# bminixhofer/zett

Hardware: AMD Instinct MI355X
Metric: predicted token-embeddings/sec (full target vocab) (higher is better)
Workload: dtype f16

## Files before the change

### zett_amd/csrc/gemm.hip.h

```cpp
#pragma once

#include <hip/hip_runtime.h>
#include <stdint.h>

#include <type_traits>

#ifndef ZETT_GROUP_M
#define ZETT_GROUP_M 4
#endif

namespace zett {

typedef __attribute__((ext_vector_type(16))) float f32x16;
typedef __attribute__((ext_vector_type(4))) float f32x4;
typedef __attribute__((ext_vector_type(8))) __bf16 bf16x8;
typedef __attribute__((ext_vector_type(4))) uint32_t u32x4;

typedef uint16_t bf16_t;
typedef _Float16 f16_t;
typedef __attribute__((ext_vector_type(8))) _Float16 f16x8;

__device__ __forceinline__ float bf16_to_f32(bf16_t v) { return __uint_as_float(((uint32_t)v) << 16); }
__device__ __forceinline__ bf16_t f32_to_bf16(float f) {
    return __builtin_bit_cast(bf16_t, (__bf16)f);
// ... 76 lines not shown
}

typedef __attribute__((ext_vector_type(2))) float f32x2;
#define ZETT_PIN_STAGE(arr, n) do { _Pragma("unroll") for (int e_ = 0; e_ < (n); ++e_) asm volatile("" : "+v"((arr)[e_])); } while (0)

template <int ACT, bool HAS_RES, bool HAS_SCALE, int NV>
__device__ __forceinline__ void epi_values(float (&vs)[NV], const float (&bias)[NV], const float (&res)[NV], const float (&sc)[NV], const float (&sh)[NV]) {
#pragma clang fp contract(off)
    static_assert(NV % 2 == 0, "pairs");
    constexpr int NP = NV / 2;
    f32x2 v[NP];
#pragma unroll
    for (int e = 0; e < NP; ++e) v[e] = f32x2{vs[2 * e], vs[2 * e + 1]} + f32x2{bias[2 * e], bias[2 * e + 1]};
    if (ACT == ACT_GELU_TANH) {
        f32x2 u2[NP], t[NP];
        ZETT_PIN_STAGE(v, NP);
#pragma unroll
        for (int e = 0; e < NP; ++e) u2[e] = (v[e] * v[e]) * v[e];
        ZETT_PIN_STAGE(u2, NP);
#pragma unroll
        for (int e = 0; e < NP; ++e) u2[e] = 1.5957691216057308f * __builtin_elementwise_fma(f32x2{0.044715f, 0.044715f}, u2[e], v[e]);
        ZETT_PIN_STAGE(u2, NP);
#pragma unroll
        for (int e = 0; e < NP; ++e) u2[e] = u2[e] * 1.4426950408889634f;
        ZETT_PIN_STAGE(u2, NP);
#pragma unroll
        for (int e = 0; e < NP; ++e) t[e] = f32x2{__builtin_amdgcn_exp2f(u2[e].x), __builtin_amdgcn_exp2f(u2[e].y)};
        ZETT_PIN_STAGE(t, NP);
#pragma unroll
        for (int e = 0; e < NP; ++e) t[e] = 1.0f + t[e];
        ZETT_PIN_STAGE(t, NP);
#pragma unroll
        for (int e = 0; e < NP; ++e) t[e] = f32x2{__builtin_amdgcn_rcpf(t[e].x), __builtin_amdgcn_rcpf(t[e].y)};
        ZETT_PIN_STAGE(t, NP);
#pragma unroll
        for (int e = 0; e < NP; ++e) t[e] = 1.0f - 2.0f * t[e];
        ZETT_PIN_STAGE(t, NP);
#pragma unroll
        for (int e = 0; e < NP; ++e) v[e] = (0.5f * v[e]) * (1.0f + t[e]);
        ZETT_PIN_STAGE(v, NP);
    } else if (ACT == ACT_GELU_ERF) {
        f32x2 z[NP], ax[NP], t[NP], p[NP], ex[NP];
        ZETT_PIN_STAGE(v, NP);
#pragma unroll
        for (int e = 0; e < NP; ++e) z[e] = v[e] * 0.70710678118654752440f;
        ZETT_PIN_STAGE(z, NP);
#pragma unroll
        for (int e = 0; e < NP; ++e) ax[e] = __builtin_elementwise_abs(z[e]);
#pragma unroll
        for (int e = 0; e < NP; ++e) t[e] = __builtin_elementwise_fma(f32x2{0.3275911f, 0.3275911f}, ax[e], f32x2{1.0f, 1.0f});
        ZETT_PIN_STAGE(t, NP);
#pragma unroll
        for (int e = 0; e < NP; ++e) t[e] = f32x2{__builtin_amdgcn_rcpf(t[e].x), __builtin_amdgcn_rcpf(t[e].y)};
        ZETT_PIN_STAGE(t, NP);
#pragma unroll
        for (int e = 0; e < NP; ++e) ex[e] = (ax[e] * ax[e]) * -1.4426950408889634f;
        ZETT_PIN_STAGE(ex, NP);
#pragma unroll
        for (int e = 0; e < NP; ++e) ex[e] = f32x2{__builtin_amdgcn_exp2f(ex[e].x), __builtin_amdgcn_exp2f(ex[e].y)};
        ZETT_PIN_STAGE(ex, NP);
#pragma unroll
        for (int e = 0; e < NP; ++e) p[e] = __builtin_elementwise_fma(f32x2{1.061405429f, 1.061405429f}, t[e], f32x2{-1.453152027f, -1.453152027f});
        ZETT_PIN_STAGE(p, NP);
#pragma unroll
        for (int e = 0; e < NP; ++e) p[e] = __builtin_elementwise_fma(p[e], t[e], f32x2{1.421413741f, 1.421413741f});
        ZETT_PIN_STAGE(p, NP);
#pragma unroll
        for (int e = 0; e < NP; ++e) p[e] = __builtin_elementwise_fma(p[e], t[e], f32x2{-0.284496736f, -0.284496736f});
        ZETT_PIN_STAGE(p, NP);
#pragma unroll
        for (int e = 0; e < NP; ++e) p[e] = __builtin_elementwise_fma(p[e], t[e], f32x2{0.254829592f, 0.254829592f});
        ZETT_PIN_STAGE(p, NP);
#pragma unroll
        for (int e = 0; e < NP; ++e) p[e] = -(p[e] * t[e]);
        ZETT_PIN_STAGE(p, NP);
#pragma unroll
        for (int e = 0; e < NP; ++e) p[e] = __builtin_elementwise_fma(p[e], ex[e], f32x2{1.0f, 1.0f});
        ZETT_PIN_STAGE(p, NP);
#pragma unroll
        for (int e = 0; e < NP; ++e) p[e] = 1.0f + __builtin_elementwise_copysign(p[e], z[e]);
        ZETT_PIN_STAGE(p, NP);
#pragma unroll
        for (int e = 0; e < NP; ++e) v[e] = (v[e] * 0.5f) * p[e];
        ZETT_PIN_STAGE(v, NP);
    }
    if (HAS_RES) {
#pragma unroll
        for (int e = 0; e < NP; ++e) v[e] = v[e] + f32x2{res[2 * e], res[2 * e + 1]};
    }
    if (HAS_SCALE) {
#pragma unroll
        for (int e = 0; e < NP; ++e) v[e] = __builtin_elementwise_fma(f32x2{sc[2 * e], sc[2 * e + 1]}, v[e], f32x2{sh[2 * e], sh[2 * e + 1]});
    }
#pragma unroll
    for (int e = 0; e < NP; ++e) { vs[2 * e] = v[e].x; vs[2 * e + 1] = v[e].y; }
}

template <typename T>
struct GemmEpilogue {
    const float* bias;
    int act;
    const float* residual;
    int ld_res;
    const float* res_stats;
    const float* res_gamma;
    const float* res_beta;
    const int32_t* res_index;
    float2* stats_part;
    int ld_part;
    const float* fold_stats;
    const float* fold_c;
    const float* scale;
    const float* shift;
    float* out_f32;
    int ld_f32;
    T* out_lo;
    int ld_lo;
    int split_col;
    float* out_f32_b;
    int32_t* range_flag;
    int range_final;
    const T* residual_lo;
    int ld_res_lo;
    void* dst;
    const int64_t* dst_rows;
    int64_t ld_dst;
    int dst_dtype;
};

template <typename T> struct LoRange { static constexpr bool checked = false; static constexpr float limit = 0.f; };
template <> struct LoRange<f16_t> { static constexpr bool checked = true; static constexpr float limit = 65504.0f; };
__device__ __forceinline__ bool out_of_range(float v, float limit) { return !(__builtin_fabsf(v) <= limit); }
constexpr float ZETT_F32_MAX = 3.402823466e38f;
constexpr int ZETT_RANGE_BIT_SOURCE = 1, ZETT_RANGE_BIT_ACTIVATION = 2, ZETT_RANGE_BIT_OUTPUT = 4, ZETT_RANGE_BIT_WEIGHT = 8, ZETT_RANGE_BIT_DEST = 16;
template <typename OT> __device__ __forceinline__ bool dest_overflow(float v) {
    if constexpr (std::is_same<OT, f16_t>::value) { const float a = __builtin_fabsf(v); return a >= 65520.0f && a <= 3.402823466e38f; }
    else return false;
}
__device__ __forceinline__ void range_report(int32_t* flag, bool bad, int bit) {
    if (bad && flag) atomicOr(flag, bit);
}

template <typename T>
struct GemmArgs {
    const T* A;
    int lda;
    const T* W;
    int ldw;
    int M, N, K;
    GemmEpilogue<T> epi;
    int tile_order = 0;
    int group = 0;
    int row0 = 0;
};

constexpr int GEMM_BM = 128;
constexpr int GEMM_BN = 128;
constexpr int GEMM_WAIT_VMCNT0 = 0x0F70;
constexpr int GEMM_ROW_BYTES = 128;
constexpr int GEMM_TILE_BYTES = GEMM_BM * GEMM_ROW_BYTES;

__device__ __forceinline__ int lds_chunk_off(int row, int chunk) {
    return row * GEMM_ROW_BYTES + ((chunk ^ ((row >> 1) & 7)) << 4);
}

template <typename T>
__device__ __forceinline__ void mfma_chunk(const u32x4& a, const u32x4& b, f32x16& acc);

template <>
__device__ __forceinline__ void mfma_chunk<bf16_t>(const u32x4& a, const u32x4& b, f32x16& acc) {
    acc = __builtin_amdgcn_mfma_f32_32x32x16_bf16(__builtin_bit_cast(bf16x8, a), __builtin_bit_cast(bf16x8, b),
                                                  acc, 0, 0, 0);
}
template <>
__device__ __forceinline__ void mfma_chunk<f16_t>(const u32x4& a, const u32x4& b, f32x16& acc) {
    acc = __builtin_amdgcn_mfma_f32_32x32x16_f16(__builtin_bit_cast(f16x8, a), __builtin_bit_cast(f16x8, b), acc, 0, 0, 0);
}
template <>
__device__ __forceinline__ void mfma_chunk<float>(const u32x4& a, const u32x4& b, f32x16& acc) {
#pragma unroll
    for (int j = 0; j < 4; ++j)
        acc = __builtin_amdgcn_mfma_f32_32x32x2f32(__uint_as_float(a[j]), __uint_as_float(b[j]), acc, 0, 0, 0);
}

template <typename T>
__global__ __launch_bounds__(256) void gemm_tn_kernel(GemmArgs<T> g) {
    extern __shared__ __attribute__((aligned(16))) unsigned char smem[];
    constexpr int EPC = 16 / (int)sizeof(T);
    constexpr int BK = GEMM_ROW_BYTES / (int)sizeof(T);

    const int tiles_m = (g.M + GEMM_BM - 1) / GEMM_BM;
    const int tiles_n = (g.N + GEMM_BN - 1) / GEMM_BN;
    const int nwg = tiles_m * tiles_n;
    int wg = blockIdx.x;
    {
        const int q = nwg >> 3, r = nwg & 7, xcd = wg & 7;
        wg = (xcd < r ? xcd * (q + 1) : r * (q + 1) + (xcd - r) * q) + (wg >> 3);
    }
    constexpr int GROUP_M = 8;
    const int group_size = GROUP_M * tiles_n;
    const int first_m = (wg / group_size) * GROUP_M;
    const int gm = (tiles_m - first_m) < GROUP_M ? (tiles_m - first_m) : GROUP_M;
    const int tm = first_m + (wg % group_size) % gm;
    const int tn = (wg % group_size) / gm;
    const int m0 = tm * GEMM_BM, n0 = tn * GEMM_BN;

    const int tid = threadIdx.x;
    const int lane = tid & 63, wave = tid >> 6;
    const int wm = wave >> 1, wn = wave & 1;
    const int l31 = lane & 31, hi = lane >> 5;

    const unsigned char* a_src[4];
    const unsigned char* w_src[4];
    int lds_dst[4];
#pragma unroll
    for (int i = 0; i < 4; ++i) {
        const int c = tid + 256 * i;
        const int row = c >> 3, ch = c & 7;
        int ar = m0 + row; ar = ar < g.M ? ar : g.M - 1;
        int wr = n0 + row; wr = wr < g.N ? wr : g.N - 1;
        a_src[i] = (const unsigned char*)(g.A + (size_t)ar * g.lda) + ch * 16;
        w_src[i] = (const unsigned char*)(g.W + (size_t)wr * g.ldw) + ch * 16;
        lds_dst[i] = lds_chunk_off(row, ch);
    }

    f32x16 acc[2][2];
#pragma unroll
    for (int i = 0; i < 2; ++i)
#pragma unroll
        for (int j = 0; j < 2; ++j)
#pragma unroll
            for (int r = 0; r < 16; ++r) acc[i][j][r] = 0.f;

    const int nk = g.K / BK;
    u32x4 ra[4], rw[4];
#pragma unroll
    for (int i = 0; i < 4; ++i) {
        ra[i] = *(const u32x4*)(a_src[i]);
        rw[i] = *(const u32x4*)(w_src[i]);
    }
#pragma unroll
    for (int i = 0; i < 4; ++i) {
        *(u32x4*)(smem + lds_dst[i]) = ra[i];
        *(u32x4*)(smem + GEMM_TILE_BYTES + lds_dst[i]) = rw[i];
    }
    __syncthreads();

    for (int kt = 0; kt < nk; ++kt) {
        const int cur = kt & 1;
        const unsigned char* As = smem + cur * 2 * GEMM_TILE_BYTES;
        const unsigned char* Ws = As + GEMM_TILE_BYTES;
        const bool more = kt + 1 < nk;
        if (more) {
            const size_t koff = (size_t)(kt + 1) * GEMM_ROW_BYTES;
#pragma unroll
            for (int i = 0; i < 4; ++i) {
                ra[i] = *(const u32x4*)(a_src[i] + koff);
                rw[i] = *(const u32x4*)(w_src[i] + koff);
            }
        }
#pragma unroll
        for (int kk = 0; kk < 4; ++kk) {
            const int ch = kk * 2 + hi;
            u32x4 fa[2], fw[2];
#pragma unroll
            for (int i = 0; i < 2; ++i) {
                fa[i] = *(const u32x4*)(As + lds_chunk_off(wm * 64 + i * 32 + l31, ch));
                fw[i] = *(const u32x4*)(Ws + lds_chunk_off(wn * 64 + i * 32 + l31, ch));
            }
#pragma unroll
            for (int i = 0; i < 2; ++i)
#pragma unroll
                for (int j = 0; j < 2; ++j) mfma_chunk<T>(fa[i], fw[j], acc[i][j]);
        }
        if (more) {
            unsigned char* Ad = smem + (cur ^ 1) * 2 * GEMM_TILE_BYTES;
#pragma unroll
            for (int i = 0; i < 4; ++i) {
                *(u32x4*)(Ad + lds_dst[i]) = ra[i];
                *(u32x4*)(Ad + GEMM_TILE_BYTES + lds_dst[i]) = rw[i];
            }
        }
        __syncthreads();
    }
    (void)EPC;

    const GemmEpilogue<T>& e = g.epi;
    bool bad_lo = false, bad_out = false;
#pragma unroll
    for (int j = 0; j < 2; ++j) {
        const int col = n0 + wn * 64 + j * 32 + l31;
        if (col >= g.N) continue;
        const float bias = e.bias ? e.bias[col] : 0.f;
        const float sc = e.scale ? e.scale[col] : 1.f;
        const float sh = e.shift ? e.shift[col] : 0.f;
#pragma unroll
        for (int i = 0; i < 2; ++i) {
#pragma unroll
            for (int r = 0; r < 16; ++r) {
                const int row = m0 + wm * 64 + i * 32 + (r & 3) + 8 * (r >> 2) + 4 * hi;
                if (row >= g.M) continue;
                const size_t rrow = e.res_index ? (size_t)e.res_index[row] : (size_t)row;
                float res = e.residual ? e.residual[rrow * e.ld_res + col] : 0.f;
                if (e.residual && e.res_stats) res = ln_affine(res, e.res_stats[2 * rrow], e.res_stats[2 * rrow + 1], e.res_gamma[col], e.res_beta[col]);
                const bool hr = e.residual != nullptr, hs = e.scale != nullptr;
                const float v = e.act == ACT_GELU_TANH ? epi_value<ACT_GELU_TANH>(acc[i][j][r], bias, hr, res, hs, sc, sh)
                              : e.act == ACT_GELU_ERF ? epi_value<ACT_GELU_ERF>(acc[i][j][r], bias, hr, res, hs, sc, sh)
// ... 31 lines not shown
```

### zett_amd/csrc/gemm4d.hip.h

```cpp
#pragma once

#include <hip/hip_runtime.h>
#include <stdint.h>

#include <algorithm>
#include <type_traits>

#include "gemm_tile.hip.h"

namespace zett {

#ifndef G4D_ABLATE
#define G4D_ABLATE 5
#endif
constexpr int G4D_ABL = G4D_ABLATE;
#ifdef G4D_MFMA32
constexpr bool G4D_M32 = true;
static_assert(G4D_ABLATE < 5, "the 32x32x16 K loop exists for the ablation levels without an epilogue");
#else
constexpr bool G4D_M32 = false;
#endif
typedef float f32x16 __attribute__((ext_vector_type(16)));

constexpr int g4d_wait_vm(int n) { return ((n >> 4) << 14) | 0x0F70 | (n & 15); }

template <typename T> __device__ __forceinline__ void mfma16_agpr(f32x4& c, const u32x4& a, const u32x4& b);
template <> __device__ __forceinline__ void mfma16_agpr<bf16_t>(f32x4& c, const u32x4& a, const u32x4& b) {
    asm volatile("v_mfma_f32_16x16x32_bf16 %0, %1, %2, %0" : "+a"(c) : "v"(a), "v"(b));
}
template <> __device__ __forceinline__ void mfma16_agpr<f16_t>(f32x4& c, const u32x4& a, const u32x4& b) {
    asm volatile("v_mfma_f32_16x16x32_f16 %0, %1, %2, %0" : "+a"(c) : "v"(a), "v"(b));
}

template <typename T> __device__ __forceinline__ void mfma32_agpr(f32x16& c, const u32x4& a, const u32x4& b);
template <> __device__ __forceinline__ void mfma32_agpr<bf16_t>(f32x16& c, const u32x4& a, const u32x4& b) {
    asm volatile("v_mfma_f32_32x32x16_bf16 %0, %1, %2, %0" : "+a"(c) : "v"(a), "v"(b));
}
template <> __device__ __forceinline__ void mfma32_agpr<f16_t>(f32x16& c, const u32x4& a, const u32x4& b) {
    asm volatile("v_mfma_f32_32x32x16_f16 %0, %1, %2, %0" : "+a"(c) : "v"(a), "v"(b));
}

template <int K> __device__ __forceinline__ float g4d_xor_lane(float v) {
    return __builtin_bit_cast(float, __builtin_amdgcn_ds_swizzle(__builtin_bit_cast(int, v), (K << 10) | 0x1f));
}


enum { G4D_EPI_GENERIC = 0, G4D_EPI_LO = 1, G4D_EPI_F32 = 2, G4D_EPI_F32_SCALE = 3, G4D_EPI_BOTH = 4, G4D_EPI_F32_LN = 5, G4D_EPI_LO_FOLD = 6,
       G4D_EPI_LO_LN = 7, G4D_EPI_F32_SCALE_FOLD = 8, G4D_EPI_LN16 = 9 };
constexpr int G4D_EPI_STRIDE = 132;
constexpr int G4D_EPI_REGION = 64 * G4D_EPI_STRIDE * 4;
constexpr int G4D_LDS_BYTES = 4 * G4D_EPI_REGION;
static_assert(G4D_LDS_BYTES >= G256_LDS_BYTES && G4D_LDS_BYTES <= 160 * 1024, "LDS budget");

template <bool HALF> struct G4dGeom {
    static constexpr int BM = HALF ? 128 : G256_BM;
    static constexpr int WROWS = BM / 2;
    static constexpr int MI = WROWS / 16;
    static constexpr int AREQ = BM / 32;
    static constexpr int NREQ = AREQ + 8;
    static constexpr int NPASS = WROWS / 64;
    static constexpr int STAGES = HALF ? 3 : 2;
    static constexpr int A_BYTES = BM * GEMM_ROW_BYTES;
    static constexpr int STAGE_BYTES = A_BYTES + G256_OPERAND_BYTES;
    static constexpr int LDS_BYTES = STAGES * STAGE_BYTES;
};

template <typename T, int ACT = ACT_NONE, bool RES = false, int EPI = G4D_EPI_GENERIC, bool HALF = false, typename OT = void>
__global__ __launch_bounds__(256) __attribute__((amdgpu_waves_per_eu(1, 1))) void gemm4d_tn_kernel(GemmArgs<T> g) {
    extern __shared__ __attribute__((aligned(16))) unsigned char smem[];
    constexpr int BK = GEMM_ROW_BYTES / (int)sizeof(T);
    typedef G4dGeom<HALF> GEO;
    static_assert(!HALF || EPI != G4D_EPI_GENERIC, "the half tile carries the streamlined epilogues only");
    constexpr bool DST = !std::is_void<OT>::value;
    static_assert(!DST || EPI == G4D_EPI_F32_SCALE || EPI == G4D_EPI_F32_SCALE_FOLD, "destination stores: the output heads' epilogues only");

    const int tiles_m = (g.M - g.row0 + GEO::BM - 1) / GEO::BM;
    const int tiles_n = (g.N + G256_BN - 1) / G256_BN;
    const int nwg = tiles_m * tiles_n;
    int wg = blockIdx.x;
    {
        const int q = nwg >> 3, r = nwg & 7, xcd = wg & 7;
        wg = (xcd < r ? xcd * (q + 1) : r * (q + 1) + (xcd - r) * q) + (wg >> 3);
    }
    const int GROUP_N = g.group > 0 ? g.group : 4;
    int tm, tn;
    if (g.tile_order == 0) {
        const int group_size = GROUP_N * tiles_m;
        const int first_n = (wg / group_size) * GROUP_N;
        const int gn = (tiles_n - first_n) < GROUP_N ? (tiles_n - first_n) : GROUP_N;
        tn = first_n + (wg % group_size) % gn;
        tm = (wg % group_size) / gn;
    } else {
        const int GROUP_M = g.group > 0 ? g.group : ZETT_GROUP_M;
        const int group_size = GROUP_M * tiles_n;
        const int first_m = (wg / group_size) * GROUP_M;
        const int gm = (tiles_m - first_m) < GROUP_M ? (tiles_m - first_m) : GROUP_M;
        tm = first_m + (wg % group_size) % gm;
        tn = (wg % group_size) / gm;
    }
    const int m0 = g.row0 + tm * GEO::BM, n0 = tn * G256_BN;

    const int tid = threadIdx.x;
    const int lane = tid & 63;
    const int wave = __builtin_amdgcn_readfirstlane(tid >> 6);
    const int wm = wave >> 1, wn = wave & 1;

    const unsigned char* a_base = (const unsigned char*)(g.A + (size_t)m0 * g.lda);
    const unsigned char* w_base = (const unsigned char*)(g.W + (size_t)n0 * g.ldw);
    uint32_t a_voff[8], w_voff[8];
#pragma unroll
    for (int r = 0; r < 8; ++r) {
        const int row = wave * 64 + r * 8 + (lane >> 3);
        const int chunk = ((lane & 7) ^ ((row >> 1) & 7)) << 4;
        int wr = row; wr = n0 + wr < g.N ? wr : g.N - 1 - n0;
        w_voff[r] = (uint32_t)wr * (uint32_t)g.ldw * (uint32_t)sizeof(T) + chunk;
    }
#pragma unroll
    for (int r = 0; r < GEO::AREQ; ++r) {
        const int row = wave * (GEO::AREQ * 8) + r * 8 + (lane >> 3);
        const int chunk = ((lane & 7) ^ ((row >> 1) & 7)) << 4;
        int ar = row; ar = m0 + ar < g.M ? ar : g.M - 1 - m0;
        a_voff[r] = (uint32_t)ar * (uint32_t)g.lda * (uint32_t)sizeof(T) + chunk;
    }
    const __amdgpu_buffer_rsrc_t a_rsrc = __builtin_amdgcn_make_buffer_rsrc((void*)a_base, (short)0, 0x7fffffff, G4R_RSRC_WORD3);
    const __amdgpu_buffer_rsrc_t w_rsrc = __builtin_amdgcn_make_buffer_rsrc((void*)w_base, (short)0, 0x7fffffff, G4R_RSRC_WORD3);
    unsigned char* const my_rows = smem + wave * 64 * GEMM_ROW_BYTES;
    unsigned char* const my_a_rows = smem + wave * (GEO::AREQ * 8) * GEMM_ROW_BYTES;
    auto dma_a = [&](int stage, int kt, int r) {
        __builtin_amdgcn_raw_ptr_buffer_load_lds(a_rsrc, (lds_ptr_t)(my_a_rows + stage * GEO::STAGE_BYTES + r * 8 * GEMM_ROW_BYTES), 16,
                                                 a_voff[r], kt * GEMM_ROW_BYTES, 0, 0);
    };
    auto dma_w = [&](int stage, int kt, int r) {
        __builtin_amdgcn_raw_ptr_buffer_load_lds(w_rsrc, (lds_ptr_t)(my_rows + stage * GEO::STAGE_BYTES + GEO::A_BYTES + r * 8 * GEMM_ROW_BYTES), 16,
                                                 w_voff[r], kt * GEMM_ROW_BYTES, 0, 0);
    };

    constexpr bool M32 = G4D_M32 && !HALF;
    f32x4 acc[8][8];
    f32x16 acc32[4][4];
    if constexpr (M32) {
#pragma unroll
        for (int i = 0; i < 4; ++i)
#pragma unroll
            for (int j = 0; j < 4; ++j)
#pragma unroll
                for (int r = 0; r < 16; ++r) acc32[i][j][r] = 0.f;
    } else {
#pragma unroll
    for (int i = 0; i < GEO::MI; ++i)
#pragma unroll
        for (int j = 0; j < 8; ++j)
#pragma unroll
            for (int r = 0; r < 4; ++r) acc[i][j][r] = 0.f;
    }

    int a_off[2], w_off[2];
    {
        const int l15 = lane & 15, kq = lane >> 4;
        const int swz = (l15 >> 1) & 7;
#pragma unroll
        for (int kb = 0; kb < 2; ++kb) {
            const int c = ((kb * 4 + kq) ^ swz) << 4;
            a_off[kb] = (wm * GEO::WROWS + l15) * GEMM_ROW_BYTES + c;
            w_off[kb] = GEO::A_BYTES + (wn * 128 + l15) * GEMM_ROW_BYTES + c;
        }
    }
    int a_off32[4], w_off32[4];
    if constexpr (M32) {
        const int l31 = lane & 31, kh = lane >> 5;
        const int swz = (l31 >> 1) & 7;
#pragma unroll
        for (int k16 = 0; k16 < 4; ++k16) {
            const int c = ((k16 * 2 + kh) ^ swz) << 4;
            a_off32[k16] = (wm * GEO::WROWS + l31) * GEMM_ROW_BYTES + c;
            w_off32[k16] = GEO::A_BYTES + (wn * 128 + l31) * GEMM_ROW_BYTES + c;
        }
    }
    u32x4 fa[2][8], fw[2][8];
    auto read_a = [&](int stage, int kb, int i) {
        if constexpr (M32) fa[kb][i] = *(const u32x4*)(smem + stage * GEO::STAGE_BYTES + a_off32[kb * 2 + (i >> 2)] + (i & 3) * 32 * GEMM_ROW_BYTES);
        else fa[kb][i] = *(const u32x4*)(smem + stage * GEO::STAGE_BYTES + a_off[kb] + i * 16 * GEMM_ROW_BYTES);
    };
    auto read_w = [&](int stage, int kb, int j) {
        if constexpr (M32) fw[kb][j] = *(const u32x4*)(smem + stage * GEO::STAGE_BYTES + w_off32[kb * 2 + (j >> 2)] + (j & 3) * 32 * GEMM_ROW_BYTES);
        else fw[kb][j] = *(const u32x4*)(smem + stage * GEO::STAGE_BYTES + w_off[kb] + j * 16 * GEMM_ROW_BYTES);
    };

    const int nk = g.K / BK;
    constexpr bool LN16K = EPI == G4D_EPI_LN16;
    uint4 res16[LN16K ? 16 : 1];
    const bool res16_early = LN16K && g.epi.res_index == nullptr;
    auto res16_request = [&](int p, int t) __attribute__((always_inline)) {
        if constexpr (LN16K) {
            int grow = m0 + wm * GEO::WROWS + p * 64 + t * 4 + (lane >> 4);
            grow = grow < g.M ? grow : g.M - 1;
            int gc = n0 + wn * 128 + (lane & 15) * 8;
            gc = gc < g.N ? gc : 0;
            res16[t] = *(const uint4*)(g.epi.residual_lo + (size_t)grow * g.epi.ld_res_lo + gc);
        }
    };
#pragma unroll
    for (int st = 0; st < GEO::STAGES; ++st) {
        if (st < nk) {
#pragma unroll
            for (int r = 0; r < 8; ++r) dma_w(st, st, r);
#pragma unroll
            for (int r = 0; r < GEO::AREQ; ++r) dma_a(st, st, r);
        }
    }
    {
        const int ahead = (nk < GEO::STAGES ? nk : GEO::STAGES) - 1;
        if (ahead >= 2) __builtin_amdgcn_s_waitcnt(g4d_wait_vm(2 * GEO::NREQ));
        else if (ahead == 1) __builtin_amdgcn_s_waitcnt(g4d_wait_vm(GEO::NREQ));
        else __builtin_amdgcn_s_waitcnt(g4d_wait_vm(0));
    }
    __builtin_amdgcn_s_barrier();
    __builtin_amdgcn_sched_barrier(0);
#pragma unroll
    for (int j = 0; j < 8; ++j) read_w(0, 0, j);
#pragma unroll
    for (int i = 0; i < GEO::MI; ++i) read_a(0, 0, i);
    if constexpr (G4D_ABL < 2) {
#pragma unroll
        for (int j = 0; j < 8; ++j) read_w(0, 1, j);
#pragma unroll
        for (int i = 0; i < GEO::MI; ++i) read_a(0, 1, i);
        __builtin_amdgcn_s_waitcnt(G4R_WAIT_LGKM0);
    }

    auto step = [&](int kt, int cur, auto more_c, auto more2_c, auto moreA_c, auto wave_c) {
        constexpr bool more = decltype(more_c)::value, more2 = decltype(more2_c)::value, moreA = decltype(moreA_c)::value;
        constexpr int WV = decltype(wave_c)::value;
        const int nxt = cur + 1 == GEO::STAGES ? 0 : cur + 1;
        constexpr int P_BAR1 = HALF ? 26 : 36, P_BAR2 = HALF ? 52 : 102;
        constexpr int INFLIGHT = HALF ? ((more2 ? 1 : 0) + (moreA ? 1 : 0)) * GEO::NREQ : (moreA ? GEO::NREQ : 0);
#pragma unroll
        for (int kb = 0; kb < 2; ++kb)
#pragma unroll
        for (int i = 0; i < GEO::MI; ++i)
// ... 301 lines not shown
                            const f32x2 y = __builtin_elementwise_fma(f32x2{v[u * CPL + c], v[u * CPL + c + 1]}, r2, x);
                            v[u * CPL + c] = y.x; v[u * CPL + c + 1] = y.y;
                            bb[u * CPL + c] = 0.f; bb[u * CPL + c + 1] = 0.f;
                        }
                    }
                }
                epi_values<ACT, RES, SCALE, NV>(v, bb, rr, ss, hh);
                if constexpr (CHK16) {
#pragma unroll
                    for (int x = 0; x < NV; ++x) bad |= out_of_range(v[x], LoRange<T>::limit);
                } else if (chk_final) {
#pragma unroll
                    for (int x = 0; x < NV; ++x) bad |= out_of_range(v[x], ZETT_F32_MAX);
                }
                if constexpr (LN16) {
                    static_assert(!LN16 || (GROUP == 4 && CPL == 8 && RPI == 4), "reduce-scatter layout");
                    float S[4], Q[4];
#pragma unroll
                    for (int u = 0; u < 4; ++u) {
                        const float* x = v + 8 * u;
                        S[u] = ((x[0] + x[1]) + (x[2] + x[3])) + ((x[4] + x[5]) + (x[6] + x[7]));
                        Q[u] = __builtin_fmaf(x[0], x[0], __builtin_fmaf(x[1], x[1], __builtin_fmaf(x[2], x[2], __builtin_fmaf(x[3], x[3],
                               __builtin_fmaf(x[4], x[4], __builtin_fmaf(x[5], x[5], __builtin_fmaf(x[6], x[6], x[7] * x[7])))))));
                    }
                    const bool b3 = (idx & 8) != 0, b2 = (idx & 4) != 0;
                    float ks0 = b3 ? S[2] : S[0], ks1 = b3 ? S[3] : S[1], kq0 = b3 ? Q[2] : Q[0], kq1 = b3 ? Q[3] : Q[1];
                    ks0 += g4d_xor_lane<8>(b3 ? S[0] : S[2]); ks1 += g4d_xor_lane<8>(b3 ? S[1] : S[3]);
                    kq0 += g4d_xor_lane<8>(b3 ? Q[0] : Q[2]); kq1 += g4d_xor_lane<8>(b3 ? Q[1] : Q[3]);
                    float ks = b2 ? ks1 : ks0, kq = b2 ? kq1 : kq0;
                    ks += g4d_xor_lane<4>(b2 ? ks0 : ks1); kq += g4d_xor_lane<4>(b2 ? kq0 : kq1);
                    ks += g4d_xor_lane<2>(ks); kq += g4d_xor_lane<2>(kq);
                    ks += g4d_xor_lane<1>(ks); kq += g4d_xor_lane<1>(kq);
                    const bool mine = (idx & 3) == (t0 >> 2);
                    acc_s = mine ? ks : acc_s; acc_q = mine ? kq : acc_q;
                } else if constexpr (LNP) {
                    static_assert(GROUP == 4 && CPL == 4 && RPI == 2, "reduce-scatter layout");
                    float S[4], Q[4];
#pragma unroll
                    for (int u = 0; u < 4; ++u) {
                        const float a = v[4 * u], b = v[4 * u + 1], c = v[4 * u + 2], d = v[4 * u + 3];
                        S[u] = (a + b) + (c + d);
                        Q[u] = __builtin_fmaf(a, a, __builtin_fmaf(b, b, __builtin_fmaf(c, c, d * d)));
                    }
                    const bool b4 = (idx & 16) != 0, b3 = (idx & 8) != 0;
                    float ks0 = b4 ? S[2] : S[0], ks1 = b4 ? S[3] : S[1], kq0 = b4 ? Q[2] : Q[0], kq1 = b4 ? Q[3] : Q[1];
                    ks0 += g4d_xor_lane<16>(b4 ? S[0] : S[2]); ks1 += g4d_xor_lane<16>(b4 ? S[1] : S[3]);
                    kq0 += g4d_xor_lane<16>(b4 ? Q[0] : Q[2]); kq1 += g4d_xor_lane<16>(b4 ? Q[1] : Q[3]);
                    float ks = b3 ? ks1 : ks0, kq = b3 ? kq1 : kq0;
                    ks += g4d_xor_lane<8>(b3 ? ks0 : ks1); kq += g4d_xor_lane<8>(b3 ? kq0 : kq1);
                    ks += g4d_xor_lane<4>(ks); kq += g4d_xor_lane<4>(kq);
                    ks += g4d_xor_lane<2>(ks); kq += g4d_xor_lane<2>(kq);
                    ks += g4d_xor_lane<1>(ks); kq += g4d_xor_lane<1>(kq);
                    const bool mine = (idx & 7) == (t0 >> 2);
                    acc_s = mine ? ks : acc_s; acc_q = mine ? kq : acc_q;
                }
#pragma unroll
                for (int u = 0; u < GROUP; ++u) {
                    const int grow = grow0 + p * 64 + (t0 + u) * RPI;
                    if (!FULL && (grow >= g.M || !col_ok)) continue;
                    if constexpr (LO || LN16) {
                        const float4 a = make_float4(v[u * 8], v[u * 8 + 1], v[u * 8 + 2], v[u * 8 + 3]);
                        const float4 b = make_float4(v[u * 8 + 4], v[u * 8 + 5], v[u * 8 + 6], v[u * 8 + 7]);
                        store_out8<T>(e.out_lo + (size_t)grow * e.ld_lo + gcol, a, b);
                    } else {
                        const f32x4 x = {v[u * 4], v[u * 4 + 1], v[u * 4 + 2], v[u * 4 + 3]};
                        if constexpr (DST) {
                            const int r0 = (t0 + u) * RPI;
                            static_assert(!DST || RPI == 2, "two rows per instruction");
                            const uint64_t d64 = (uint64_t)drow[p];
                            const uint32_t lo0 = __builtin_amdgcn_readlane((uint32_t)d64, r0), hi0 = __builtin_amdgcn_readlane((uint32_t)(d64 >> 32), r0);
                            const uint32_t lo1 = __builtin_amdgcn_readlane((uint32_t)d64, r0 + 1), hi1 = __builtin_amdgcn_readlane((uint32_t)(d64 >> 32), r0 + 1);
                            const int64_t d = (int64_t)(((uint64_t)(rsub ? hi1 : hi0) << 32) | (rsub ? lo1 : lo0));
                            if (d >= 0) {
                                store_out4<OT>((OT*)e.dst + d * e.ld_dst + gcol, make_float4(x[0], x[1], x[2], x[3]));
#pragma unroll
                                for (int c = 0; c < 4; ++c) bad_dst |= dest_overflow<OT>(x[c]);
                            }
                        } else if constexpr (WF32) {
                            float* d = e.out_f32 + (size_t)grow * e.ld_f32 + gcol;
                            if (RES) asm volatile("global_store_dwordx4 %0, %1, off nt\n\ts_nop 1" :: "v"(d), "v"(x) : "memory");
                            else *(f32x4*)d = x;
                        }
                        if constexpr (EPI == G4D_EPI_BOTH || LNP)
                            store_out4<T>(e.out_lo + (size_t)grow * e.ld_lo + gcol, make_float4(x[0], x[1], x[2], x[3]));
                    }
                }
                if constexpr (LN16 && GEO::NPASS == 2) { if (p == 0 && t0 == GROUP) load_res16(1, 0, NIT / 2); }
            }
            if constexpr (LN16 && GEO::NPASS == 2) { if (p == 0) load_res16(1, NIT / 2, NIT); }
            if constexpr (LNP) {
                const int rp = LN16 ? (((4 * (idx & 3) + 2 * ((idx >> 3) & 1) + ((idx >> 2) & 1)) << 2) + rsub)
                                    : (((4 * (idx & 7) + 2 * ((idx >> 4) & 1) + ((idx >> 3) & 1)) << 1) + rsub);
                const int grow = m0 + wm * GEO::WROWS + p * 64 + rp;
                if (grow < g.M && n0 + wn * 128 < g.N)
                    e.stats_part[(size_t)((n0 + wn * 128) >> 7) * e.ld_part + grow] = make_float2(acc_s, acc_q);
            }
        };
        auto drain_pass = [&](int p) {
            const bool full = m0 + wm * GEO::WROWS + p * 64 + 64 <= g.M && n0 + wn * 128 + 128 <= g.N;
            if (full) drain(p, std::integral_constant<bool, true>{});
            else drain(p, std::integral_constant<bool, false>{});
        };
        if constexpr (LN16) { if (!res16_early) load_res(0); }
        else load_res(0);
        stage(0);
        __builtin_amdgcn_sched_barrier(0);
        if constexpr (!LNP && GEO::NPASS == 2) load_res(1);
        __builtin_amdgcn_sched_barrier(0);
        drain_pass(0);
        if constexpr (GEO::NPASS == 2) {
            if constexpr (LNP && !LN16) { __builtin_amdgcn_sched_barrier(0); load_res(1); __builtin_amdgcn_sched_barrier(0); }
            stage(1);
            drain_pass(1);
        }
        range_report(e.range_flag, bad, W16 ? ZETT_RANGE_BIT_ACTIVATION : ZETT_RANGE_BIT_OUTPUT);
        if constexpr (DST) range_report(e.range_flag, bad_dst, ZETT_RANGE_BIT_DEST);
    }
}

template <typename T>
inline int gemm4d_epi_mode(const GemmArgs<T>& g) {
    const GemmEpilogue<T>& e = g.epi;
    if (e.stats_part && e.residual_lo) {
        if (sizeof(T) == 2 && e.out_lo && !e.out_f32 && !e.residual && e.act == ACT_NONE && !e.scale && !e.shift && !e.out_f32_b && e.split_col >= g.N &&
            g.N % 128 == 0 && e.ld_lo % 8 == 0 && e.ld_res_lo % 8 == 0) return G4D_EPI_LN16;
        return -1;
    }
    if (e.stats_part) {
        const bool common = e.out_lo && e.residual && !e.scale && !e.shift && !e.out_f32_b && e.split_col >= g.N && g.N % 128 == 0 &&
                            e.ld_lo % 4 == 0 && e.ld_res % 4 == 0;
        if (common && e.out_f32 && e.act == ACT_NONE && e.ld_f32 % 4 == 0) return G4D_EPI_F32_LN;
        if (common && !e.out_f32 && e.act == ACT_GELU_TANH && !e.res_stats && !e.res_index) return G4D_EPI_LO_LN;
        return -1;
    }
    if (e.fold_stats) {
        if (e.fold_c && e.out_lo && !e.out_f32 && !e.residual && !e.scale && !e.shift && !e.out_f32_b && e.split_col >= g.N &&
            g.N % 8 == 0 && e.ld_lo % 8 == 0) return G4D_EPI_LO_FOLD;
        if (e.fold_c && e.out_f32 && !e.out_lo && !e.residual && e.scale && e.shift && e.act == ACT_NONE && !e.out_f32_b && e.split_col >= g.N &&
            g.N % 4 == 0 && e.ld_f32 % 4 == 0) return G4D_EPI_F32_SCALE_FOLD;
        return -1;
    }
    if (e.out_f32_b || e.split_col < g.N) return G4D_EPI_GENERIC;
    if (e.res_stats && (e.act != ACT_NONE || !e.residual)) return G4D_EPI_GENERIC;
    if (e.out_lo && !e.out_f32 && !e.residual && !e.scale && !e.shift && g.N % 8 == 0 && e.ld_lo % 8 == 0) return G4D_EPI_LO;
    if (e.out_f32 && e.out_lo && !e.residual && !e.scale && !e.shift && e.act == ACT_NONE && g.N % 4 == 0 && e.ld_f32 % 4 == 0 && e.ld_lo % 4 == 0)
        return G4D_EPI_BOTH;
    if (e.out_f32 && !e.out_lo && g.N % 4 == 0 && e.ld_f32 % 4 == 0 && (!e.residual || e.ld_res % 4 == 0)) {
        if (e.scale && e.shift && !e.residual && e.act == ACT_NONE) return G4D_EPI_F32_SCALE;
        if (!e.scale && !e.shift && (e.act == ACT_NONE || (e.act == ACT_GELU_TANH && e.residual))) return G4D_EPI_F32;
    }
    return G4D_EPI_GENERIC;
}

template <typename T, int ACT, bool RES, int EPI, bool HALF = false>
inline hipError_t launch_gemm4d_inst(const GemmArgs<T>& g, hipStream_t stream) {
    constexpr int lds = EPI == G4D_EPI_GENERIC ? G256_LDS_BYTES : (G4dGeom<HALF>::LDS_BYTES > G4D_LDS_BYTES ? G4dGeom<HALF>::LDS_BYTES : G4D_LDS_BYTES);
    static_assert(lds <= 160 * 1024, "LDS budget");
    static DeviceFlags attr;
    bool* done = attr.current();
    if (!done || !*done) {
        hipError_t e = hipFuncSetAttribute((const void*)gemm4d_tn_kernel<T, ACT, RES, EPI, HALF>, hipFuncAttributeMaxDynamicSharedMemorySize, lds);
        if (e != hipSuccess) return e;
        if (done) *done = true;
    }
    constexpr int BM = HALF ? 128 : G256_BM;
    const int tiles_m = (g.M - g.row0 + BM - 1) / BM;
    const int tiles_n = (g.N + G256_BN - 1) / G256_BN;
    if (tiles_m <= 0 || tiles_n <= 0) return hipSuccess;
    hipLaunchKernelGGL((gemm4d_tn_kernel<T, ACT, RES, EPI, HALF>), dim3(tiles_m * tiles_n), dim3(256), lds, stream, g);
    return hipGetLastError();
}

template <typename T, int ACT, bool HALF>
inline hipError_t launch_gemm4d_act(const GemmArgs<T>& g, hipStream_t stream, int mode) {
    const bool res = g.epi.residual != nullptr;
    switch (mode) {
        case G4D_EPI_LO: return launch_gemm4d_inst<T, ACT, false, G4D_EPI_LO, HALF>(g, stream);
        case G4D_EPI_LO_FOLD: return launch_gemm4d_inst<T, ACT, false, G4D_EPI_LO_FOLD, HALF>(g, stream);
        case G4D_EPI_F32:
            if constexpr (ACT == ACT_NONE) return res ? launch_gemm4d_inst<T, ACT, true, G4D_EPI_F32, HALF>(g, stream) : launch_gemm4d_inst<T, ACT, false, G4D_EPI_F32, HALF>(g, stream);
            else if constexpr (ACT == ACT_GELU_TANH) { if (res) return launch_gemm4d_inst<T, ACT, true, G4D_EPI_F32, HALF>(g, stream); }
            [[fallthrough]];
        default:
            if constexpr (HALF) return hipErrorInvalidValue;
            else return res ? launch_gemm4d_inst<T, ACT, true, G4D_EPI_GENERIC>(g, stream) : launch_gemm4d_inst<T, ACT, false, G4D_EPI_GENERIC>(g, stream);
    }
}

template <typename T, bool HALF>
inline hipError_t launch_gemm4d_mode(const GemmArgs<T>& g, hipStream_t stream, int mode) {
    if (mode == G4D_EPI_F32_LN) return launch_gemm4d_inst<T, ACT_NONE, true, G4D_EPI_F32_LN, HALF>(g, stream);
    if (mode == G4D_EPI_LN16) return launch_gemm4d_inst<T, ACT_NONE, true, G4D_EPI_LN16, HALF>(g, stream);
    if (mode == G4D_EPI_LO_LN) return launch_gemm4d_inst<T, ACT_GELU_TANH, true, G4D_EPI_LO_LN, HALF>(g, stream);
    if (mode == G4D_EPI_F32_SCALE_FOLD) return launch_gemm4d_inst<T, ACT_NONE, false, G4D_EPI_F32_SCALE_FOLD, HALF>(g, stream);
    if (mode == G4D_EPI_F32_SCALE) return launch_gemm4d_inst<T, ACT_NONE, false, G4D_EPI_F32_SCALE, HALF>(g, stream);
    if (mode == G4D_EPI_BOTH) return launch_gemm4d_inst<T, ACT_NONE, false, G4D_EPI_BOTH, HALF>(g, stream);
    switch (g.epi.act) {
        case ACT_GELU_TANH: return launch_gemm4d_act<T, ACT_GELU_TANH, HALF>(g, stream, mode);
        case ACT_GELU_ERF: return launch_gemm4d_act<T, ACT_GELU_ERF, HALF>(g, stream, mode);
        default: return launch_gemm4d_act<T, ACT_NONE, HALF>(g, stream, mode);
    }
}

template <typename T>
inline bool gemm4d_half_ok(const GemmArgs<T>& g, int mode) {
    if (mode <= G4D_EPI_GENERIC) return false;
    if (mode == G4D_EPI_F32) return g.epi.act == ACT_NONE || (g.epi.act == ACT_GELU_TANH && g.epi.residual);
    return true;
}

inline int gemm4d_row_split(int M, int N, int cus = 256, double half_cost = 0.62) {
    const long tn = (N + G256_BN - 1) / G256_BN, tm = (M + G256_BM - 1) / G256_BM;
    const long T = tm * tn;
    if (T % cus == 0) return M;
    const long rounds = (T + cus - 1) / cus;
    const long tm_full = std::min<long>(tm, ((rounds - 1) * cus) / tn);
    const long row0 = tm_full * G256_BM;
    if (row0 >= M) return M;
    const long th = ((M - row0 + 127) / 128) * tn;
    const double cost = (double)((tm_full * tn + cus - 1) / cus) + half_cost * (double)((th + cus - 1) / cus);
    return cost < (double)rounds - 0.05 ? (int)row0 : M;
}

template <typename T, int EPI, typename OT, bool HALF>
inline hipError_t launch_gemm4d_dst_inst(const GemmArgs<T>& g, hipStream_t stream) {
    constexpr int lds = G4dGeom<HALF>::LDS_BYTES > G4D_LDS_BYTES ? G4dGeom<HALF>::LDS_BYTES : G4D_LDS_BYTES;
    static DeviceFlags attr;
    bool* done = attr.current();
    if (!done || !*done) {
        hipError_t e = hipFuncSetAttribute((const void*)gemm4d_tn_kernel<T, ACT_NONE, false, EPI, HALF, OT>, hipFuncAttributeMaxDynamicSharedMemorySize, lds);
        if (e != hipSuccess) return e;
        if (done) *done = true;
    }
    constexpr int BM = HALF ? 128 : G256_BM;
    const int tiles_m = (g.M - g.row0 + BM - 1) / BM;
    const int tiles_n = (g.N + G256_BN - 1) / G256_BN;
    if (tiles_m <= 0 || tiles_n <= 0) return hipSuccess;
    hipLaunchKernelGGL((gemm4d_tn_kernel<T, ACT_NONE, false, EPI, HALF, OT>), dim3(tiles_m * tiles_n), dim3(256), lds, stream, g);
    return hipGetLastError();
}

template <typename T, bool HALF>
inline hipError_t launch_gemm4d_dst_mode(const GemmArgs<T>& g, hipStream_t stream, int mode) {
    const int dt = g.epi.dst_dtype;
    if (mode == G4D_EPI_F32_SCALE_FOLD) {
        if (dt == 1) return launch_gemm4d_dst_inst<T, G4D_EPI_F32_SCALE_FOLD, f16_t, HALF>(g, stream);
        if (dt == 2) return launch_gemm4d_dst_inst<T, G4D_EPI_F32_SCALE_FOLD, bf16_t, HALF>(g, stream);
        return launch_gemm4d_dst_inst<T, G4D_EPI_F32_SCALE_FOLD, float, HALF>(g, stream);
    }
    if (dt == 1) return launch_gemm4d_dst_inst<T, G4D_EPI_F32_SCALE, f16_t, HALF>(g, stream);
    if (dt == 2) return launch_gemm4d_dst_inst<T, G4D_EPI_F32_SCALE, bf16_t, HALF>(g, stream);
    return launch_gemm4d_dst_inst<T, G4D_EPI_F32_SCALE, float, HALF>(g, stream);
}

template <typename T>
inline int gemm4d_dst_mode(const GemmArgs<T>& g) {
    const GemmEpilogue<T>& e = g.epi;
    if (!e.dst || e.dst_dtype < 0 || e.dst_dtype > 2 || e.ld_dst % 4 != 0) return -1;
    const size_t align = e.dst_dtype == 0 ? 16 : 8;
    if ((uintptr_t)e.dst % align) return -1;
    GemmArgs<T> f = g;
    f.epi.out_f32 = (float*)e.dst;
    f.epi.ld_f32 = 4;
    const int mode = gemm4d_epi_mode(f);
    return (mode == G4D_EPI_F32_SCALE || mode == G4D_EPI_F32_SCALE_FOLD) ? mode : -1;
}

hipError_t launch_gemm_4d_half(const GemmArgs<f16_t>& g, hipStream_t stream, int mode);
hipError_t launch_gemm_4d_half(const GemmArgs<bf16_t>& g, hipStream_t stream, int mode);

hipError_t launch_gemm_4d_half_dst(const GemmArgs<f16_t>& g, hipStream_t stream, int mode);
hipError_t launch_gemm_4d_half_dst(const GemmArgs<bf16_t>& g, hipStream_t stream, int mode);

template <typename T>
inline hipError_t launch_gemm4d(const GemmArgs<T>& g, hipStream_t stream, bool force_generic = false) {
    const bool dst = g.epi.dst != nullptr;
    const int mode = dst ? gemm4d_dst_mode(g) : (force_generic && !g.epi.stats_part && !g.epi.fold_stats) ? G4D_EPI_GENERIC : gemm4d_epi_mode(g);
    if (mode < 0) return hipErrorInvalidValue;
    int split = g.row0 == -1 ? gemm4d_row_split(g.M, g.N) : (g.row0 == -2 ? 0 : (g.row0 > 0 ? std::min(g.row0, g.M) : g.M));
    if (split < g.M && (!gemm4d_half_ok(g, mode) || split % G256_BM != 0)) split = g.M;
    GemmArgs<T> full = g;
    full.row0 = 0;
    if (split < g.M) {
        full.M = split;
        if (split > 0)
            if (hipError_t e = dst ? launch_gemm4d_dst_mode<T, false>(full, stream, mode) : launch_gemm4d_mode<T, false>(full, stream, mode); e != hipSuccess) return e;
        GemmArgs<T> rest = g;
        rest.row0 = split;
        return dst ? launch_gemm_4d_half_dst(rest, stream, mode) : launch_gemm_4d_half(rest, stream, mode);
    }
    return dst ? launch_gemm4d_dst_mode<T, false>(full, stream, mode) : launch_gemm4d_mode<T, false>(full, stream, mode);
}

}
```

### zett_amd/csrc/gemm4d.inc

```
#include <hip/hip_runtime.h>

#include "gemm.hip.h"
#include "gemm_tile.hip.h"
#include "gemm4d.hip.h"
#include "gemm_launch.hip.h"

namespace zett {

hipError_t launch_gemm_4d(const GemmArgs<ZETT_GEMM_T>& g, hipStream_t stream, bool generic_epilogue) {
    return launch_gemm4d<ZETT_GEMM_T>(g, stream, generic_epilogue);
}

int gemm_4d_dst_mode(const GemmArgs<ZETT_GEMM_T>& g) { return gemm4d_dst_mode<ZETT_GEMM_T>(g); }

}
```

### zett_amd/csrc/gemm_launch.hip.h

```cpp
#pragma once

#include <hip/hip_runtime.h>

#include "gemm.hip.h"

namespace zett {

hipError_t launch_gemm_variant(int variant, const GemmArgs<f16_t>& g, hipStream_t stream);
hipError_t launch_gemm_variant(int variant, const GemmArgs<bf16_t>& g, hipStream_t stream);
hipError_t launch_gemm_variant(int variant, const GemmArgs<float>& g, hipStream_t stream);

hipError_t launch_gemm_x(int variant, const GemmArgs<f16_t>& g, hipStream_t stream);
hipError_t launch_gemm_x(int variant, const GemmArgs<bf16_t>& g, hipStream_t stream);
hipError_t launch_gemm_x(int variant, const GemmArgs<float>& g, hipStream_t stream);
hipError_t launch_gemm_4d(const GemmArgs<f16_t>& g, hipStream_t stream, bool generic_epilogue);
hipError_t launch_gemm_4d(const GemmArgs<bf16_t>& g, hipStream_t stream, bool generic_epilogue);
int gemm_4d_dst_mode(const GemmArgs<f16_t>& g);
int gemm_4d_dst_mode(const GemmArgs<bf16_t>& g);
inline int gemm_4d_dst_mode(const GemmArgs<float>&) { return -1; }

}
```

### zett_amd/csrc/rowops.hip.h

```cpp
#pragma once

#include <hip/hip_runtime.h>
#include <stdint.h>

#include <type_traits>

#include "gemm.hip.h"

namespace zett {


struct PlanArrays {
    int32_t* row_count;
    int32_t* row_offset;
    uint8_t* row_uniform;
    int32_t* id_flag;
    int32_t* id_slot;
    int32_t* id_list;
    int32_t* tok_slot;
    int32_t* tok_pos;
    int32_t* tok_row;
    int32_t* tok_pkey;
    int32_t* pair_flag;
    int32_t* pair_slot;
    int32_t* tok_pair;
    int32_t* pair_tslot;
    int32_t* pair_pos;
    uint8_t* tok_key;
    int32_t* err;
    int32_t* counters;
    int32_t n_pair_keys;
};

__global__ void plan_rows_kernel(const int32_t* __restrict__ sfm, int64_t n_rows, int seq, int pad, int lam,
                                 int n_ids, PlanArrays p) {
    const int64_t n = (int64_t)blockIdx.x * blockDim.x + threadIdx.x;
    if (n >= n_rows) return;
    const int32_t* row = sfm + n * seq;
    int visible = 0;
    for (int j = 0; j < seq; ++j) {
        const int id = row[j];
        if (id < 0 || id >= n_ids) {
            atomicMax(p.err, (int)(n < 0x7ffffffe ? n + 1 : 0x7fffffff));
            p.row_count[n] = 0;
            p.row_uniform[n] = 2;
            return;
        }
        visible += (id != pad);
    }
    const bool uniform = (visible + lam) == 0;
    int count;
    if (uniform) {
        count = seq;
        for (int j = 0; j < seq; ++j) p.id_flag[row[j]] = 1;
    } else {
        count = visible + lam + (row[0] == pad ? 1 : 0);
        for (int j = 0; j < seq; ++j)
            if (j == 0 || row[j] != pad) p.id_flag[row[j]] = 1;
    }
    p.row_count[n] = count;
    p.row_uniform[n] = uniform ? 1 : 0;
}

__global__ __launch_bounds__(1024) void exclusive_scan_kernel(const int32_t* __restrict__ in,
                                                              int32_t* __restrict__ out, int64_t n) {
    __shared__ int32_t part[1024];
    const int t = threadIdx.x;
    const int64_t per = (n + 1023) / 1024;
    const int64_t b = (int64_t)t * per, e = (b + per < n) ? b + per : n;
    int32_t s = 0;
    for (int64_t i = b; i < e; ++i) s += in[i];
    part[t] = s;
    __syncthreads();
    for (int off = 1; off < 1024; off <<= 1) {
        int32_t v = (t >= off) ? part[t - off] : 0;
        __syncthreads();
        part[t] += v;
        __syncthreads();
    }
    int32_t run = (t == 0) ? 0 : part[t - 1];
    for (int64_t i = b; i < e; ++i) { const int32_t v = in[i]; out[i] = run; run += v; }
    if (t == 1023) out[n] = part[1023];
}

constexpr int SCAN_CHUNK = 4096;

__device__ __forceinline__ int32_t block_exclusive_scan_256(int32_t v, int32_t* sh , int32_t* total) {
    const int t = threadIdx.x;
    sh[t] = v;
    __syncthreads();
    for (int off = 1; off < 256; off <<= 1) {
        const int32_t add = (t >= off) ? sh[t - off] : 0;
        __syncthreads();
        sh[t] += add;
        __syncthreads();
    }
    if (total) *total = sh[255];
    return sh[t] - v;
}

__global__ __launch_bounds__(256) void scan_chunk_sums_kernel(const int32_t* __restrict__ in, int64_t n, int32_t* __restrict__ sums) {
    __shared__ int32_t sh[256];
    const int64_t base = (int64_t)blockIdx.x * SCAN_CHUNK + threadIdx.x * 16;
    int32_t s = 0;
#pragma unroll
    for (int k = 0; k < 16; ++k) { const int64_t i = base + k; if (i < n) s += in[i]; }
    int32_t total;
    block_exclusive_scan_256(s, sh, &total);
    if (threadIdx.x == 0) sums[blockIdx.x] = total;
}

__global__ __launch_bounds__(256) void scan_apply_kernel(const int32_t* __restrict__ in, int64_t n, const int32_t* __restrict__ offs,
                                                         int32_t* __restrict__ out) {
    __shared__ int32_t sh[256];
    const int64_t base = (int64_t)blockIdx.x * SCAN_CHUNK + threadIdx.x * 16;
    int32_t v[16];
    int32_t s = 0;
#pragma unroll
    for (int k = 0; k < 16; ++k) { const int64_t i = base + k; v[k] = i < n ? in[i] : 0; s += v[k]; }
    int32_t run = offs[blockIdx.x] + block_exclusive_scan_256(s, sh, nullptr);
#pragma unroll
    for (int k = 0; k < 16; ++k) { const int64_t i = base + k; if (i < n) out[i] = run; run += v[k]; }
    if (blockIdx.x == gridDim.x - 1 && threadIdx.x == 0) out[n] = offs[gridDim.x];
}

inline void launch_exclusive_scan(const int32_t* in, int32_t* out, int64_t n, int32_t* scratch, hipStream_t st) {
    if (n <= SCAN_CHUNK * 4) {
        hipLaunchKernelGGL(exclusive_scan_kernel, dim3(1), dim3(1024), 0, st, in, out, n);
        return;
    }
    const int chunks = (int)((n + SCAN_CHUNK - 1) / SCAN_CHUNK);
    int32_t* sums = scratch;
    int32_t* offs = scratch + chunks;
    hipLaunchKernelGGL(scan_chunk_sums_kernel, dim3(chunks), dim3(256), 0, st, in, n, sums);
    hipLaunchKernelGGL(exclusive_scan_kernel, dim3(1), dim3(1024), 0, st, (const int32_t*)sums, offs, (int64_t)chunks);
    hipLaunchKernelGGL(scan_apply_kernel, dim3(chunks), dim3(256), 0, st, in, n, (const int32_t*)offs, out);
}

__global__ void plan_tokens_kernel(const int32_t* __restrict__ sfm, int64_t n_rows, int seq, int pad, int lam,
                                   int n_ids, PlanArrays p) {
    const int64_t n = (int64_t)blockIdx.x * blockDim.x + threadIdx.x;
    if (n >= n_rows) return;
    const int32_t* row = sfm + n * seq;
    int t = p.row_offset[n];
    if (p.row_uniform[n] == 2) return;
    const bool uniform = p.row_uniform[n] == 1;
    const int lp = seq + lam;
    for (int j = 0; j < seq; ++j) {
        const int id = row[j];
        const bool vis = id != pad;
        if (uniform || vis || j == 0) {
            p.tok_slot[t] = p.id_slot[id];
            p.tok_pos[t] = j;
            p.tok_row[t] = (int32_t)n;
            p.tok_key[t] = vis ? 1 : 0;
            if (p.pair_flag) { const int key = id * lp + j; p.tok_pkey[t] = key; p.pair_flag[key] = 1; }
            ++t;
        }
    }
    if (lam) {
        p.tok_slot[t] = -1;
        p.tok_pos[t] = seq;
        p.tok_row[t] = (int32_t)n;
        p.tok_key[t] = 1;
        if (p.pair_flag) { const int key = n_ids * lp + seq; p.tok_pkey[t] = key; p.pair_flag[key] = 1; }
    }
}

__global__ void plan_pairs_kernel(int64_t n_rows, PlanArrays p) {
    const int64_t t = (int64_t)blockIdx.x * blockDim.x + threadIdx.x;
    if (t >= p.row_offset[n_rows]) return;
    const int ps = p.pair_slot[p.tok_pkey[t]];
    p.tok_pair[t] = ps;
    p.pair_tslot[ps] = p.tok_slot[t];
    p.pair_pos[ps] = p.tok_pos[t];
}

__device__ __forceinline__ int chunk_row(int t_rel, int row_rel, bool first, int rows);
__global__ void pair_rows_kernel(int m, int tok0, int64_t row0, int rows, PlanArrays p, int32_t* __restrict__ brow_pair) {
    const int t = blockIdx.x * blockDim.x + threadIdx.x;
    if (t >= m) return;
    const int n = p.tok_row[tok0 + t];
    brow_pair[chunk_row(t, (int)(n - row0), p.row_offset[n] == tok0 + t, rows)] = p.tok_pair[tok0 + t];
}

__global__ void plan_idlist_kernel(int n_ids, PlanArrays p) {
    const int id = blockIdx.x * blockDim.x + threadIdx.x;
    if (id < n_ids && p.id_flag[id]) p.id_list[p.id_slot[id]] = id;
    if (id == 0) {
        p.counters[0] = p.id_slot[n_ids];
        p.counters[1] = p.err[0];
        p.counters[2] = p.n_pair_keys ? p.pair_slot[p.n_pair_keys] : 0;
    }
}

__device__ __forceinline__ float wave_sum(float v) {
#pragma unroll
    for (int off = 32; off > 0; off >>= 1) v += __shfl_xor(v, off, 64);
    return v;
}

__device__ __forceinline__ float block_sum_256(float v, float* red ) {
    v = wave_sum(v);
    __syncthreads();
    if ((threadIdx.x & 63) == 0) red[threadIdx.x >> 6] = v;
    __syncthreads();
    return red[0] + red[1] + red[2] + red[3];
}

template <typename T> __device__ __forceinline__ void store_lo4(T* dst, float4 v);
template <> __device__ __forceinline__ void store_lo4<float>(float* dst, float4 v) { *(float4*)dst = v; }
template <> __device__ __forceinline__ void store_lo4<bf16_t>(bf16_t* dst, float4 v) {
    *(uint2*)dst = make_uint2(pack2_lo<bf16_t>(v.x, v.y), pack2_lo<bf16_t>(v.z, v.w));
}
template <> __device__ __forceinline__ void store_lo4<f16_t>(f16_t* dst, float4 v) {
    *(uint2*)dst = make_uint2(pack2_lo<f16_t>(v.x, v.y), pack2_lo<f16_t>(v.z, v.w));
}

template <int SRC_DTYPE> __device__ __forceinline__ float4 load_src4(const void* base, size_t elem);
template <> __device__ __forceinline__ float4 load_src4<0>(const void* base, size_t e) {
    return *(const float4*)((const float*)base + e);
}
template <> __device__ __forceinline__ float4 load_src4<1>(const void* base, size_t e) {
    const uint2 u = *(const uint2*)((const uint16_t*)base + e);
    typedef __attribute__((ext_vector_type(4))) _Float16 f16x4;
    const f16x4 hv = __builtin_bit_cast(f16x4, u);
    return make_float4((float)hv[0], (float)hv[1], (float)hv[2], (float)hv[3]);
}
template <> __device__ __forceinline__ float4 load_src4<2>(const void* base, size_t e) {
    const uint2 u = *(const uint2*)((const uint16_t*)base + e);
    return make_float4(__uint_as_float(u.x << 16), __uint_as_float(u.x & 0xffff0000u),
                       __uint_as_float(u.y << 16), __uint_as_float(u.y & 0xffff0000u));
}

template <typename T, int SRC_DTYPE>
__global__ __launch_bounds__(256) void gather_src_kernel(const int32_t* __restrict__ id_list, int slot0, int n_slots,
                                                         const void* __restrict__ src, int e_in, int v0,
                                                         const float* __restrict__ fallback,
                                                         const float* __restrict__ sc_w, const float* __restrict__ sc_b,
                                                         T* __restrict__ out, int32_t* __restrict__ range_flag) {
    const int s = blockIdx.x;
    if (s >= n_slots) return;
    const int id = id_list[slot0 + s];
    T* dst = out + (size_t)s * e_in;
    bool bad = false;
    auto chk = [&](float4 v) {
        if (LoRange<T>::checked)
            bad |= out_of_range(v.x, LoRange<T>::limit) | out_of_range(v.y, LoRange<T>::limit) | out_of_range(v.z, LoRange<T>::limit) |
                   out_of_range(v.w, LoRange<T>::limit);
    };
    if (id >= v0) {
        const float* f = fallback + (size_t)(id - v0) * e_in;
        for (int c = threadIdx.x * 4; c < e_in; c += 1024) { const float4 v = *(const float4*)(f + c); chk(v); store_lo4<T>(dst + c, v); }
    } else {
        const size_t base = (size_t)id * e_in;
        for (int c = threadIdx.x * 4; c < e_in; c += 1024) {
            float4 v = load_src4<SRC_DTYPE>(src, base + c);
            if (sc_w) {
                const float4 w = *(const float4*)(sc_w + c), b = *(const float4*)(sc_b + c);
                v.x = w.x * v.x + b.x; v.y = w.y * v.y + b.y; v.z = w.z * v.z + b.z; v.w = w.w * v.w + b.w;
            }
            chk(v);
            store_lo4<T>(dst + c, v);
        }
    }
    range_report(range_flag, bad, ZETT_RANGE_BIT_SOURCE);
}

struct LnEmbed {
    const float* table;
    const int32_t* tok_slot;
    const int32_t* tok_pos;
    const float* type0;
    const float* pos_emb;
    const float* lang;
    int lang_pos;
    const int32_t* tok_row;
    const int32_t* row_offset;
    int64_t row0;
    int rows;
    const void* table_lo;
    const float* table_stats;
    const float* table_gamma;
    const float* table_beta;
};

__device__ __forceinline__ int chunk_row(int t_rel, int row_rel, bool first, int rows) {
    return first ? row_rel : rows + t_rel - row_rel - 1;
}

struct LnReadout {
    const float* bias_w;
    const float* bias_b;
    float* out_bias;
    const void* in_lo;
    const int64_t* bias_rows;
    int32_t* range_flag;
};

template <typename BT> __device__ __forceinline__ void ln_readout_store(const LnReadout& ro, int r, float v) {
    if constexpr (std::is_void<BT>::value) {
        ro.out_bias[r] = v;
    } else {
        const int64_t d = ro.bias_rows ? ro.bias_rows[r] : (int64_t)r;
        if (d < 0) return;
        ((BT*)ro.out_bias)[d] = to_lo<BT>(v);
        range_report(ro.range_flag, dest_overflow<BT>(v), ZETT_RANGE_BIT_DEST);
    }
}

constexpr int LN_MAX_VEC = 8;

template <typename T, bool EMBED, int TPR = 256, bool READOUT = false, typename BT = void>
__global__ __launch_bounds__(256) void layernorm_rows_kernel(const float* __restrict__ in, int ld_in, int rows, int H,
                                                             const float* __restrict__ gamma,
                                                             const float* __restrict__ beta, float eps,
                                                             float* __restrict__ out_f32, T* __restrict__ out_lo,
                                                             float* __restrict__ stats_out, float* __restrict__ sum_out,
                                                             LnEmbed emb, int tok0, LnReadout readout) {
    __shared__ float red[4];
    const int r = blockIdx.x * (256 / TPR) + (int)threadIdx.x / TPR;
    if (r >= rows) return;
    const int nvec = H >> 2;
    const int tid = threadIdx.x % TPR;
    auto row_sum = [&](float x_) { return TPR == 256 ? block_sum_256(x_, red) : wave_sum(x_); };
    const float* x = nullptr;
    const float* posr = nullptr;
    bool is_lang = false;
    int ro = r;
    const T* tbl_lo = nullptr;
    float2 tbl_st = make_float2(0.f, 1.f);
    if constexpr (EMBED) {
        const int slot = emb.tok_slot[tok0 + r];
        is_lang = slot < 0;
        if (emb.table_lo && !is_lang) {
            tbl_lo = (const T*)emb.table_lo + (size_t)slot * H;
            tbl_st = *(const float2*)(emb.table_stats + 2 * (size_t)slot);
            x = emb.lang;
        } else
        x = is_lang ? emb.lang : emb.table + (size_t)slot * H;
        posr = emb.pos_emb + (size_t)emb.tok_pos[tok0 + r] * H;
        if (emb.tok_row) {
            const int n = emb.tok_row[tok0 + r];
            ro = chunk_row(r, (int)(n - emb.row0), emb.row_offset[n] == tok0 + r, emb.rows);
        }
// ... 187 lines not shown
                load8<float>(emb.pos_emb + (size_t)emb.lang_pos * H + c, pl);
#pragma unroll
                for (int k = 0; k < 8; ++k) a[k] -= (t0[k] + pl[k]);
            }
#pragma unroll
            for (int k = 0; k < 8; ++k) a[k] = (a[k] + t0[k]) + p[k];
        }
    };
    float v[NVMAX][8];
    float s = 0.f;
#pragma unroll
    for (int j = 0; j < NVMAX; ++j) {
        if (j < nv) {
            load((tid + TPR * j) * 8, v[j]);
            s += ((v[j][0] + v[j][1]) + (v[j][2] + v[j][3])) + ((v[j][4] + v[j][5]) + (v[j][6] + v[j][7]));
        }
    }
    const float mean = group_sum<TPR>(s) / (float)H;
    float q = 0.f;
#pragma unroll
    for (int j = 0; j < NVMAX; ++j) {
        if (j < nv) {
            float d[8];
#pragma unroll
            for (int k = 0; k < 8; ++k) { d[k] = v[j][k] - mean; d[k] *= d[k]; }
            q += ((d[0] + d[1]) + (d[2] + d[3])) + ((d[4] + d[5]) + (d[6] + d[7]));
        }
    }
    const float var = group_sum<TPR>(q) / (float)H;
    const float rstd = 1.0f / sqrtf(var + eps);
    if (stats_out && tid == 0) *(float2*)(stats_out + 2 * (size_t)ro) = make_float2(mean, rstd);
    float dot = 0.f;
#pragma unroll
    for (int j = 0; j < NVMAX; ++j) {
        if (j < nv) {
            const int c = (tid + TPR * j) * 8;
            float g[8], b[8], o[8];
            load8<float>(gamma + c, g);
            load8<float>(beta + c, b);
#pragma unroll
            for (int k = 0; k < 8; ++k) o[k] = ln_affine(v[j][k], mean, rstd, g[k], b[k]);
            if (EMBED && sum_out) store8<float>(sum_out + (size_t)ro * H + c, v[j]);
            if (out_f32) store8<float>(out_f32 + (size_t)ro * H + c, o);
            if (out_lo) store8<T>(out_lo + (size_t)ro * H + c, o);
            if (READOUT && readout.bias_w) {
                float w[8];
                load8<float>(readout.bias_w + c, w);
                dot += ((o[0] * w[0] + o[1] * w[1]) + (o[2] * w[2] + o[3] * w[3])) + ((o[4] * w[4] + o[5] * w[5]) + (o[6] * w[6] + o[7] * w[7]));
            }
        }
    }
    if constexpr (READOUT) {
        if (readout.out_bias) {
            const float tot = group_sum<TPR>(dot);
            if (tid == 0) ln_readout_store<BT>(readout, r, readout.bias_w ? tot + readout.bias_b[0] : 0.f);
        }
    }
}

constexpr int ATT_FAST_KEYS = 8;

template <typename T> __device__ __forceinline__ float dot8_lo(const uint4& a, const uint4& b);
template <> __device__ __forceinline__ float dot8_lo<f16_t>(const uint4& a, const uint4& b) {
    typedef __attribute__((ext_vector_type(2))) _Float16 h2;
    float s = __builtin_amdgcn_fdot2(__builtin_bit_cast(h2, a.x), __builtin_bit_cast(h2, b.x), 0.f, false);
    s = __builtin_amdgcn_fdot2(__builtin_bit_cast(h2, a.y), __builtin_bit_cast(h2, b.y), s, false);
    s = __builtin_amdgcn_fdot2(__builtin_bit_cast(h2, a.z), __builtin_bit_cast(h2, b.z), s, false);
    return __builtin_amdgcn_fdot2(__builtin_bit_cast(h2, a.w), __builtin_bit_cast(h2, b.w), s, false);
}
template <> __device__ __forceinline__ float dot8_lo<bf16_t>(const uint4& a, const uint4& b) {
    float x[8], y[8];
    unpack2_lo<bf16_t>(a.x, x[0], x[1]); unpack2_lo<bf16_t>(a.y, x[2], x[3]); unpack2_lo<bf16_t>(a.z, x[4], x[5]); unpack2_lo<bf16_t>(a.w, x[6], x[7]);
    unpack2_lo<bf16_t>(b.x, y[0], y[1]); unpack2_lo<bf16_t>(b.y, y[2], y[3]); unpack2_lo<bf16_t>(b.z, y[4], y[5]); unpack2_lo<bf16_t>(b.w, y[6], y[7]);
    float s = 0.f;
#pragma unroll
    for (int c = 0; c < 8; ++c) s = fmaf(x[c], y[c], s);
    return s;
}
template <> __device__ __forceinline__ float dot8_lo<float>(const uint4&, const uint4&) { return 0.f; }

__device__ __forceinline__ float head_sum(float s, int lph) {
    auto dpp = [](float v, auto ctrl) {
        return __builtin_bit_cast(float, __builtin_amdgcn_update_dpp(0, __builtin_bit_cast(int, v), decltype(ctrl)::value, 0xf, 0xf, true));
    };
    if (lph >= 2) s += dpp(s, std::integral_constant<int, 0xB1>{});
    if (lph >= 4) s += dpp(s, std::integral_constant<int, 0x4E>{});
    if (lph >= 8) s += dpp(s, std::integral_constant<int, 0x141>{});
    if (lph >= 16) s += dpp(s, std::integral_constant<int, 0x140>{});
    if (lph >= 32) s += __builtin_bit_cast(float, __builtin_amdgcn_ds_swizzle(__builtin_bit_cast(int, s), (16 << 10) | 0x1f));
    if (lph >= 64) s += __shfl_xor(s, 32, 64);
    return s;
}

struct AttentionWaves { int64_t total, full; int full_groups, lanes_per_row; };
__host__ __device__ inline AttentionWaves attention_waves(int rows, int H, bool pack) {
    const int rem = H & 511, gfull = H >> 9;
    AttentionWaves a;
    if (pack && (rem == 256 || rem == 128 || rem == 64)) {
        a.full_groups = gfull; a.lanes_per_row = rem >> 3;
        a.full = (int64_t)rows * gfull;
        const int per = 64 / a.lanes_per_row;
        a.total = a.full + (rows + per - 1) / per;
    } else {
        a.full_groups = (H + 511) >> 9; a.lanes_per_row = 64;
        a.full = (int64_t)rows * a.full_groups;
        a.total = a.full;
    }
    return a;
}

template <typename T>
__global__ __launch_bounds__(256) void attention_rows_kernel(const T* __restrict__ qbase, size_t ldq,
                                                             const T* __restrict__ kbase, const T* __restrict__ vbase,
                                                             size_t ldkv, int H, int head_dim,
                                                             const int32_t* __restrict__ row_offset,
                                                             const uint8_t* __restrict__ row_uniform,
                                                             const uint8_t* __restrict__ tok_key, int64_t row0,
                                                             int rows, int tok0, float scaling, int flags ,
                                                             const int32_t* __restrict__ tok_pair, T* __restrict__ ctx) {
    const int cls_only = flags & 1;
    const int lane = threadIdx.x & 63;
    const int64_t w = (int64_t)blockIdx.x * 4 + (threadIdx.x >> 6);
    const AttentionWaves aw = attention_waves(rows, H, (flags & 4) != 0);
    if (w >= aw.total) return;
    int rl, grp, li = lane, base = 0, lpr = 64;
    bool valid = true;
    if (w < aw.full) { rl = (int)(w / aw.full_groups); grp = (int)(w % aw.full_groups); }
    else {
        lpr = aw.lanes_per_row;
        const int sub = lane / lpr;
        li = lane - sub * lpr;
        base = sub * lpr;
        rl = (int)(w - aw.full) * (64 / lpr) + sub;
        grp = aw.full_groups;
        valid = rl < rows;
        if (!valid) rl = rows - 1;
    }
    const int col = grp * 512 + li * 8;
    const bool active = valid && col < H;
    const int lph = head_dim >> 3;
    const int64_t n = row0 + rl;
    const int t0 = row_offset[n] - tok0, t1 = row_offset[n + 1] - tok0;
    const bool uniform = row_uniform[n];
    const int nq = cls_only ? 1 : (t1 - t0);
    const int ccol = active ? col : 0;
    auto brow = [&](int t) -> size_t { return (size_t)chunk_row(t, rl, t == t0, rows); };
    int pslot = 0;
    if (tok_pair) { const int t = t0 + li; pslot = t < t1 ? tok_pair[tok0 + t] : 0; }
    auto qrow = [&](int t) -> size_t {
        if (!tok_pair) return brow(t);
        return t - t0 < lpr ? (size_t)__shfl(pslot, base + (t - t0), 64) : (size_t)tok_pair[tok0 + t];
    };
    const int nk = t1 - t0;
    if constexpr (sizeof(T) == 2) {
        if (nk <= ATT_FAST_KEYS && (flags & 2)) {
            const bool mine = li < nk && (uniform || tok_key[tok0 + t0 + li] != 0);
            const unsigned on = (unsigned)(__ballot(mine) >> base) & (lpr >= 32 ? 0xffffffffu : ((1u << lpr) - 1u));
            uint4 kk[ATT_FAST_KEYS], vv[ATT_FAST_KEYS], qq[ATT_FAST_KEYS];
#pragma unroll
            for (int j = 0; j < ATT_FAST_KEYS; ++j) {
                if (j < nk) {
                    const size_t kr = qrow(t0 + j);
                    kk[j] = *(const uint4*)(kbase + kr * ldkv + ccol);
                    vv[j] = *(const uint4*)(vbase + kr * ldkv + ccol);
                    if (!cls_only) qq[j] = *(const uint4*)(qbase + kr * ldq + ccol);
                }
            }
            if (cls_only) qq[0] = *(const uint4*)(qbase + (size_t)rl * ldq + ccol);
            const float sc2 = scaling * 1.4426950408889634f;
#pragma unroll
            for (int qi = 0; qi < ATT_FAST_KEYS; ++qi) {
                if (qi < nq) {
                    float sj[ATT_FAST_KEYS];
                    float mx = -INFINITY;
#pragma unroll
                    for (int j = 0; j < ATT_FAST_KEYS; ++j) {
                        sj[j] = -INFINITY;
                        if (j < nk && ((on >> j) & 1u)) {
                            const float d = head_sum(dot8_lo<T>(qq[qi], kk[j]), lph);
                            sj[j] = uniform ? 0.f : d * sc2;
                            mx = fmaxf(mx, sj[j]);
                        }
                    }
                    float l = 0.f, acc[8];
#pragma unroll
                    for (int c = 0; c < 8; ++c) acc[c] = 0.f;
#pragma unroll
                    for (int j = 0; j < ATT_FAST_KEYS; ++j) {
                        if (j < nk && ((on >> j) & 1u)) {
                            const float pj = __builtin_amdgcn_exp2f(sj[j] - mx);
                            l += pj;
                            float v[8];
                            unpack2_lo<T>(vv[j].x, v[0], v[1]); unpack2_lo<T>(vv[j].y, v[2], v[3]);
                            unpack2_lo<T>(vv[j].z, v[4], v[5]); unpack2_lo<T>(vv[j].w, v[6], v[7]);
#pragma unroll
                            for (int c = 0; c < 8; ++c) acc[c] = fmaf(pj, v[c], acc[c]);
                        }
                    }
                    const float inv = 1.0f / l;
#pragma unroll
                    for (int c = 0; c < 8; ++c) acc[c] *= inv;
                    if (active) {
                        const size_t orow = cls_only ? (size_t)rl : brow(t0 + qi);
                        store8<T>(ctx + orow * H + col, acc);
                    }
                }
            }
            return;
        }
    }
    for (int qi = 0; qi < nq; ++qi) {
        float q[8];
        load8<T>(qbase + (cls_only ? (size_t)rl : qrow(t0 + qi)) * ldq + ccol, q);
        float mx = -INFINITY, l = 0.f, acc[8];
#pragma unroll
        for (int c = 0; c < 8; ++c) acc[c] = 0.f;
        for (int kj = t0; kj < t1; ++kj) {
            if (!uniform && !tok_key[tok0 + kj]) continue;
            float k[8], v[8];
            const size_t kr = qrow(kj);
            load8<T>(kbase + kr * ldkv + ccol, k);
            load8<T>(vbase + kr * ldkv + ccol, v);
            float s = 0.f;
#pragma unroll
            for (int c = 0; c < 8; ++c) s = fmaf(q[c], k[c], s);
            for (int off = 1; off < lph; off <<= 1) s += __shfl_xor(s, off, 64);
            s = uniform ? 0.f : s * scaling;
            const float nm = fmaxf(mx, s);
            const float corr = expf(mx - nm);
            const float p = expf(s - nm);
            l = fmaf(l, corr, p);
#pragma unroll
            for (int c = 0; c < 8; ++c) acc[c] = fmaf(acc[c], corr, p * v[c]);
            mx = nm;
        }
        const float inv = 1.0f / l;
#pragma unroll
        for (int c = 0; c < 8; ++c) acc[c] *= inv;
        if (active) {
            const size_t orow = cls_only ? (size_t)rl : brow(t0 + qi);
            store8<T>(ctx + orow * H + col, acc);
        }
    }
}

__global__ __launch_bounds__(64) void ln_stats_kernel(const float2* __restrict__ part, int parts, int ld_part, int rows, int H, float eps,
                                                      float* __restrict__ stats) {
    const int r = blockIdx.x * blockDim.x + threadIdx.x;
    if (r >= rows) return;
    float s = 0.f, q = 0.f;
    const float2* col = part + r;
    int p = 0;
    for (; p + 8 <= parts; p += 8) {
        float2 v[8];
#pragma unroll
        for (int j = 0; j < 8; ++j) v[j] = col[(size_t)(p + j) * ld_part];
#pragma unroll
        for (int j = 0; j < 8; ++j) { s += v[j].x; q += v[j].y; }
    }
    {
        float2 v[8];
#pragma unroll
        for (int j = 0; j < 8; ++j) v[j] = p + j < parts ? col[(size_t)(p + j) * ld_part] : make_float2(0.f, 0.f);
#pragma unroll
        for (int j = 0; j < 8; ++j)
            if (p + j < parts) { s += v[j].x; q += v[j].y; }
    }
    const float mean = s / (float)H;
    const float var = fmaxf(q / (float)H - mean * mean, 0.f);
    *(float2*)(stats + 2 * (size_t)r) = make_float2(mean, 1.0f / sqrtf(var + eps));
}

template <typename T>
__global__ __launch_bounds__(256) void fold_weight_kernel(const float* __restrict__ w, int K, const float* __restrict__ gamma,
                                                          const float* __restrict__ beta, const float* __restrict__ bias,
                                                          T* __restrict__ w_fold, float* __restrict__ c_out, float* __restrict__ b_out,
                                                          int32_t* __restrict__ range_flag) {
    __shared__ float red[4];
    const int n = blockIdx.x;
    const float* row = w + (size_t)n * K;
    float cs = 0.f, bs = 0.f;
    for (int k = threadIdx.x; k < K; k += 256) {
        const float x = row[k];
        if (LoRange<T>::checked) range_report(range_flag, out_of_range(x * gamma[k], LoRange<T>::limit), ZETT_RANGE_BIT_WEIGHT);
        const T lo = to_lo<T>(x * gamma[k]);
        w_fold[(size_t)n * K + k] = lo;
        cs += lo_to_f32<T>(lo);
        bs = fmaf(x, beta[k], bs);
    }
    const float ct = block_sum_256(cs, red);
    const float bt = block_sum_256(bs, red);
    if (threadIdx.x == 0) { c_out[n] = ct; b_out[n] = bias[n] + bt; }
}

template <typename T>
__global__ void convert_f32_to_lo_kernel(const float* __restrict__ in, T* __restrict__ out, size_t n, int32_t* __restrict__ range_flag) {
    size_t i = ((size_t)blockIdx.x * blockDim.x + threadIdx.x) * 4;
    const size_t stride = (size_t)gridDim.x * blockDim.x * 4;
    bool bad = false;
    for (; i + 3 < n; i += stride) {
        const float4 v = *(const float4*)(in + i);
        if (LoRange<T>::checked)
            bad |= out_of_range(v.x, LoRange<T>::limit) | out_of_range(v.y, LoRange<T>::limit) | out_of_range(v.z, LoRange<T>::limit) |
                   out_of_range(v.w, LoRange<T>::limit);
        store_lo4<T>(out + i, v);
    }
    if (blockIdx.x == 0 && threadIdx.x == 0) {
        for (size_t j = n & ~(size_t)3; j < n; ++j) { out[j] = to_lo<T>(in[j]); if (LoRange<T>::checked) bad |= out_of_range(in[j], LoRange<T>::limit); }
    }
    range_report(range_flag, bad, ZETT_RANGE_BIT_WEIGHT);
}
template <int SRC_DTYPE>
__global__ void convert_to_f32_kernel(const void* __restrict__ in, float* __restrict__ out, size_t n) {
    size_t i = (size_t)blockIdx.x * blockDim.x + threadIdx.x;
    const size_t stride = (size_t)gridDim.x * blockDim.x;
    for (; i < n; i += stride) {
        if constexpr (SRC_DTYPE == 1) out[i] = (float)((const _Float16*)in)[i];
        else out[i] = __uint_as_float(((uint32_t)((const uint16_t*)in)[i]) << 16);
    }
}

template <typename OT> __device__ __forceinline__ void store4_dst(OT* d, float4 v) {
    if constexpr (std::is_same<OT, float>::value) *(float4*)d = v;
    else *(uint2*)d = make_uint2(pack2_lo<OT>(v.x, v.y), pack2_lo<OT>(v.z, v.w));
}

template <typename OT, bool VEC>
__global__ __launch_bounds__(256) void dest_store_rows_kernel(const float* __restrict__ src, int64_t ld_src, OT* __restrict__ dst, int64_t ld_dst,
                                                              const int64_t* __restrict__ rows, int64_t n_rows, int cols, int32_t* range_flag) {
    bool bad = false;
    for (int64_t i = blockIdx.x; i < n_rows; i += gridDim.x) {
        const int64_t d = rows ? rows[i] : i;
        if (d < 0) continue;
        const float* s = src + i * ld_src;
        OT* o = dst + d * ld_dst;
        if constexpr (VEC) {
            for (int c = (int)threadIdx.x * 4; c < cols; c += 256 * 4) {
                const float4 v = *(const float4*)(s + c);
                store4_dst<OT>(o + c, v);
                bad |= dest_overflow<OT>(v.x) | dest_overflow<OT>(v.y) | dest_overflow<OT>(v.z) | dest_overflow<OT>(v.w);
            }
        } else {
            for (int c = (int)threadIdx.x; c < cols; c += 256) {
                const float v = s[c];
                o[c] = to_lo<OT>(v);
                bad |= dest_overflow<OT>(v);
            }
        }
    }
    range_report(range_flag, bad, ZETT_RANGE_BIT_DEST);
}

__global__ void dest_rows_check_kernel(const int64_t* __restrict__ rows, int64_t n, int64_t n_dest, int32_t* err) {
    const int64_t i = (int64_t)blockIdx.x * blockDim.x + threadIdx.x;
    if (i < n && rows[i] >= n_dest) atomicMax(err, (int)(i < 0x7ffffffe ? i + 1 : 0x7fffffff));
}

}
```

### zett_amd/csrc/zett_hip.hip

```cpp
#include <hip/hip_runtime.h>

#include <algorithm>
#include <array>
#include <cstdlib>
#include <cmath>
#include <cstdarg>
#include <cstdio>
#include <cstring>
#include <map>
#include <string>
#include <type_traits>
#include <vector>

#include "../../include/zett_hip.h"
#include "common.hip.h"
#include "gemm.hip.h"
#include "gemm_launch.hip.h"
#include "rowops.hip.h"
#include "retok.hip.h"
#include "lexical.hip.h"
#include "partition.hip.h"

using namespace zett;

namespace {

struct Tensor {
    float* f32 = nullptr;
    void* lo = nullptr;
    std::vector<int64_t> shape;
    size_t numel = 0;
};

inline size_t round_up(size_t v, size_t m) { return (v + m - 1) / m * m; }

}

struct zett_hypernet {
    zett_config cfg{};
    int device = 0;
    int precision = ZETT_PREC_BF16;
    bool finalized = false;
    std::map<std::string, Tensor> w;
    std::vector<void*> qkv_w;
    std::vector<float*> qkv_b;
    struct Folded { void* w = nullptr; float* c = nullptr; float* b = nullptr; };
    std::vector<Folded> fold_qkv, fold_up;
    Folded fold_head_in, fold_head_out;
    float* head_one = nullptr;
    float* head_zero = nullptr;
    int ln_fold = 1;
    float* head_scale = nullptr;
    float* head_shift = nullptr;
    std::vector<void*> owned;
    int64_t max_chunk_tokens = 0;
    int time_gemm = 0;
    int cls_only_last = 1;
    int pair_dedupe = 1;
    int residual_lo = 1;
    int concurrent_lanes = 0;
    hipStream_t lane_stream = nullptr;
    hipEvent_t lane_ev[4] = {nullptr, nullptr, nullptr, nullptr};
    int attention_fast = 1;
    int attention_pack = 1;
    int gemm_tail_split = 1;
    int gemm_tile_order = 0;
    int ln_rows8 = 1;
    int table_lo = 1;
    int gemm_group = 0;
    int gemm4d_min_k = 512;
    int gemm_variant = 0;
    struct PlanSlot {
        DevBuf i32, u8;
        int32_t* host = nullptr;
        size_t host_ints = 0;
        hipEvent_t done = nullptr;
        hipEvent_t released = nullptr;
        const int32_t* sfm = nullptr;
        int64_t n_rows = 0;
        int seq = 0;
        bool pair_plan = false;
        const int32_t* ext_id_slot = nullptr;
        bool pending = false;
    } plan[2];
    PlanSlot table_plan;
    struct ExtTable { const void* table = nullptr; const float* stats = nullptr; const int32_t* id_slot = nullptr; } ext;
    int plan_cur = 0;
    hipStream_t plan_stream = nullptr;
    hipEvent_t plan_fork = nullptr;
    DevBuf table, x0, yf, yt, big, pre, ctx, cf, ct, lnstats, lnparts;
    hipEvent_t out_ready[2] = {nullptr, nullptr};
    bool out_recorded = false;
    int range_accumulate = 0;
    int32_t* range_word = nullptr;
    int32_t* range_host = nullptr;
    DevBuf dest_word, dest_stage[2], dest_sink;
    int32_t* dest_host = nullptr;
    hipEvent_t dest_checked = nullptr;
    std::vector<hipEvent_t> ev;
    size_t ev_used = 0;
    std::vector<double> ev_flops;
    std::vector<std::array<int, 4>> ev_shape;
    std::vector<zett_gemm_record> gemm_log;
    zett_stats stats{};
};

namespace {

size_t elt_size(int precision) { return precision == ZETT_PREC_F32 ? 4 : 2; }

bool is_gemm_weight(const std::string& n) {
    static const char* suffixes[] = {"input_projection.0.weight", "dense1.weight", "dense2.weight",
                                     "query.weight", "key.weight", "value.weight", "dense.weight",
                                     "output_projection.1.weight", "output_projection_out.1.weight"};
    for (const char* s : suffixes) {
        const size_t ls = strlen(s);
        if (n.size() >= ls && n.compare(n.size() - ls, ls, s) == 0) return true;
    }
    return false;
}

void expected_shapes(const zett_config& c, std::map<std::string, std::vector<int64_t>>& s) {
    const int64_t H = c.hidden, I = c.intermediate;
    auto proj = [&](const std::string& p) {
        s[p + "dense1.weight"] = {I, H}; s[p + "dense1.bias"] = {I};
        s[p + "dense2.weight"] = {H, I}; s[p + "dense2.bias"] = {H};
        s[p + "ln.weight"] = {H}; s[p + "ln.bias"] = {H};
    };
    if (c.embed_lang) s["lang_embeddings.weight"] = {c.n_langs, H};
    s["model.embeddings.token_type_embeddings.weight"] = {1, H};
    s["model.embeddings.LayerNorm.weight"] = {H};
    s["model.embeddings.LayerNorm.bias"] = {H};
    s["model.embeddings.position_embeddings.weight"] = {c.max_positions, H};
    for (int l = 0; l < c.layers; ++l) {
        const std::string p = "model.encoder.layer." + std::to_string(l) + ".";
        for (const char* q : {"query", "key", "value"}) {
            s[p + "attention.self." + q + ".weight"] = {H, H};
            s[p + "attention.self." + q + ".bias"] = {H};
        }
        s[p + "attention.output.dense.weight"] = {H, H}; s[p + "attention.output.dense.bias"] = {H};
        s[p + "attention.output.LayerNorm.weight"] = {H}; s[p + "attention.output.LayerNorm.bias"] = {H};
        s[p + "intermediate.dense.weight"] = {I, H}; s[p + "intermediate.dense.bias"] = {I};
        s[p + "output.dense.weight"] = {H, I}; s[p + "output.dense.bias"] = {H};
        s[p + "output.LayerNorm.weight"] = {H}; s[p + "output.LayerNorm.bias"] = {H};
    }
    s["fallback_embeddings.weight"] = {c.n_extra, c.n_in_embd};
    s["input_projection.0.weight"] = {H, c.n_in_embd}; s["input_projection.0.bias"] = {H};
    proj("input_projection.1.");
    proj("output_projection.0.");
    const int64_t w0 = c.single_head ? c.n_in_embd : c.n_embd;
    s["output_projection.1.weight"] = {w0, H}; s["output_projection.1.bias"] = {w0};
    if (c.separate_out && !c.single_head) {
        proj("output_projection_out.0.");
        s["output_projection_out.1.weight"] = {c.n_embd, H}; s["output_projection_out.1.bias"] = {c.n_embd};
    }
    if (c.rescale) {
        s["in_scaler.w"] = {1, c.n_in_embd}; s["in_scaler.b"] = {1, c.n_in_embd};
        s["scaler.w"] = {1, c.n_embd}; s["scaler.b"] = {1, c.n_embd};
        if (c.separate_out) { s["out_scaler.w"] = {1, c.n_embd}; s["out_scaler.b"] = {1, c.n_embd}; }
    }
    if (c.predict_bias) { s["bias_projection.weight"] = {1, H}; s["bias_projection.bias"] = {1}; }
}

int validate_config(const zett_config& c, int precision) {
    if (c.n_embd <= 0 || c.hidden <= 0 || c.intermediate <= 0 || c.heads <= 0 || c.layers <= 0)
        return fail(ZETT_E_INVALID, "non-positive dimension in zett_config");
    if (c.n_in_embd != (c.separate_out ? 2 * c.n_embd : c.n_embd))
        return fail(ZETT_E_INVALID, "n_in_embd must be 2*n_embd iff separate_out");
    if (c.hidden % c.heads) return fail(ZETT_E_INVALID, "hidden %d not divisible by heads %d", c.hidden, c.heads);
    const int d = c.hidden / c.heads;
    if (d < 8 || d > 512 || (d & (d - 1))) return fail(ZETT_E_INVALID, "head_dim %d unsupported (need a power of two in [8,512])", d);
    const int kq = precision == ZETT_PREC_F32 ? 32 : 64;
    for (int k : {c.n_in_embd, c.hidden, c.intermediate})
        if (k % kq) return fail(ZETT_E_INVALID, "contraction width %d is not a multiple of %d", k, kq);
    if (c.n_embd % 4) return fail(ZETT_E_INVALID, "n_embd must be a multiple of 4");
    if (c.n_extra < 1) return fail(ZETT_E_INVALID, "n_extra must be >= 1 (reference allocates max(hn_n_extra_tokens,1))");
    if (c.pad_token_id < 0) return fail(ZETT_E_INVALID, "pad_token_id is required");
    if (c.embed_lang && c.n_langs <= 0) return fail(ZETT_E_INVALID, "hn_embed_lang_id needs n_langs");
    return 0;
}

struct WorkspaceSizes {
    int64_t chunk_tokens;
    size_t table, x0, f32_rows, lo_rows, big, stats;
    size_t total() const { return table + x0 + 3 * f32_rows + 3 * lo_rows + big + stats; }
};

static int64_t pair_keys(const zett_config& c, int seq) {
    return ((int64_t)c.original_vocab_size + c.n_extra + 1) * (int64_t)(seq + (c.embed_lang ? 1 : 0));
}

static size_t plan_i32_bytes(const zett_config& c, int64_t N, int seq) {
    const int64_t V = (int64_t)c.original_vocab_size + c.n_extra;
    const int64_t max_tok = N * (int64_t)(seq + (c.embed_lang ? 1 : 0));
    const int64_t K = pair_keys(c, seq);
    const size_t scan_scratch = 2 * ((size_t)std::max<int64_t>(std::max<int64_t>(N, V), K) / SCAN_CHUNK + 2) + 1;
    return ((size_t)N + (N + 1) + 3 + V + (V + 1) + V + 7 * (size_t)max_tok + 2 * (size_t)K + 2 + scan_scratch) * 4;
}

static int64_t chunk_token_cap(const zett_config& c, size_t es) {
    const size_t wide = (size_t)std::max(c.intermediate, 3 * c.hidden);
    const size_t per_token = (size_t)c.n_in_embd * es + 3 * (size_t)c.hidden * 4 + 3 * (size_t)c.hidden * es + wide * es + 24;
    return std::max<int64_t>(131072, (int64_t)(((size_t)12 << 30) / per_token));
}

static WorkspaceSizes workspace_sizes(const zett_config& c, size_t es, int seq, int64_t Ttot, int64_t D, int64_t cap) {
    const int lam = c.embed_lang ? 1 : 0;
    WorkspaceSizes w{};
    if (cap <= 0) cap = chunk_token_cap(c, es);
    w.chunk_tokens = std::max<int64_t>(std::min<int64_t>(cap, std::max<int64_t>(Ttot, D)), seq + lam);
    const size_t MC = (size_t)w.chunk_tokens, MCS = MC + 768;
    const size_t wide = (size_t)std::max(c.intermediate, 3 * c.hidden);
    w.table = (size_t)D * c.hidden * 4;
    w.x0 = MCS * c.n_in_embd * es;
    w.f32_rows = MCS * c.hidden * 4;
    w.lo_rows = MCS * c.hidden * es;
    w.big = MCS * wide * es;
    w.stats = 2 * MCS * 2 * sizeof(float);
    return w;
}

struct PlanLayout {
    PlanArrays p{};
    int32_t* scan_tmp = nullptr;
    bool pair_plan = false;
    int64_t PK = 0;
    size_t n_clear = 0;
};
static PlanLayout plan_layout(const zett_hypernet* h, const zett_hypernet::PlanSlot& s, int64_t N, int seq) {
    const zett_config& c = h->cfg;
    const int lam = c.embed_lang ? 1 : 0;
    const int V = c.original_vocab_size + c.n_extra;
    const int64_t max_tok = N * (int64_t)(seq + lam);
    PlanLayout L;
    PlanArrays& p = L.p;
    L.PK = pair_keys(c, seq);
    L.pair_plan = h->pair_dedupe && c.layers >= 2 && L.PK <= std::max<int64_t>(4 * max_tok, (int64_t)1 << 23) && L.PK < (int64_t)0x7fffffff;
    int32_t* base = s.i32.as<int32_t>();
    p.id_flag = base; base += V;
    if (L.pair_plan) { p.pair_flag = base; base += L.PK; }
    p.err = base; base += 1;
    L.n_clear = (size_t)(base - s.i32.as<int32_t>());
    p.row_count = base; base += N;
    p.row_offset = base; base += N + 1;
    p.counters = base; base += 3;
    p.id_slot = base; base += V + 1;
    p.id_list = base; base += V;
    p.tok_slot = base; base += max_tok;
    p.tok_pos = base; base += max_tok;
    p.tok_row = base; base += max_tok;
    p.n_pair_keys = L.pair_plan ? (int32_t)L.PK : 0;
    if (L.pair_plan) {
        p.tok_pkey = base; base += max_tok;
        p.tok_pair = base; base += max_tok;
        p.pair_tslot = base; base += max_tok;
        p.pair_pos = base; base += max_tok;
        p.pair_slot = base; base += L.PK + 1;
    }
    L.scan_tmp = base;
    p.row_uniform = s.u8.as<uint8_t>();
    p.tok_key = p.row_uniform + N;
    return L;
}

static int enqueue_plan(zett_hypernet* h, zett_hypernet::PlanSlot& s, const int32_t* sfm, int64_t N, int seq, hipStream_t st) {
    const zett_config& c = h->cfg;
    const int lam = c.embed_lang ? 1 : 0;
    const int V = c.original_vocab_size + c.n_extra;
    const int64_t max_tok = N * (int64_t)(seq + lam);
    if (int rc = s.i32.reserve(plan_i32_bytes(c, N, seq))) return rc;
    if (int rc = s.u8.reserve((size_t)N + (size_t)max_tok)) return rc;
    const size_t need_ints = (size_t)N + 1 + 3;
    if (s.host_ints < need_ints) {
        if (s.host) (void)hipHostFree(s.host);
        s.host = nullptr;
        HIP_TRY(hipHostMalloc((void**)&s.host, need_ints * 4, hipHostMallocDefault));
        s.host_ints = need_ints;
    }
    if (!s.done) HIP_TRY(hipEventCreateWithFlags(&s.done, hipEventDisableTiming));
    if (!s.released) HIP_TRY(hipEventCreateWithFlags(&s.released, hipEventDisableTiming));
    const PlanLayout L = plan_layout(h, s, N, seq);
    const PlanArrays& p = L.p;
    HIP_TRY(hipMemsetAsync(s.i32.p, 0, L.n_clear * 4, st));
    const int rb = (int)((N + 255) / 256);
    hipLaunchKernelGGL(plan_rows_kernel, dim3(rb), dim3(256), 0, st, sfm, N, seq, c.pad_token_id, lam, V, p);
    launch_exclusive_scan(p.row_count, p.row_offset, N, L.scan_tmp, st);
    launch_exclusive_scan(p.id_flag, p.id_slot, (int64_t)V, L.scan_tmp, st);
    {
        PlanArrays pt = p;
        if (h->ext.id_slot) pt.id_slot = const_cast<int32_t*>(h->ext.id_slot);
        hipLaunchKernelGGL(plan_tokens_kernel, dim3(rb), dim3(256), 0, st, sfm, N, seq, c.pad_token_id, lam, V, pt);
    }
    if (L.pair_plan) {
        launch_exclusive_scan(p.pair_flag, p.pair_slot, L.PK, L.scan_tmp, st);
        hipLaunchKernelGGL(plan_pairs_kernel, dim3((unsigned)((max_tok + 255) / 256)), dim3(256), 0, st, N, p);
    }
    hipLaunchKernelGGL(plan_idlist_kernel, dim3((V + 255) / 256), dim3(256), 0, st, V, p);
    HIP_TRY(hipGetLastError());
    HIP_TRY(hipMemcpyAsync(s.host, p.row_offset, ((size_t)N + 1 + 3) * 4, hipMemcpyDeviceToHost, st));
    HIP_TRY(hipEventRecord(s.done, st));
    s.sfm = sfm; s.n_rows = N; s.seq = seq; s.pair_plan = L.pair_plan; s.ext_id_slot = h->ext.id_slot;
    return 0;
}

template <typename T>
int do_forward(zett_hypernet* h, const int32_t* sfm, int64_t N, int seq, const void* src, int src_dtype, const zett_dest* dest,
               int64_t v_src, int lang_index, float* out_in, float* out_out, float* out_bias, hipStream_t st);
template <typename T>
int do_table_rows(zett_hypernet* h, const int32_t* id_list, int first, int count, const void* src, int src_dtype, void* table_out, float* stats_out, hipStream_t st);

}

extern "C" {

const char* zett_last_error(void) { return g_err.c_str(); }
int zett_abi_version(void) { return ZETT_ABI_VERSION; }

int zett_create(const zett_config* cfg, int device, int precision, zett_hypernet** out) {
    if (!cfg || !out) return fail(ZETT_E_INVALID, "null argument");
    if (precision != ZETT_PREC_BF16 && precision != ZETT_PREC_F32 && precision != ZETT_PREC_F16) return fail(ZETT_E_INVALID, "unknown precision %d", precision);
    if (int rc = validate_config(*cfg, precision)) return rc;
    int ndev = 0;
    HIP_TRY(hipGetDeviceCount(&ndev));
    if (device < 0 || device >= ndev) return fail(ZETT_E_INVALID, "device %d out of range (%d visible)", device, ndev);
    ZETT_ON_DEVICE(device);
    auto* h = new zett_hypernet();
    h->cfg = *cfg;
    h->device = device;
    h->precision = precision;
    if (hipMalloc((void**)&h->range_word, 64) != hipSuccess || hipHostMalloc((void**)&h->range_host, 64, hipHostMallocDefault) != hipSuccess ||
        hipMemset(h->range_word, 0, 64) != hipSuccess) {
        if (h->range_word) (void)hipFree(h->range_word);
        if (h->range_host) (void)hipHostFree(h->range_host);
        delete h;
        return fail(ZETT_E_HIP, "allocation of the range word failed");
    }
    *out = h;
    return 0;
}

int zett_destroy(zett_hypernet* h) {
    if (!h) return 0;
    ::zett::DeviceScope _scope(h->device);
    for (auto& kv : h->w) {
        if (kv.second.f32) (void)hipFree(kv.second.f32);
        if (kv.second.lo && kv.second.lo != (void*)kv.second.f32) (void)hipFree(kv.second.lo);
    }
    for (void* p : h->owned) (void)hipFree(p);
    for (DevBuf* b : {&h->table, &h->x0, &h->yf, &h->yt, &h->big, &h->pre, &h->ctx, &h->cf, &h->ct, &h->lnstats, &h->lnparts, &h->dest_word, &h->dest_stage[0], &h->dest_stage[1], &h->dest_sink})
        b->release();
    for (zett_hypernet::PlanSlot* psp : {&h->plan[0], &h->plan[1], &h->table_plan}) {
        zett_hypernet::PlanSlot& ps = *psp;
        ps.i32.release(); ps.u8.release();
        if (ps.host) (void)hipHostFree(ps.host);
        if (ps.done) (void)hipEventDestroy(ps.done);
        if (ps.released) (void)hipEventDestroy(ps.released);
    }
    if (h->plan_stream) (void)hipStreamDestroy(h->plan_stream);
    if (h->plan_fork) (void)hipEventDestroy(h->plan_fork);
    if (h->range_word) (void)hipFree(h->range_word);
    if (h->range_host) (void)hipHostFree(h->range_host);
    if (h->dest_host) (void)hipHostFree(h->dest_host);
    if (h->dest_checked) (void)hipEventDestroy(h->dest_checked);
    for (hipEvent_t e : h->out_ready) if (e) (void)hipEventDestroy(e);
    for (hipEvent_t e : h->lane_ev) if (e) (void)hipEventDestroy(e);
    if (h->lane_stream) (void)hipStreamDestroy(h->lane_stream);
    for (hipEvent_t e : h->ev) (void)hipEventDestroy(e);
    delete h;
    return 0;
}

int zett_load_weight(zett_hypernet* h, const char* name, const void* data, int dtype, const int64_t* shape, int ndim) {
    if (!h || !name || !data || !shape || ndim < 1) return fail(ZETT_E_INVALID, "null argument");
    if (h->finalized) return fail(ZETT_E_STATE, "weights are frozen after zett_finalize");
    std::map<std::string, std::vector<int64_t>> exp;
    expected_shapes(h->cfg, exp);
    const std::string n(name);
    auto it = exp.find(n);
    if (it == exp.end()) return 0;
    std::vector<int64_t> got(shape, shape + ndim);
    if (got != it->second) {
        std::string a, b;
        for (auto v : got) a += std::to_string(v) + ",";
        for (auto v : it->second) b += std::to_string(v) + ",";
        return fail(ZETT_E_INVALID, "%s: shape [%s] does not match the config's [%s]", name, a.c_str(), b.c_str());
    }
    ZETT_ON_DEVICE(h->device);
    size_t numel = 1;
    for (auto v : got) numel *= (size_t)v;
    Tensor& t = h->w[n];
    if (t.f32) { (void)hipFree(t.f32); t.f32 = nullptr; }
    t.shape = got;
    t.numel = numel;
    HIP_TRY(hipMalloc((void**)&t.f32, numel * 4));
    if (dtype == ZETT_F32) {
        HIP_TRY(hipMemcpy(t.f32, data, numel * 4, hipMemcpyDefault));
    } else if (dtype == ZETT_F16 || dtype == ZETT_BF16) {
        void* stage = nullptr;
        HIP_TRY(hipMalloc(&stage, numel * 2));
        hipError_t e = hipMemcpy(stage, data, numel * 2, hipMemcpyDefault);
        if (e == hipSuccess) {
            const int blocks = (int)std::min<size_t>((numel + 255) / 256, 65535);
            if (dtype == ZETT_F16) hipLaunchKernelGGL(convert_to_f32_kernel<1>, dim3(blocks), dim3(256), 0, 0, stage, t.f32, numel);
            else hipLaunchKernelGGL(convert_to_f32_kernel<2>, dim3(blocks), dim3(256), 0, 0, stage, t.f32, numel);
            e = hipDeviceSynchronize();
        }
        (void)hipFree(stage);
        if (e != hipSuccess) return fail(ZETT_E_HIP, "upload of %s failed: %s", name, hipGetErrorString(e));
    } else {
        return fail(ZETT_E_INVALID, "unknown dtype %d", dtype);
    }
    return 0;
}

int zett_finalize(zett_hypernet* h) {
    if (!h) return fail(ZETT_E_INVALID, "null handle");
    if (h->finalized) return 0;
    ZETT_ON_DEVICE(h->device);
    std::map<std::string, std::vector<int64_t>> exp;
    expected_shapes(h->cfg, exp);
    for (auto& kv : exp)
        if (!h->w.count(kv.first)) return fail(ZETT_E_STATE, "missing weight: %s", kv.first.c_str());
    const zett_config& c = h->cfg;
    const size_t es = elt_size(h->precision);
    for (auto& kv : h->w) {
        Tensor& t = kv.second;
        if (!is_gemm_weight(kv.first)) continue;
        if (h->precision == ZETT_PREC_F32) { t.lo = t.f32; continue; }
        HIP_TRY(hipMalloc(&t.lo, t.numel * 2));
        const int blocks = (int)std::min<size_t>((t.numel / 4 + 255) / 256 + 1, 65535);
        if (h->precision == ZETT_PREC_F16)
            hipLaunchKernelGGL(convert_f32_to_lo_kernel<f16_t>, dim3(blocks), dim3(256), 0, 0, t.f32, (f16_t*)t.lo, t.numel, h->range_word);
        else
            hipLaunchKernelGGL(convert_f32_to_lo_kernel<bf16_t>, dim3(blocks), dim3(256), 0, 0, t.f32, (bf16_t*)t.lo, t.numel, h->range_word);
    }
    HIP_TRY(hipDeviceSynchronize());
    const size_t H = c.hidden;
    for (int l = 0; l < c.layers; ++l) {
        const std::string p = "model.encoder.layer." + std::to_string(l) + ".attention.self.";
        void* wq = nullptr; float* bq = nullptr;
        HIP_TRY(hipMalloc(&wq, 3 * H * H * es));
        HIP_TRY(hipMalloc((void**)&bq, 3 * H * 4));
        h->owned.push_back(wq); h->owned.push_back(bq);
        int k = 0;
        for (const char* q : {"query", "key", "value"}) {
            Tensor& tw = h->w[p + q + ".weight"];
            Tensor& tb = h->w[p + q + ".bias"];
            HIP_TRY(hipMemcpy((char*)wq + (size_t)k * H * H * es, tw.lo, H * H * es, hipMemcpyDeviceToDevice));
            HIP_TRY(hipMemcpy(bq + (size_t)k * H, tb.f32, H * 4, hipMemcpyDeviceToDevice));
            ++k;
        }
        h->qkv_w.push_back(wq);
        h->qkv_b.push_back(bq);
    }
    if (h->precision != ZETT_PREC_F32 && c.hidden % 128 == 0) {
        auto fold = [&](const float* w32, size_t N, size_t K, const float* gamma, const float* beta, const float* bias,
                        zett_hypernet::Folded& f) -> int {
            HIP_TRY(hipMalloc(&f.w, N * K * es));
            HIP_TRY(hipMalloc((void**)&f.c, N * 4));
            HIP_TRY(hipMalloc((void**)&f.b, N * 4));
            h->owned.push_back(f.w); h->owned.push_back(f.c); h->owned.push_back(f.b);
            if (h->precision == ZETT_PREC_F16)
                hipLaunchKernelGGL(fold_weight_kernel<f16_t>, dim3((unsigned)N), dim3(256), 0, 0, w32, (int)K, gamma, beta, bias, (f16_t*)f.w, f.c, f.b, h->range_word);
            else
                hipLaunchKernelGGL(fold_weight_kernel<bf16_t>, dim3((unsigned)N), dim3(256), 0, 0, w32, (int)K, gamma, beta, bias, (bf16_t*)f.w, f.c, f.b, h->range_word);
            return 0;
        };
        h->fold_qkv.resize(c.layers); h->fold_up.resize(c.layers);
        float* tmp = nullptr;
        HIP_TRY(hipMalloc((void**)&tmp, 3 * H * H * 4));
        for (int l = 0; l < c.layers; ++l) {
            const std::string lp = "model.encoder.layer." + std::to_string(l) + ".";
            if (int rc = fold(h->w[lp + "intermediate.dense.weight"].f32, c.intermediate, H, h->w[lp + "attention.output.LayerNorm.weight"].f32,
                              h->w[lp + "attention.output.LayerNorm.bias"].f32, h->w[lp + "intermediate.dense.bias"].f32, h->fold_up[l])) return rc;
            if (l == 0) continue;
            const std::string pp = "model.encoder.layer." + std::to_string(l - 1) + ".output.LayerNorm.";
            int k = 0;
            for (const char* q : {"query", "key", "value"}) {
                HIP_TRY(hipMemcpy(tmp + (size_t)k * H * H, h->w[lp + "attention.self." + q + ".weight"].f32, H * H * 4, hipMemcpyDeviceToDevice));
                ++k;
            }
            if (int rc = fold(tmp, 3 * H, H, h->w[pp + "weight"].f32, h->w[pp + "bias"].f32, h->qkv_b[l], h->fold_qkv[l])) return rc;
        }
        if (!(c.single_head && c.separate_out)) {
            const size_t w0 = c.single_head ? c.n_in_embd : c.n_embd;
            if (int rc = fold(h->w["output_projection.1.weight"].f32, w0, H, h->w["output_projection.0.ln.weight"].f32,
                              h->w["output_projection.0.ln.bias"].f32, h->w["output_projection.1.bias"].f32, h->fold_head_in)) return rc;
            if (c.separate_out && !c.single_head)
                if (int rc = fold(h->w["output_projection_out.1.weight"].f32, c.n_embd, H, h->w["output_projection_out.0.ln.weight"].f32,
                                  h->w["output_projection_out.0.ln.bias"].f32, h->w["output_projection_out.1.bias"].f32, h->fold_head_out)) return rc;
            std::vector<float> ones(w0, 1.0f), zeros(w0, 0.0f);
            HIP_TRY(hipMalloc((void**)&h->head_one, w0 * 4));
            HIP_TRY(hipMalloc((void**)&h->head_zero, w0 * 4));
            h->owned.push_back(h->head_one); h->owned.push_back(h->head_zero);
            HIP_TRY(hipMemcpy(h->head_one, ones.data(), w0 * 4, hipMemcpyHostToDevice));
            HIP_TRY(hipMemcpy(h->head_zero, zeros.data(), w0 * 4, hipMemcpyHostToDevice));
        }
        HIP_TRY(hipDeviceSynchronize());
        (void)hipFree(tmp);
    }
    HIP_TRY(hipMemcpy(h->range_host, h->range_word, 4, hipMemcpyDeviceToHost));
    if (h->range_host[0] & ZETT_RANGE_WEIGHT)
        return fail(ZETT_E_RANGE, "a GEMM weight (or a LayerNorm-folded weight W*gamma) exceeds the half range (|w| > 65504 or not finite): "
                                  "this checkpoint needs ZETT_PREC_BF16 or ZETT_PREC_F32");
    if (c.rescale) {
        const size_t w0 = c.single_head ? c.n_in_embd : c.n_embd;
        HIP_TRY(hipMalloc((void**)&h->head_scale, w0 * 4));
        HIP_TRY(hipMalloc((void**)&h->head_shift, w0 * 4));
        h->owned.push_back(h->head_scale); h->owned.push_back(h->head_shift);
        HIP_TRY(hipMemcpy(h->head_scale, h->w["scaler.w"].f32, c.n_embd * 4, hipMemcpyDeviceToDevice));
        HIP_TRY(hipMemcpy(h->head_shift, h->w["scaler.b"].f32, c.n_embd * 4, hipMemcpyDeviceToDevice));
        if (c.single_head && c.separate_out) {
            HIP_TRY(hipMemcpy(h->head_scale + c.n_embd, h->w["out_scaler.w"].f32, c.n_embd * 4, hipMemcpyDeviceToDevice));
            HIP_TRY(hipMemcpy(h->head_shift + c.n_embd, h->w["out_scaler.b"].f32, c.n_embd * 4, hipMemcpyDeviceToDevice));
        }
    }
    if (h->precision != ZETT_PREC_F32) {
        for (auto& kv : h->w) {
            Tensor& t = kv.second;
            if (is_gemm_weight(kv.first) && t.f32) { (void)hipFree(t.f32); t.f32 = nullptr; }
        }
    }
    h->finalized = true;
    return 0;
}

int zett_set_option(zett_hypernet* h, const char* key, int64_t value) {
    if (!h || !key) return fail(ZETT_E_INVALID, "null argument");
    const std::string k(key);
    if (k == "max_chunk_tokens") {
        if (value < 1024) return fail(ZETT_E_INVALID, "max_chunk_tokens must be >= 1024");
        h->max_chunk_tokens = value;
    } else if (k == "time_gemm") {
        h->time_gemm = value != 0;
    } else if (k == "cls_only_last_layer") {
        h->cls_only_last = value != 0;
    } else if (k == "pair_dedupe") {
        h->pair_dedupe = value != 0;
    } else if (k == "residual_lo") {
        if (value < 0 || value > 2) return fail(ZETT_E_INVALID, "residual_lo must be 0 (fp32 residual stream), 1 (16-bit stream in f16 mode) or 2 (in bf16 mode too)");
        h->residual_lo = (int)value;
    } else if (k == "concurrent_lanes") {
        if (value < 0 || value > 2) return fail(ZETT_E_INVALID, "concurrent_lanes must be 0 (never), 1 (auto) or 2 (whenever a call is one chunk of >= 512 rows)");
        h->concurrent_lanes = (int)value;
    } else if (k == "attention_fast") {
        h->attention_fast = value != 0;
    } else if (k == "ln_fold") {
        if (value < 0 || value > 2) return fail(ZETT_E_INVALID, "ln_fold must be 0 (off), 1 (encoder and output heads) or 2 (encoder only: A/B)");
        h->ln_fold = (int)value;
    } else if (k == "gemm_tail_split") {
        if (value < 0 || value > 3) return fail(ZETT_E_INVALID, "gemm_tail_split must be 0 (never), 1 (auto), 2 (cut every gemm4d launch in the middle) or 3 (128x256 tiles only)");
        h->gemm_tail_split = (int)value;
    } else if (k == "attention_pack") {
        h->attention_pack = value != 0;
    } else if (k == "ln_rows8") {
        h->ln_rows8 = value != 0;
    } else if (k == "table_lo") {
        h->table_lo = value != 0;
    } else if (k == "gemm_group") {
        if (value < 0 || value > 64) return fail(ZETT_E_INVALID, "gemm_group must be 0 (default: 4) .. 64");
        h->gemm_group = (int)value;
    } else if (k == "gemm_tile_order") {
        if (value < 0 || value > 1) return fail(ZETT_E_INVALID, "gemm_tile_order must be 0 or 1");
        h->gemm_tile_order = (int)value;
    } else if (k == "gemm4d_min_k") {
        if (value < 64) return fail(ZETT_E_INVALID, "gemm4d_min_k must be >= 64");
        h->gemm4d_min_k = (int)value;
    } else if (k == "range_accumulate") {
        h->range_accumulate = value != 0;
    } else if (k == "gemm_variant") {
        if (value != 0 && value != 1 && value != 2 && value != 3 && value != 7 && value != 8)
            return fail(ZETT_E_INVALID, "gemm_variant must be 0 (auto), 1 (128x128), 2 (256x256 register-staged), 3 (384x256), 7 (256x256 four-wave direct-to-LDS) or 8 (7 with the generic epilogue drain)");
        h->gemm_variant = (int)value;
    } else {
        return fail(ZETT_E_INVALID, "unknown option %s", key);
    }
    return 0;
}

int zett_workspace_bytes(const zett_hypernet* h, int64_t n_rows, int32_t seq, int64_t* out_bytes) {
    if (!h || !out_bytes) return fail(ZETT_E_INVALID, "null argument");
    if (n_rows < 0 || seq < 1) return fail(ZETT_E_INVALID, "bad surface-form shape [%lld, %d]", (long long)n_rows, seq);
    const zett_config& c = h->cfg;
    const int64_t V = (int64_t)c.original_vocab_size + c.n_extra;
    const int64_t max_tok = n_rows * (int64_t)(seq + (c.embed_lang ? 1 : 0));
    const WorkspaceSizes w = workspace_sizes(c, elt_size(h->precision), seq, max_tok, std::min<int64_t>(V, max_tok), h->max_chunk_tokens);
    const size_t parts = c.hidden % 128 == 0 ? (size_t)(c.hidden / 128) * ((size_t)w.chunk_tokens + 768) * 8 : 0;
    *out_bytes = (int64_t)(w.total() + parts + plan_i32_bytes(c, n_rows, seq) + (size_t)n_rows + (size_t)max_tok);
    return 0;
}

int zett_get_stats(const zett_hypernet* h, zett_stats* out) {
    if (!h || !out) return fail(ZETT_E_INVALID, "null argument");
    *out = h->stats;
    return 0;
}

int zett_stream_wait_output(zett_hypernet* h, int which, void* stream) {
    if (!h) return fail(ZETT_E_INVALID, "null handle");
    if (which != ZETT_OUT_IN && which != ZETT_OUT_BIAS) return fail(ZETT_E_INVALID, "which must be ZETT_OUT_IN or ZETT_OUT_BIAS");
    if (!h->out_recorded) return fail(ZETT_E_STATE, "no forward has run on this handle");
    ZETT_ON_DEVICE(h->device);
    HIP_TRY(hipStreamWaitEvent((hipStream_t)stream, h->out_ready[which], 0));
    return 0;
}

int zett_get_gemm_log(const zett_hypernet* h, zett_gemm_record* out, int64_t capacity, int64_t* count) {
    if (!h || !count || capacity < 0 || (capacity > 0 && !out)) return fail(ZETT_E_INVALID, "null argument");
    *count = (int64_t)h->gemm_log.size();
    for (int64_t i = 0; i < capacity && i < *count; ++i) out[i] = h->gemm_log[(size_t)i];
    return 0;
}

int zett_check_range(zett_hypernet* h, void* stream, int32_t* flags) {
    if (!h) return fail(ZETT_E_INVALID, "null handle");
    ZETT_ON_DEVICE(h->device);
    hipStream_t st = (hipStream_t)stream;
    HIP_TRY(hipMemcpyAsync(h->range_host, h->range_word, 4, hipMemcpyDeviceToHost, st));
    HIP_TRY(hipStreamSynchronize(st));
    const int32_t w = h->range_host[0];
    if (h->range_accumulate && w) HIP_TRY(hipMemsetAsync(h->range_word, 0, 4, st));
    if (flags) *flags = w;
    if (!w) return 0;
    return fail(ZETT_E_RANGE, "the last forward left the range of its arithmetic:%s%s%s%s (precision %s)",
                (w & ZETT_RANGE_SOURCE) ? " in_scaler(source_embeddings) beyond the half range;" : "",
                (w & ZETT_RANGE_ACTIVATION) ? " a 16-bit activation (Q/K/V, FFN intermediate or the operand copy of the residual sum) beyond the half range;" : "",
                (w & ZETT_RANGE_OUTPUT) ? " non-finite predicted embeddings;" : "",
                (w & ZETT_RANGE_DEST) ? " a finite value beyond the range of an f16 destination (stored as inf);" : "",
                h->precision == ZETT_PREC_F16 ? "f16: re-run with ZETT_PREC_BF16" : h->precision == ZETT_PREC_BF16 ? "bf16" : "f32");
}

int zett_partition_workspace_bytes(int64_t n_rows, int32_t n_ids, int64_t* out_bytes) {
    if (!out_bytes || n_rows < 0 || n_ids < 1) return fail(ZETT_E_INVALID, "bad argument");
    *out_bytes = (int64_t)partition_workspace_bytes(n_rows, n_ids);
    return 0;
}

int zett_partition_rows(const int32_t* surface_forms, int64_t n_rows, int32_t seq, int32_t pad_id, int32_t n_ids, int32_t world,
                        const int32_t* caps, int32_t* perm_out, void* workspace, int64_t workspace_bytes, int32_t device, void* stream) {
    if (n_rows < 0 || seq < 1 || n_ids < 1) return fail(ZETT_E_INVALID, "bad surface-form shape [%lld, %d] / id range %d", (long long)n_rows, seq, n_ids);
    if (world < 1 || world > PART_MAX_RANKS) return fail(ZETT_E_INVALID, "zett_partition_rows handles 1..%d ranks (one node), got %d", PART_MAX_RANKS, world);
    if (n_rows == 0) return 0;
    if (!surface_forms || !caps || !perm_out || !workspace) return fail(ZETT_E_INVALID, "null argument");
    if (n_rows >= (int64_t)0x7fffffff) return fail(ZETT_E_INVALID, "too many rows for one call");
    int64_t total = 0;
    for (int r = 0; r < world; ++r) { if (caps[r] < 0) return fail(ZETT_E_INVALID, "negative capacity"); total += caps[r]; }
    if (total != n_rows) return fail(ZETT_E_INVALID, "the ranks' capacities sum to %lld, the matrix has %lld rows", (long long)total, (long long)n_rows);
    if ((size_t)workspace_bytes < partition_workspace_bytes(n_rows, n_ids)) return fail(ZETT_E_INVALID, "workspace too small (zett_partition_workspace_bytes)");
    ZETT_ON_DEVICE(device);
    hipStream_t st = (hipStream_t)stream;
    const size_t have_bytes = ((size_t)(n_ids + 3) / 4) * 4 + 64;
    uint32_t* have = (uint32_t*)workspace;
    PartCaps caps_arg = {};
    for (int r = 0; r < world; ++r) caps_arg.v[r] = caps[r];
    HIP_TRY(hipMemsetAsync(have, 0, have_bytes, st));
    const size_t lds_have = ((size_t)(n_ids + 3) / 4) * 4;
    if (lds_have <= 150 * 1024) {
        static bool attr_set[64] = {};
        if (device >= 64 || !attr_set[device]) {
            HIP_TRY(hipFuncSetAttribute((const void*)partition_rows_kernel<true>, hipFuncAttributeMaxDynamicSharedMemorySize, 150 * 1024));
            if (device < 64) attr_set[device] = true;
        }
        hipLaunchKernelGGL(partition_rows_kernel<true>, dim3(1), dim3(PART_THREADS), lds_have, st, surface_forms, n_rows, (int)seq, (int)pad_id, (int)n_ids,
                           (int)world, caps_arg, have, perm_out);
    } else {
        hipLaunchKernelGGL(partition_rows_kernel<false>, dim3(1), dim3(PART_THREADS), 0, st, surface_forms, n_rows, (int)seq, (int)pad_id, (int)n_ids,
                           (int)world, caps_arg, have, perm_out);
    }
    HIP_TRY(hipGetLastError());
    return 0;
}

int zett_scatter_rows(const void* src, void* dst, const int64_t* order, int64_t n_rows, int64_t row_bytes, int32_t device, void* stream) {
    if (n_rows < 0 || row_bytes < 1) return fail(ZETT_E_INVALID, "bad shape");
    if (n_rows == 0) return 0;
    if (!src || !dst || !order) return fail(ZETT_E_INVALID, "null argument");
    if (row_bytes != 4 && row_bytes % 16 != 0) return fail(ZETT_E_INVALID, "row_bytes must be 4 or a multiple of 16, got %lld", (long long)row_bytes);
    if (((uintptr_t)src | (uintptr_t)dst) % (row_bytes == 4 ? 4 : 16)) return fail(ZETT_E_INVALID, "misaligned buffer");
    ZETT_ON_DEVICE(device);
    hipStream_t st = (hipStream_t)stream;
    if (row_bytes == 4)
        hipLaunchKernelGGL(scatter_words_kernel, dim3((unsigned)((n_rows + 255) / 256)), dim3(256), 0, st, (const uint32_t*)src, (uint32_t*)dst, order, n_rows);
    else
        hipLaunchKernelGGL(scatter_rows_kernel, dim3((unsigned)std::min<int64_t>(n_rows, 65535 * 16)), dim3(256), 0, st, (const unsigned char*)src, (unsigned char*)dst,
                           order, n_rows, row_bytes);
    HIP_TRY(hipGetLastError());
    return 0;
}

int zett_forward_prepare(zett_hypernet* h, const int32_t* surface_forms, int64_t n_rows, int32_t seq, void* input_stream) {
    if (!h) return fail(ZETT_E_INVALID, "null handle");
    if (!h->finalized) return fail(ZETT_E_STATE, "zett_finalize has not been called");
    const zett_config& c = h->cfg;
    if (n_rows < 0 || seq < 1) return fail(ZETT_E_INVALID, "bad surface-form shape [%lld, %d]", (long long)n_rows, seq);
    if (n_rows == 0) return 0;
    if (!surface_forms) return fail(ZETT_E_INVALID, "null tensor argument");
    if (n_rows * (int64_t)(seq + 1) >= (int64_t)0x7fffffff) return fail(ZETT_E_INVALID, "too many positions for one call");
    (void)c;
    ZETT_ON_DEVICE(h->device);
    if (!h->plan_stream) {
        int least = 0, greatest = 0;
        HIP_TRY(hipDeviceGetStreamPriorityRange(&least, &greatest));
        HIP_TRY(hipStreamCreateWithPriority(&h->plan_stream, hipStreamNonBlocking, greatest));
    }
    if (!h->plan_fork) HIP_TRY(hipEventCreateWithFlags(&h->plan_fork, hipEventDisableTiming));
    zett_hypernet::PlanSlot& ps = h->plan[h->plan_cur ^ 1];
    if (ps.pending) HIP_TRY(hipEventSynchronize(ps.done));
    HIP_TRY(hipEventRecord(h->plan_fork, (hipStream_t)input_stream));
    HIP_TRY(hipStreamWaitEvent(h->plan_stream, h->plan_fork, 0));
    if (ps.released) HIP_TRY(hipStreamWaitEvent(h->plan_stream, ps.released, 0));
    if (int rc = enqueue_plan(h, ps, surface_forms, n_rows, seq, h->plan_stream)) return rc;
    ps.pending = true;
    return 0;
}

}

namespace {

int check_dest(const zett_hypernet* h, const zett_dest* d, int64_t n_rows) {
    const zett_config& c = h->cfg;
    if (!d) return fail(ZETT_E_INVALID, "null destination");
    if (!d->in) return fail(ZETT_E_INVALID, "the destination's `in` matrix is null");
    if (c.separate_out != (d->out != nullptr))
        return fail(ZETT_E_INVALID, c.separate_out ? "the destination's `out` matrix is required when separate_out_embeddings is set"
                                                   : "the destination's `out` must be null: this config has no second output");
    if (d->dtype < ZETT_F32 || d->dtype > ZETT_BF16) return fail(ZETT_E_INVALID, "unknown destination dtype %d", d->dtype);
    if (d->bias && (d->bias_dtype < ZETT_F32 || d->bias_dtype > ZETT_BF16)) return fail(ZETT_E_INVALID, "unknown bias destination dtype %d", d->bias_dtype);
    if (d->ld_in < c.n_embd || (d->out && d->ld_out < c.n_embd))
        return fail(ZETT_E_INVALID, "destination leading dimension (%lld, %lld) below n_embd %d", (long long)d->ld_in, (long long)d->ld_out, c.n_embd);
    if (d->n_dest_rows < 0 || (!d->rows && d->n_dest_rows < n_rows))
        return fail(ZETT_E_INVALID, "the destination has %lld rows, the identity map needs %lld", (long long)d->n_dest_rows, (long long)n_rows);
    return 0;
}

int forward_entry(zett_hypernet* h, const int32_t* surface_forms, int64_t n_rows, int32_t seq, const void* source_embeddings, int src_dtype,
                  int64_t v_src, int32_t lang_index, const zett_dest* dest, float* out_in, float* out_out, float* out_bias, void* stream) {
    if (!h) return fail(ZETT_E_INVALID, "null handle");
    if (!h->finalized) return fail(ZETT_E_STATE, "zett_finalize has not been called");
    const zett_config& c = h->cfg;
    if (n_rows < 0 || seq < 1) return fail(ZETT_E_INVALID, "bad surface-form shape [%lld, %d]", (long long)n_rows, seq);
    if (seq + (c.embed_lang ? 1 : 0) > c.max_positions) return fail(ZETT_E_INDEX, "sequence %d exceeds position_embeddings (%d rows)", seq, c.max_positions);
    if (n_rows == 0) {
        h->stats = zett_stats{};
        ZETT_ON_DEVICE(h->device);
        if (!h->range_accumulate) HIP_TRY(hipMemsetAsync(h->range_word, 0, 4, (hipStream_t)stream));
        for (hipEvent_t& e : h->out_ready) {
            if (!e) HIP_TRY(hipEventCreateWithFlags(&e, hipEventDisableTiming));
            HIP_TRY(hipEventRecord(e, (hipStream_t)stream));
        }
        h->out_recorded = true;
        return 0;
    }
    if (!surface_forms || !source_embeddings || (!dest && (!out_in || !out_bias))) return fail(ZETT_E_INVALID, "null tensor argument");
    const bool has_out = c.separate_out;
    if (!dest && has_out && !out_out) return fail(ZETT_E_INVALID, "out_out is required when separate_out_embeddings is set");
    if (src_dtype < ZETT_F32 || src_dtype > ZETT_BF16) return fail(ZETT_E_INVALID, "unknown source dtype %d", src_dtype);
    if (v_src < c.original_vocab_size) return fail(ZETT_E_INDEX, "source_embeddings has %lld rows, config.original_vocab_size is %d", (long long)v_src, c.original_vocab_size);
    if (c.embed_lang && (lang_index < 0 || lang_index >= c.n_langs)) return fail(ZETT_E_INDEX, "lang_index %d outside [0,%d)", lang_index, c.n_langs);
    if (n_rows * (int64_t)(seq + 1) >= (int64_t)0x7fffffff) return fail(ZETT_E_INVALID, "too many positions for one call");
    ZETT_ON_DEVICE(h->device);
    hipStream_t st = (hipStream_t)stream;
    if (h->precision == ZETT_PREC_F16)
        return do_forward<f16_t>(h, surface_forms, n_rows, seq, source_embeddings, src_dtype, dest, v_src, lang_index, out_in, out_out, out_bias, st);
    if (h->precision == ZETT_PREC_BF16)
        return do_forward<bf16_t>(h, surface_forms, n_rows, seq, source_embeddings, src_dtype, dest, v_src, lang_index, out_in, out_out, out_bias, st);
    return do_forward<float>(h, surface_forms, n_rows, seq, source_embeddings, src_dtype, dest, v_src, lang_index, out_in, out_out, out_bias, st);
}

}

extern "C" {

int zett_forward(zett_hypernet* h, const int32_t* surface_forms, int64_t n_rows, int32_t seq,
                 const void* source_embeddings, int src_dtype, int64_t v_src, int32_t lang_index,
                 float* out_in, float* out_out, float* out_bias, void* stream) {
    return forward_entry(h, surface_forms, n_rows, seq, source_embeddings, src_dtype, v_src, lang_index, nullptr, out_in, out_out, out_bias, stream);
}

int zett_forward_into(zett_hypernet* h, const int32_t* surface_forms, int64_t n_rows, int32_t seq, const void* source_embeddings, int src_dtype,
                      int64_t v_src, int32_t lang_index, const zett_dest* dest, void* stream) {
    if (!h) return fail(ZETT_E_INVALID, "null handle");
    if (int rc = check_dest(h, dest, n_rows)) return rc;
    return forward_entry(h, surface_forms, n_rows, seq, source_embeddings, src_dtype, v_src, lang_index, dest, nullptr, nullptr, nullptr, stream);
}

int zett_table_plan(zett_hypernet* h, const int32_t* surface_forms, int64_t n_rows, int32_t seq, int32_t* id_slot_out, int32_t* id_list_out,
                    int64_t* n_ids_out, void* stream) {
    if (!h) return fail(ZETT_E_INVALID, "null handle");
    if (!h->finalized) return fail(ZETT_E_STATE, "zett_finalize has not been called");
    if (!surface_forms || !id_slot_out || !id_list_out || !n_ids_out) return fail(ZETT_E_INVALID, "null argument");
    if (n_rows < 1 || seq < 1) return fail(ZETT_E_INVALID, "bad surface-form shape [%lld, %d]", (long long)n_rows, seq);
    if (n_rows * (int64_t)(seq + 1) >= (int64_t)0x7fffffff) return fail(ZETT_E_INVALID, "too many positions for one call");
    const zett_config& c = h->cfg;
    const int V = c.original_vocab_size + c.n_extra;
    ZETT_ON_DEVICE(h->device);
    hipStream_t st = (hipStream_t)stream;
    zett_hypernet::PlanSlot& ps = h->table_plan;
    const zett_hypernet::ExtTable saved = h->ext;
    h->ext = zett_hypernet::ExtTable{};
    const int rc = enqueue_plan(h, ps, surface_forms, n_rows, seq, st);
    h->ext = saved;
    if (rc) return rc;
    HIP_TRY(hipEventSynchronize(ps.done));
    const int32_t* hoff = ps.host;
    if (hoff[n_rows + 2] != 0)
        return fail(ZETT_E_INDEX, "surface-form row %d holds an id outside [0, %d) (original_vocab_size %d + %d fallback rows)",
                    hoff[n_rows + 2] - 1, V, c.original_vocab_size, c.n_extra);
    const int D = hoff[n_rows + 1];
    const PlanLayout L = plan_layout(h, ps, n_rows, seq);
    HIP_TRY(hipMemcpyAsync(id_slot_out, L.p.id_slot, ((size_t)V + 1) * 4, hipMemcpyDeviceToDevice, st));
    if (D > 0) HIP_TRY(hipMemcpyAsync(id_list_out, L.p.id_list, (size_t)D * 4, hipMemcpyDeviceToDevice, st));
    *n_ids_out = D;
    return 0;
}

int zett_table_rows(zett_hypernet* h, const int32_t* id_list, int64_t first, int64_t count, const void* source_embeddings, int src_dtype,
                    int64_t v_src, void* table_out, float* stats_out, void* stream) {
    if (!h) return fail(ZETT_E_INVALID, "null handle");
    if (!h->finalized) return fail(ZETT_E_STATE, "zett_finalize has not been called");
    if (first < 0 || count < 0 || first + count >= (int64_t)0x7fffffff) return fail(ZETT_E_INVALID, "bad table range [%lld, +%lld)", (long long)first, (long long)count);
    if (count == 0) return 0;
    if (!id_list || !source_embeddings || !table_out || !stats_out) return fail(ZETT_E_INVALID, "null tensor argument");
    if (src_dtype < ZETT_F32 || src_dtype > ZETT_BF16) return fail(ZETT_E_INVALID, "unknown source dtype %d", src_dtype);
    if (v_src < h->cfg.original_vocab_size) return fail(ZETT_E_INDEX, "source_embeddings has %lld rows, config.original_vocab_size is %d", (long long)v_src, h->cfg.original_vocab_size);
    ZETT_ON_DEVICE(h->device);
    hipStream_t st = (hipStream_t)stream;
    if (h->precision == ZETT_PREC_F16) return do_table_rows<f16_t>(h, id_list, (int)first, (int)count, source_embeddings, src_dtype, table_out, stats_out, st);
    if (h->precision == ZETT_PREC_BF16) return do_table_rows<bf16_t>(h, id_list, (int)first, (int)count, source_embeddings, src_dtype, table_out, stats_out, st);
    return fail(ZETT_E_INVALID, "zett_table_rows: the folded 16-bit table exists in the 16-bit modes only");
}

}

namespace {
int forward_table_entry(zett_hypernet* h, const int32_t* surface_forms, int64_t n_rows, int32_t seq, const void* table, const float* table_stats,
                        const int32_t* id_slot, int32_t lang_index, const zett_dest* dest, float* out_in, float* out_out, float* out_bias, void* stream) {
    if (!h) return fail(ZETT_E_INVALID, "null handle");
    if (!h->finalized) return fail(ZETT_E_STATE, "zett_finalize has not been called");
    const zett_config& c = h->cfg;
    if (n_rows < 1 || seq < 1) return fail(ZETT_E_INVALID, "bad surface-form shape [%lld, %d]", (long long)n_rows, seq);
    if (seq + (c.embed_lang ? 1 : 0) > c.max_positions) return fail(ZETT_E_INDEX, "sequence %d exceeds position_embeddings (%d rows)", seq, c.max_positions);
    if (!surface_forms || !table || !table_stats || !id_slot || (!dest && (!out_in || !out_bias))) return fail(ZETT_E_INVALID, "null tensor argument");
    if (!dest && c.separate_out && !out_out) return fail(ZETT_E_INVALID, "out_out is required when separate_out_embeddings is set");
    if (c.embed_lang && (lang_index < 0 || lang_index >= c.n_langs)) return fail(ZETT_E_INDEX, "lang_index %d outside [0,%d)", lang_index, c.n_langs);
    if (n_rows * (int64_t)(seq + 1) >= (int64_t)0x7fffffff) return fail(ZETT_E_INVALID, "too many positions for one call");
    if (h->precision == ZETT_PREC_F32) return fail(ZETT_E_INVALID, "zett_forward_table: the folded 16-bit table exists in the 16-bit modes only");
    ZETT_ON_DEVICE(h->device);
    hipStream_t st = (hipStream_t)stream;
    h->ext.table = table; h->ext.stats = table_stats; h->ext.id_slot = id_slot;
    int rc;
    if (h->precision == ZETT_PREC_F16)
        rc = do_forward<f16_t>(h, surface_forms, n_rows, seq, nullptr, ZETT_F32, dest, 0, lang_index, out_in, out_out, out_bias, st);
    else
        rc = do_forward<bf16_t>(h, surface_forms, n_rows, seq, nullptr, ZETT_F32, dest, 0, lang_index, out_in, out_out, out_bias, st);
    h->ext = zett_hypernet::ExtTable{};
    return rc;
}

}

extern "C" {

int zett_forward_table(zett_hypernet* h, const int32_t* surface_forms, int64_t n_rows, int32_t seq, const void* table, const float* table_stats,
                       const int32_t* id_slot, int32_t lang_index, float* out_in, float* out_out, float* out_bias, void* stream) {
    return forward_table_entry(h, surface_forms, n_rows, seq, table, table_stats, id_slot, lang_index, nullptr, out_in, out_out, out_bias, stream);
}

int zett_forward_table_into(zett_hypernet* h, const int32_t* surface_forms, int64_t n_rows, int32_t seq, const void* table, const float* table_stats,
                            const int32_t* id_slot, int32_t lang_index, const zett_dest* dest, void* stream) {
    if (!h) return fail(ZETT_E_INVALID, "null handle");
    if (int rc = check_dest(h, dest, n_rows)) return rc;
    return forward_table_entry(h, surface_forms, n_rows, seq, table, table_stats, id_slot, lang_index, dest, nullptr, nullptr, nullptr, stream);
}

}

namespace {

template <typename T>
struct Runner {
    zett_hypernet* h;
    hipStream_t st;
    int rc = 0;

    const Tensor& W(const std::string& n) { return h->w.at(n); }
    const T* Wlo(const std::string& n) { return (const T*)h->w.at(n).lo; }
    const float* Wf(const std::string& n) { return h->w.at(n).f32; }

    GemmEpilogue<T> epi() {
        GemmEpilogue<T> e{};
        e.split_col = 0x7fffffff;
        e.range_flag = h->range_word;
        return e;
    }

    long a_rows_readable = 0;
    bool staged_dst = false;
    int stage_lane = 0;

    int variant_for(int M, int N, int K, const GemmEpilogue<T>& e) const {
    constexpr bool is_f32 = std::is_same<T, float>::value;
    int variant = h->gemm_variant;
    if (variant == 0) {
        variant = (M > 128 && N > 128) ? 2 : 1;
        if (variant != 1 && N % 256 == 0 && !e.scale && !e.residual) {
            const long t256 = (long)((M + 255) / 256) * (N / 256), t384 = (long)((M + 383) / 384) * (N / 256);
            const double c256 = (double)((t256 + 255) / 256), c384 = 1.7 * (double)((t384 + 255) / 256);
            if (c384 < c256) variant = 3;
        }
    }
    if (variant == 3 && (N % 256 != 0 || (long)((M + 383) / 384) * 384 > a_rows_readable || e.scale || e.shift || e.residual || e.range_final)) variant = 2;
    if (h->gemm_variant == 0 && variant == 2 && !is_f32 && K >= h->gemm4d_min_k) variant = 7;
    if ((variant == 7 || variant == 8) && is_f32) variant = 2;
    const bool wide_ok = N % 8 == 0 && (!e.out_lo || e.ld_lo % 8 == 0) && e.ld_f32 % 4 == 0 && (!e.residual || e.ld_res % 4 == 0) &&
                         (e.split_col >= N || e.split_col % 8 == 0);
    if (variant != 1 && !wide_ok) variant = 1;
    if (e.residual && (e.scale || e.shift)) variant = 1;
    if (e.stats_part || e.fold_stats) variant = 7;
        return variant;
    }


    void gemm(const T* A, int lda, const T* Wp, int ldw, int M, int N, int K, const GemmEpilogue<T>& e) {
        if (rc || M <= 0) return;
        GemmArgs<T> g{A, lda, Wp, ldw, M, N, K, e};
        g.tile_order = h->gemm_tile_order;
        g.group = h->gemm_group;
        g.row0 = h->gemm_tail_split == 1 ? -1 : h->gemm_tail_split == 2 ? ((M / 2 + 255) / 256) * 256 : h->gemm_tail_split == 3 ? -2 : 0;
        const double fl = 2.0 * (double)M * (double)N * (double)K;
        hipEvent_t e0 = nullptr, e1 = nullptr;
        if (h->time_gemm) {
            while (h->ev.size() < h->ev_used + 2) {
                hipEvent_t ev;
                if (hipEventCreate(&ev) != hipSuccess) { rc = fail(ZETT_E_HIP, "hipEventCreate failed"); return; }
                h->ev.push_back(ev);
            }
            e0 = h->ev[h->ev_used++];
            e1 = h->ev[h->ev_used++];
            h->ev_flops.push_back(fl);
            h->ev_shape.push_back({M, N, K, 0});
            (void)hipEventRecord(e0, st);
        }
        const int variant = variant_for(M, N, K, e);
        if (h->time_gemm && !h->ev_shape.empty()) h->ev_shape.back()[3] = variant;
        {
            zett_gemm_record r{};
            r.m = M; r.n = N; r.k = K; r.variant = variant;
            r.epilogue = (e.out_lo ? 1 : 0) | ((e.out_f32 || e.out_f32_b) ? 2 : 0) | (e.residual ? 4 : 0) | ((e.scale || e.shift) ? 8 : 0) |
                         (e.stats_part ? 16 : 0) | (e.fold_stats ? 32 : 0) | (e.residual_lo ? 64 : 0) | (e.act << 8) |
                         (e.dst ? 1024 : 0) | (staged_dst ? 2048 : 0);
            r.flops = fl;
            const double mn = (double)M * (double)N;
            const double dst_es = e.dst_dtype == ZETT_F32 ? 4.0 : 2.0;
            r.bytes = ((double)M + (double)N) * (double)K * sizeof(T) + (e.out_lo ? mn * sizeof(T) : 0.0) + ((e.out_f32 || e.out_f32_b) ? mn * 4.0 : 0.0) +
                      (e.dst ? mn * dst_es : 0.0) +
                      (e.residual ? mn * 4.0 : 0.0) + (e.residual_lo ? mn * sizeof(T) : 0.0) + (e.stats_part ? (double)M * (N / 128) * 8.0 : 0.0) + ((e.fold_stats || e.res_stats) ? (double)M * 8.0 : 0.0);
            h->gemm_log.push_back(r);
        }
        const hipError_t err = launch_gemm_variant(variant, g, st);
        if (h->time_gemm) (void)hipEventRecord(e1, st);
        if (err != hipSuccess) { rc = fail(ZETT_E_HIP, "gemm launch failed: %s", hipGetErrorString(err)); return; }
        h->stats.executed_flops += fl;
        h->stats.gemm_launches += 1;
    }

    struct DestOut { void* p; const int64_t* rows; int64_t ld; int dtype; };

    void head_gemm(const T* A, const T* Wp, int M, int N, int K, const GemmEpilogue<T>& e, const DestOut* d, const DestOut* d_b, int split) {
        if (rc || M <= 0) return;
        if (!d) { gemm(A, K, Wp, K, M, N, K, e); return; }
        GemmEpilogue<T> ed = e;
        ed.out_f32 = nullptr; ed.out_f32_b = nullptr; ed.ld_f32 = N;
        ed.dst = d->p; ed.dst_rows = d->rows; ed.ld_dst = d->ld; ed.dst_dtype = d->dtype;
        const GemmArgs<T> probe{A, K, Wp, K, M, N, K, ed};
        if (!d_b && variant_for(M, N, K, ed) == 7 && gemm_4d_dst_mode(probe) >= 0) { gemm(A, K, Wp, K, M, N, K, ed); return; }
        DevBuf& stage_buf = h->dest_stage[stage_lane];
        if (int r = stage_buf.reserve((size_t)M * (size_t)N * sizeof(float))) { rc = r; return; }
        float* S = stage_buf.as<float>();
        GemmEpilogue<T> es = e;
        es.out_f32 = S; es.ld_f32 = N;
        if (d_b) es.out_f32_b = S + split;
        staged_dst = true;
        gemm(A, K, Wp, K, M, N, K, es);
        staged_dst = false;
        dest_store(S, N, *d, M, d_b ? split : N);
        if (d_b) dest_store(S + split, N, *d_b, M, N - split);
    }

    void dest_store(const float* S, int64_t ld_s, const DestOut& d, int rows, int cols) {
        if (rc || rows <= 0) return;
        const bool vec = cols % 4 == 0 && ld_s % 4 == 0 && d.ld % 4 == 0 && (uintptr_t)S % 16 == 0 && (uintptr_t)d.p % (d.dtype == ZETT_F32 ? 16 : 8) == 0;
        const dim3 grid((unsigned)std::min<int64_t>(rows, 65535 * 16));
#define ZETT_DEST_STORE(OT) do { if (vec) hipLaunchKernelGGL((dest_store_rows_kernel<OT, true>), grid, dim3(256), 0, st, S, ld_s, (OT*)d.p, d.ld, d.rows, (int64_t)rows, cols, h->range_word); \
                                 else hipLaunchKernelGGL((dest_store_rows_kernel<OT, false>), grid, dim3(256), 0, st, S, ld_s, (OT*)d.p, d.ld, d.rows, (int64_t)rows, cols, h->range_word); } while (0)
        if (d.dtype == ZETT_F16) ZETT_DEST_STORE(f16_t);
        else if (d.dtype == ZETT_BF16) ZETT_DEST_STORE(bf16_t);
        else ZETT_DEST_STORE(float);
#undef ZETT_DEST_STORE
        check("dest_store");
    }

    template <typename BT>
    void readout_dst(const float* in, int rows, const float* gamma, const float* beta, float eps, float* of, T* ol, const LnReadout& readout) {
        const int H = h->cfg.hidden;
        if constexpr (sizeof(T) == 2) {
            const int tpr8 = h->ln_rows8 ? ln_rows8_tpr(H) : 0;
            if (tpr8) {
                const dim3 grid8((rows + 256 / tpr8 - 1) / (256 / tpr8));
                if (tpr8 == 32) hipLaunchKernelGGL((layernorm_rows8_kernel<T, false, 32, true, BT>), grid8, dim3(256), 0, st, in, H, rows, H, gamma, beta, eps, of, ol, (float*)nullptr, (float*)nullptr, LnEmbed{}, 0, readout);
                else hipLaunchKernelGGL((layernorm_rows8_kernel<T, false, 64, true, BT>), grid8, dim3(256), 0, st, in, H, rows, H, gamma, beta, eps, of, ol, (float*)nullptr, (float*)nullptr, LnEmbed{}, 0, readout);
                check("readout");
                return;
            }
        }
        if (H <= 2048) hipLaunchKernelGGL((layernorm_rows_kernel<T, false, 64, true, BT>), dim3((rows + 3) / 4), dim3(256), 0, st, in, H, rows, H, gamma, beta, eps, of, ol, (float*)nullptr, (float*)nullptr, LnEmbed{}, 0, readout);
        else hipLaunchKernelGGL((layernorm_rows_kernel<T, false, 256, true, BT>), dim3(rows), dim3(256), 0, st, in, H, rows, H, gamma, beta, eps, of, ol, (float*)nullptr, (float*)nullptr, LnEmbed{}, 0, readout);
        check("readout");
    }

    void check(const char* what) {
        if (rc) return;
        hipError_t e = hipGetLastError();
        if (e != hipSuccess) rc = fail(ZETT_E_HIP, "%s launch failed: %s", what, hipGetErrorString(e));
    }

    void layernorm(const float* in, int rows, const float* gamma, const float* beta, float eps, float* of, T* ol, float* stats = nullptr,
                   LnReadout readout = LnReadout{}, const T* in_lo = nullptr, int bias_dtype = -1) {
        if (rc || rows <= 0) return;
        readout.in_lo = in_lo;
        if (bias_dtype >= 0 && readout.out_bias) {
            if (bias_dtype == ZETT_F16) readout_dst<f16_t>(in, rows, gamma, beta, eps, of, ol, readout);
            else if (bias_dtype == ZETT_BF16) readout_dst<bf16_t>(in, rows, gamma, beta, eps, of, ol, readout);
            else readout_dst<float>(in, rows, gamma, beta, eps, of, ol, readout);
            return;
        }
        const int H = h->cfg.hidden;
        if constexpr (sizeof(T) == 2) {
            const int tpr8 = h->ln_rows8 ? ln_rows8_tpr(H) : 0;
            if (tpr8) {
                const dim3 grid8((rows + 256 / tpr8 - 1) / (256 / tpr8));
#define ZETT_LN8_LAUNCH(TPR, RO) hipLaunchKernelGGL((layernorm_rows8_kernel<T, false, TPR, RO>), grid8, dim3(256), 0, st, in, H, rows, H, gamma, beta, eps, of, ol, stats, (float*)nullptr, LnEmbed{}, 0, readout)
                if (readout.out_bias) { if (tpr8 == 32) ZETT_LN8_LAUNCH(32, true); else ZETT_LN8_LAUNCH(64, true); }
                else { if (tpr8 == 32) ZETT_LN8_LAUNCH(32, false); else ZETT_LN8_LAUNCH(64, false); }
#undef ZETT_LN8_LAUNCH
                check("layernorm");
                return;
            }
        }
        const dim3 grid = H <= 2048 ? dim3((rows + 3) / 4) : dim3(rows);
#define ZETT_LN_LAUNCH(TPR, RO) hipLaunchKernelGGL((layernorm_rows_kernel<T, false, TPR, RO>), grid, dim3(256), 0, st, in, H, rows, H, gamma, beta, eps, of, ol, stats, (float*)nullptr, LnEmbed{}, 0, readout)
        if (readout.out_bias) { if (H <= 2048) ZETT_LN_LAUNCH(64, true); else ZETT_LN_LAUNCH(256, true); }
        else { if (H <= 2048) ZETT_LN_LAUNCH(64, false); else ZETT_LN_LAUNCH(256, false); }
#undef ZETT_LN_LAUNCH
        check("layernorm");
    }

    void ln_stats(const float2* parts, int ld_part, int rows, float eps, float* stats) {
        if (rc || rows <= 0) return;
        hipLaunchKernelGGL(ln_stats_kernel, dim3((rows + 63) / 64), dim3(64), 0, st, parts, h->cfg.hidden / 128, ld_part, rows,
                           h->cfg.hidden, eps, stats);
        check("ln_stats");
    }

    void projector(const std::string& p, const T* x_lo, const float* x_f32, int rows, T* big, float* pre, float* of, T* ol,
                   float2* fold_parts = nullptr, int ld_part = 0, float* fold_stats = nullptr) {
        const zett_config& c = h->cfg;
        GemmEpilogue<T> e1 = epi();
        e1.bias = Wf(p + "dense1.bias"); e1.act = ACT_GELU_TANH; e1.out_lo = big; e1.ld_lo = c.intermediate;
        gemm(x_lo, c.hidden, Wlo(p + "dense1.weight"), c.hidden, rows, c.intermediate, c.hidden, e1);
        GemmEpilogue<T> e2 = epi();
        e2.bias = Wf(p + "dense2.bias"); e2.act = ACT_GELU_TANH; e2.residual = x_f32; e2.ld_res = c.hidden;
        e2.ld_f32 = c.hidden;
        if (fold_parts) { e2.out_lo = ol; e2.ld_lo = c.hidden; e2.stats_part = fold_parts; e2.ld_part = ld_part; }
        else e2.out_f32 = pre;
        gemm(big, c.intermediate, Wlo(p + "dense2.weight"), c.intermediate, rows, c.hidden, c.intermediate, e2);
        if (fold_parts) ln_stats(fold_parts, ld_part, rows, c.ln_eps_projector, fold_stats);
        else layernorm(pre, rows, Wf(p + "ln.weight"), Wf(p + "ln.bias"), c.ln_eps_projector, of, ol);
    }
};

template <typename T, int SD>
void launch_gather(hipStream_t st, const int32_t* id_list, int s0, int m, const void* src, const zett_config& c,
                   const float* fallback, const float* sw, const float* sb, T* out, int32_t* range_flag) {
    hipLaunchKernelGGL((gather_src_kernel<T, SD>), dim3(m), dim3(256), 0, st, id_list, s0, m, src, c.n_in_embd,
                       c.original_vocab_size, fallback, sw, sb, out, range_flag);
}

template <typename T>
void table_phase(Runner<T>& R, const int32_t* id_list, int first, int count, const void* src, int src_dtype, int64_t MC, size_t MCS,
                 T* X0, float* Zf, T* Zt, T* BIG, float* PRE, float2* PARTS, bool table_lo, T* tbl16, float* tblst, float* tbl32) {
    zett_hypernet* h = R.h;
    const zett_config& c = h->cfg;
    const int H = c.hidden, EIN = c.n_in_embd;
    hipStream_t st = R.st;
    const float* in_w = c.rescale ? R.Wf("in_scaler.w") : nullptr;
    const float* in_b = c.rescale ? R.Wf("in_scaler.b") : nullptr;
    for (int s0 = first; s0 < first + count && !R.rc; s0 += (int)MC) {
        const int m = (int)std::min<int64_t>(MC, first + count - s0);
        const float* fb = R.Wf("fallback_embeddings.weight");
        if (src_dtype == ZETT_F32) launch_gather<T, 0>(st, id_list, s0, m, src, c, fb, in_w, in_b, X0, h->range_word);
        else if (src_dtype == ZETT_F16) launch_gather<T, 1>(st, id_list, s0, m, src, c, fb, in_w, in_b, X0, h->range_word);
        else launch_gather<T, 2>(st, id_list, s0, m, src, c, fb, in_w, in_b, X0, h->range_word);
        R.check("gather_src");
        GemmEpilogue<T> e0 = R.epi();
        e0.bias = R.Wf("input_projection.0.bias"); e0.out_f32 = Zf; e0.ld_f32 = H; e0.out_lo = Zt; e0.ld_lo = H;
        R.gemm(X0, EIN, R.Wlo("input_projection.0.weight"), EIN, m, H, EIN, e0);
        if (table_lo) R.projector("input_projection.1.", Zt, Zf, m, BIG, PRE, nullptr, tbl16 + (size_t)s0 * H, PARTS, (int)MCS, tblst + 2 * (size_t)s0);
        else R.projector("input_projection.1.", Zt, Zf, m, BIG, PRE, tbl32 + (size_t)s0 * H, nullptr);
    }
}

template <typename T>
bool folded_table_mode(const zett_hypernet* h) {
    const zett_config& c = h->cfg;
    const int H = c.hidden;
    const bool fold = h->ln_fold && !std::is_same<T, float>::value && h->gemm_variant == 0 && H % 128 == 0 && H >= 512 && (int)h->fold_up.size() == c.layers;
    const bool lo_stream = fold && c.layers >= 1 && sizeof(T) == 2 && (h->residual_lo == 2 || (h->residual_lo == 1 && std::is_same<T, f16_t>::value));
    return lo_stream && h->table_lo != 0;
}

template <typename T>
int do_table_rows(zett_hypernet* h, const int32_t* id_list, int first, int count, const void* src, int src_dtype, void* table_out, float* stats_out, hipStream_t st) {
    const zett_config& c = h->cfg;
    if (!folded_table_mode<T>(h))
        return fail(ZETT_E_INVALID, "zett_table_rows needs the folded 16-bit table: f16 arithmetic with the LayerNorm fold, the 16-bit residual stream and table_lo on");
    const WorkspaceSizes ws = workspace_sizes(c, sizeof(T), 1, count, count, h->max_chunk_tokens);
    const int64_t MC = ws.chunk_tokens;
    const size_t MCS = (size_t)MC + 768;
    if (int rc = h->x0.reserve(ws.x0)) return rc;
    if (int rc = h->yf.reserve(ws.f32_rows)) return rc;
    if (int rc = h->yt.reserve(ws.lo_rows)) return rc;
    if (int rc = h->big.reserve(ws.big)) return rc;
    if (int rc = h->pre.reserve(ws.f32_rows)) return rc;
    if (int rc = h->lnparts.reserve((size_t)(c.hidden / 128) * MCS * sizeof(float2))) return rc;
    Runner<T> R{h, st};
    R.a_rows_readable = (long)MCS;
    struct NoTiming { zett_hypernet* h; int saved; ~NoTiming() { h->time_gemm = saved; } } no_timing{h, h->time_gemm};
    h->time_gemm = 0;
    table_phase<T>(R, id_list, first, count, src, src_dtype, MC, MCS, h->x0.as<T>(), h->yf.as<float>(), h->yt.as<T>(), h->big.as<T>(), h->pre.as<float>(),
                   h->lnparts.as<float2>(), true, (T*)table_out, stats_out, nullptr);
    return R.rc;
}

template <typename T>
int do_forward(zett_hypernet* h, const int32_t* sfm, int64_t N, int seq, const void* src, int src_dtype, const zett_dest* dest,
               int64_t v_src, int lang_index, float* out_in, float* out_out, float* out_bias, hipStream_t st) {
    (void)v_src;
    const zett_config& c = h->cfg;
    const int H = c.hidden, I = c.intermediate, E = c.n_embd, EIN = c.n_in_embd;
    const int lam = c.embed_lang ? 1 : 0;
    const int V = c.original_vocab_size + c.n_extra;
    const int64_t max_tok = N * (int64_t)(seq + lam);
    h->stats = zett_stats{};
    h->stats.rows = N;
    h->ev_used = 0;
    h->ev_flops.clear();
    h->ev_shape.clear();
    h->gemm_log.clear();

    zett_hypernet::PlanSlot& ps = h->plan[h->plan_cur ^ 1];
    if (ps.pending && ps.sfm == sfm && ps.n_rows == N && ps.seq == seq && ps.pair_plan == plan_layout(h, ps, N, seq).pair_plan &&
        ps.ext_id_slot == h->ext.id_slot) {
        HIP_TRY(hipStreamWaitEvent(st, ps.done, 0));
    } else {
        if (ps.pending) HIP_TRY(hipEventSynchronize(ps.done));
        if (ps.released) HIP_TRY(hipStreamWaitEvent(st, ps.released, 0));
        if (int rc = enqueue_plan(h, ps, sfm, N, seq, st)) return rc;
    }
    ps.pending = false;
    h->plan_cur ^= 1;
    struct SlotGuard {
        zett_hypernet* h; zett_hypernet::PlanSlot* ps; hipStream_t st; bool lane_forked = false;
        ~SlotGuard() {
            if (lane_forked && h->lane_stream && h->lane_ev[3]) {
                (void)hipEventRecord(h->lane_ev[3], h->lane_stream);
                (void)hipStreamWaitEvent(st, h->lane_ev[3], 0);
            }
            if (ps->released) (void)hipEventRecord(ps->released, st);
        }
    } slot_guard{h, &ps, st};
    const PlanLayout PL = plan_layout(h, ps, N, seq);
    const PlanArrays& p = PL.p;
    const bool pair_plan = PL.pair_plan;
    if (!h->range_accumulate) HIP_TRY(hipMemsetAsync(h->range_word, 0, 4, st));
    for (hipEvent_t& e : h->out_ready)
        if (!e) HIP_TRY(hipEventCreateWithFlags(&e, hipEventDisableTiming));
    const bool dest_check = dest && dest->rows;
    if (dest_check) {
        if (int rc = h->dest_word.reserve(4)) return rc;
        if (!h->dest_host) HIP_TRY(hipHostMalloc((void**)&h->dest_host, 4, hipHostMallocDefault));
        if (!h->dest_checked) HIP_TRY(hipEventCreateWithFlags(&h->dest_checked, hipEventDisableTiming));
        HIP_TRY(hipMemsetAsync(h->dest_word.p, 0, 4, st));
        hipLaunchKernelGGL(dest_rows_check_kernel, dim3((unsigned)((N + 255) / 256)), dim3(256), 0, st, dest->rows, N, dest->n_dest_rows, h->dest_word.as<int32_t>());
        HIP_TRY(hipGetLastError());
        HIP_TRY(hipMemcpyAsync(h->dest_host, h->dest_word.p, 4, hipMemcpyDeviceToHost, st));
        HIP_TRY(hipEventRecord(h->dest_checked, st));
    }
    HIP_TRY(hipEventSynchronize(ps.done));
    int32_t* hoff = ps.host;
    if (hoff[N + 2] != 0)
        return fail(ZETT_E_INDEX, "surface-form row %d holds an id outside [0, %d) (original_vocab_size %d + %d fallback rows)",
                    hoff[N + 2] - 1, V, c.original_vocab_size, c.n_extra);
    if (dest_check) {
        HIP_TRY(hipEventSynchronize(h->dest_checked));
        if (h->dest_host[0] != 0)
            return fail(ZETT_E_INDEX, "destination row map: rows[%d] is outside the destination's %lld rows", h->dest_host[0] - 1, (long long)dest->n_dest_rows);
    }
    const int64_t Ttot = hoff[N];
    const int D = hoff[N + 1];
    h->stats.packed_tokens = Ttot;
    h->stats.distinct_ids = D;
    h->stats.distinct_positions = Ttot;

    const WorkspaceSizes ws = workspace_sizes(c, sizeof(T), seq, Ttot, D, h->max_chunk_tokens);
    const int64_t MC = ws.chunk_tokens;
    const size_t MCS = (size_t)MC + 768;
    if (int rc = h->table.reserve(ws.table)) return rc;
    if (int rc = h->x0.reserve(ws.x0)) return rc;
    if (int rc = h->yf.reserve(ws.f32_rows)) return rc;
    if (int rc = h->yt.reserve(ws.lo_rows)) return rc;
    if (int rc = h->big.reserve(ws.big)) return rc;
    if (int rc = h->pre.reserve(ws.f32_rows)) return rc;
    if (int rc = h->ctx.reserve(ws.lo_rows)) return rc;
    if (int rc = h->cf.reserve(ws.f32_rows)) return rc;
    if (int rc = h->ct.reserve(ws.lo_rows)) return rc;
    if (int rc = h->lnstats.reserve(ws.stats)) return rc;
    const bool fold = h->ln_fold && !std::is_same<T, float>::value && h->gemm_variant == 0 && H % 128 == 0 && H >= 512 &&
                      (int)h->fold_up.size() == c.layers;
    const bool lo_stream = fold && c.layers >= 1 && sizeof(T) == 2 &&
                           (h->residual_lo == 2 || (h->residual_lo == 1 && std::is_same<T, f16_t>::value));
    const size_t ws_parts = fold ? (size_t)(H / 128) * MCS * sizeof(float2) : 0;
    if (int rc = h->lnparts.reserve(ws_parts)) return rc;
    float2* PARTS = h->lnparts.as<float2>();
    float* TBL = h->table.as<float>();
    const bool table_lo = lo_stream && h->table_lo != 0;
    const bool ext_table = h->ext.table != nullptr;
    if (ext_table && !table_lo)
        return fail(ZETT_E_INVALID, "zett_forward_table needs the folded 16-bit table: f16 arithmetic with the LayerNorm fold, the 16-bit residual stream and table_lo on");
    T* TBL16 = ext_table ? (T*)const_cast<void*>(h->ext.table) : (T*)h->table.as<float>();
    float* TBLST = ext_table ? const_cast<float*>(h->ext.stats) : (float*)((char*)h->table.as<float>() + (((size_t)D * H * sizeof(T) + 15) / 16) * 16);
    T* X0 = h->x0.as<T>();
    float* Zf = h->yf.as<float>();
    T* Zt = h->yt.as<T>();
    T* BIG = h->big.as<T>();
    float* PRE = h->pre.as<float>();
    T* CTX = h->ctx.as<T>();
    float* Cf = h->cf.as<float>();
    T* Ct = h->ct.as<T>();
    float* STa = h->lnstats.as<float>();
    float* STb = STa + 2 * MCS;

    Runner<T> R{h, st};
    R.a_rows_readable = (long)MCS;

    if (!ext_table)
        table_phase<T>(R, p.id_list, 0, D, src, src_dtype, MC, MCS, X0, Zf, Zt, BIG, PRE, PARTS, table_lo, TBL16, TBLST, TBL);
    if (R.rc) return R.rc;

    const float* lang_vec = lam ? R.Wf("lang_embeddings.weight") + (size_t)lang_index * H : nullptr;
    const float scaling = 1.0f / std::sqrt((float)(H / c.heads));
    struct Lane { hipStream_t st; size_t off; };
    auto dest_out = [&](void* base, int64_t ld, int64_t r0) {
        const size_t es = dest->dtype == ZETT_F32 ? 4 : 2;
        return typename Runner<T>::DestOut{dest->rows ? base : (void*)((char*)base + (size_t)r0 * (size_t)ld * es), dest->rows ? dest->rows + r0 : nullptr, ld, dest->dtype};
    };
    const size_t ld_parts = MCS;
    auto run_chunk = [&](int64_t r0, int64_t r1, const Lane& lane, int ev_mode) -> int {
        const int rows = (int)(r1 - r0);
        const int tok0 = hoff[r0];
        const int m = hoff[r1] - tok0;
        h->stats.chunks += 1;
        hipStream_t st = lane.st;
        R.st = lane.st;
        R.stage_lane = ev_mode == 2 ? 1 : 0;
        R.a_rows_readable = (long)(MCS - lane.off);
        float* const Zf = h->yf.as<float>() + lane.off * H;
        T* const Zt = h->yt.as<T>() + lane.off * H;
        T* const BIG = h->big.as<T>() + lane.off * (size_t)std::max(I, 3 * H);
        float* const PRE = h->pre.as<float>() + lane.off * H;
        T* const CTX = h->ctx.as<T>() + lane.off * H;
        float* const Cf = h->cf.as<float>() + lane.off * H;
        T* const Ct = h->ct.as<T>() + lane.off * H;
        float* const STa = h->lnstats.as<float>() + 2 * lane.off;
        float* const STb = STa + 2 * MCS;
        float2* const PARTS = h->lnparts.as<float2>() + lane.off;

        LnEmbed emb{TBL, p.tok_slot, p.tok_pos, R.Wf("model.embeddings.token_type_embeddings.weight"),
                    R.Wf("model.embeddings.position_embeddings.weight"), lang_vec, seq, p.tok_row, p.row_offset, r0, rows,
                    table_lo ? (const void*)TBL16 : nullptr, TBLST, R.Wf("input_projection.1.ln.weight"), R.Wf("input_projection.1.ln.bias")};
        float* hs_sum = Zf;
        float* hs_stats = STb;
        const float* hs_gamma = R.Wf("model.embeddings.LayerNorm.weight");
        const float* hs_beta = R.Wf("model.embeddings.LayerNorm.bias");
        auto embed_ln = [&](const LnEmbed& e, int n, int t0, T* lo, float* stats, float* sum) {
            if constexpr (sizeof(T) == 2) {
                const int tpr8 = h->ln_rows8 ? ln_rows8_tpr(H) : 0;
                if (tpr8) {
                    const dim3 grid8((n + 256 / tpr8 - 1) / (256 / tpr8));
                    if (tpr8 == 32)
                        hipLaunchKernelGGL((layernorm_rows8_kernel<T, true, 32, false>), grid8, dim3(256), 0, st, (const float*)nullptr, H, n, H,
                                           hs_gamma, hs_beta, c.ln_eps_encoder, (float*)nullptr, lo, stats, sum, e, t0, LnReadout{});
                    else
                        hipLaunchKernelGGL((layernorm_rows8_kernel<T, true, 64, false>), grid8, dim3(256), 0, st, (const float*)nullptr, H, n, H,
                                           hs_gamma, hs_beta, c.ln_eps_encoder, (float*)nullptr, lo, stats, sum, e, t0, LnReadout{});
                    R.check("embed_layernorm");
                    return;
                }
            }
            if (H <= 2048)
                hipLaunchKernelGGL((layernorm_rows_kernel<T, true, 64>), dim3((n + 3) / 4), dim3(256), 0, st, (const float*)nullptr, H, n, H,
                                   hs_gamma, hs_beta, c.ln_eps_encoder, (float*)nullptr, lo, stats, sum, e, t0, LnReadout{});
            else
                hipLaunchKernelGGL((layernorm_rows_kernel<T, true, 256>), dim3(n), dim3(256), 0, st, (const float*)nullptr, H, n, H,
                                   hs_gamma, hs_beta, c.ln_eps_encoder, (float*)nullptr, lo, stats, sum, e, t0, LnReadout{});
            R.check("embed_layernorm");
        };
        const int P = pair_plan ? hoff[N + 3] : 0;
        const bool pairs = pair_plan && rows == N && P > 0 && (int64_t)P * 100 <= (int64_t)m * 85;
        int32_t* brow_pair = p.tok_pkey;
        if (pairs) {
            LnEmbed pe = emb;
            pe.tok_slot = p.pair_tslot; pe.tok_pos = p.pair_pos; pe.tok_row = nullptr;
            embed_ln(pe, P, 0, Zt, hs_stats, lo_stream ? (float*)nullptr : hs_sum);
            hipLaunchKernelGGL(pair_rows_kernel, dim3((m + 255) / 256), dim3(256), 0, st, m, tok0, r0, rows, p, brow_pair);
            R.check("pair_rows");
            h->stats.distinct_positions = P;
        } else {
            embed_ln(emb, m, tok0, Zt, hs_stats, lo_stream ? (float*)nullptr : hs_sum);
        }

        int zrows = m;
        bool raw = false;
        auto other = [&](float* b) { return b == Zf ? PRE : Zf; };
        auto other_stats = [&](float* b) { return b == STa ? STb : STa; };
        for (int l = 0; l < c.layers && !R.rc; ++l) {
            const std::string lp = "model.encoder.layer." + std::to_string(l) + ".";
            const bool last = l == c.layers - 1;
            const bool cls_only = h->cls_only_last && last;
            const T* wqkv = raw ? (const T*)h->fold_qkv[l].w : (const T*)h->qkv_w[l];
            const float* bqkv = raw ? h->fold_qkv[l].b : h->qkv_b[l];
            const float* cqkv = raw ? h->fold_qkv[l].c : nullptr;
            const int64_t waves = attention_waves(rows, H, h->attention_pack != 0).total;
            const int att_flags = (h->attention_fast ? 2 : 0) | (h->attention_pack ? 4 : 0);
            if (!cls_only) {
                const bool by_pair = pairs && l == 0;
                GemmEpilogue<T> eq = R.epi();
                eq.bias = bqkv; eq.out_lo = BIG; eq.ld_lo = 3 * H;
                if (raw) { eq.fold_stats = hs_stats; eq.fold_c = cqkv; }
                R.gemm(Zt, H, wqkv, H, by_pair ? P : m, 3 * H, H, eq);
                hipLaunchKernelGGL((attention_rows_kernel<T>), dim3((unsigned)((waves + 3) / 4)), dim3(256), 0, st,
                                   (const T*)BIG, (size_t)3 * H, (const T*)BIG + H, (const T*)BIG + 2 * H, (size_t)3 * H,
                                   H, H / c.heads, p.row_offset, p.row_uniform, p.tok_key, r0, rows, tok0, scaling, 0 | att_flags,
                                   by_pair ? (const int32_t*)p.tok_pair : (const int32_t*)nullptr, CTX);
                R.check("attention");
            } else {
                T* KV = BIG;
                T* Q = BIG + (size_t)m * 2 * H;
                GemmEpilogue<T> ekv = R.epi();
                ekv.bias = bqkv + H; ekv.out_lo = KV; ekv.ld_lo = 2 * H;
                if (raw) { ekv.fold_stats = hs_stats; ekv.fold_c = cqkv + H; }
                R.gemm(Zt, H, wqkv + (size_t)H * H, H, m, 2 * H, H, ekv);
                GemmEpilogue<T> eq = R.epi();
                eq.bias = bqkv; eq.out_lo = Q; eq.ld_lo = H;
                if (raw) { eq.fold_stats = hs_stats; eq.fold_c = cqkv; }
                R.gemm(Zt, H, wqkv, H, rows, H, H, eq);
                hipLaunchKernelGGL((attention_rows_kernel<T>), dim3((unsigned)((waves + 3) / 4)), dim3(256), 0, st,
                                   (const T*)Q, (size_t)H, (const T*)KV, (const T*)KV + H, (size_t)2 * H,
                                   H, H / c.heads, p.row_offset, p.row_uniform, p.tok_key, r0, rows, tok0, scaling, 1 | att_flags,
                                   (const int32_t*)nullptr, CTX);
                R.check("attention(position 0)");
                zrows = rows;
            }
            float* s1 = other(hs_sum);
            float* st1 = other_stats(hs_stats);
            GemmEpilogue<T> eo = R.epi();
            eo.bias = R.Wf(lp + "attention.output.dense.bias");
            if (pairs && l == 0) eo.res_index = brow_pair;
            if (lo_stream) {
                eo.residual_lo = Zt; eo.ld_res_lo = H;
                if (raw) { eo.res_stats = hs_stats; eo.res_gamma = hs_gamma; eo.res_beta = hs_beta; }
                eo.out_lo = Ct; eo.ld_lo = H; eo.stats_part = PARTS; eo.ld_part = (int)ld_parts;
            } else {
                eo.residual = hs_sum; eo.ld_res = H;
                eo.res_stats = hs_stats; eo.res_gamma = hs_gamma; eo.res_beta = hs_beta;
                eo.out_f32 = s1; eo.ld_f32 = H;
                if (fold) { eo.out_lo = Zt; eo.ld_lo = H; eo.stats_part = PARTS; eo.ld_part = (int)ld_parts; }
            }
            R.gemm(CTX, H, R.Wlo(lp + "attention.output.dense.weight"), H, zrows, H, H, eo);
            const float* g1 = R.Wf(lp + "attention.output.LayerNorm.weight");
            const float* b1 = R.Wf(lp + "attention.output.LayerNorm.bias");
            const T* mid = lo_stream ? Ct : Zt;
            GemmEpilogue<T> ei = R.epi();
            ei.act = ACT_GELU_ERF; ei.out_lo = BIG; ei.ld_lo = I;
            if (fold) {
                R.ln_stats(PARTS, (int)ld_parts, zrows, c.ln_eps_encoder, st1);
                ei.bias = h->fold_up[l].b; ei.fold_stats = st1; ei.fold_c = h->fold_up[l].c;
                R.gemm(mid, H, (const T*)h->fold_up[l].w, H, zrows, I, H, ei);
            } else {
                R.layernorm(s1, zrows, g1, b1, c.ln_eps_encoder, nullptr, Zt, st1);
                ei.bias = R.Wf(lp + "intermediate.dense.bias");
                R.gemm(Zt, H, R.Wlo(lp + "intermediate.dense.weight"), H, zrows, I, H, ei);
            }
            float* s2 = other(s1);
            float* st2 = other_stats(st1);
            GemmEpilogue<T> ef = R.epi();
            ef.bias = R.Wf(lp + "output.dense.bias");
            if (lo_stream) {
                ef.residual_lo = Ct; ef.ld_res_lo = H; ef.res_stats = st1; ef.res_gamma = g1; ef.res_beta = b1;
                ef.out_lo = Zt; ef.ld_lo = H; ef.stats_part = PARTS; ef.ld_part = (int)ld_parts;
            } else {
                ef.residual = s1; ef.ld_res = H;
                ef.res_stats = st1; ef.res_gamma = g1; ef.res_beta = b1;
                ef.out_f32 = s2; ef.ld_f32 = H;
                if (fold && !last) { ef.out_lo = Zt; ef.ld_lo = H; ef.stats_part = PARTS; ef.ld_part = (int)ld_parts; }
            }
            R.gemm(BIG, I, R.Wlo(lp + "output.dense.weight"), I, zrows, H, I, ef);
            hs_gamma = R.Wf(lp + "output.LayerNorm.weight");
            hs_beta = R.Wf(lp + "output.LayerNorm.bias");
            hs_sum = s2; hs_stats = st2;
            if (!last) {
                if (fold) { R.ln_stats(PARTS, (int)ld_parts, zrows, c.ln_eps_encoder, st2); raw = true; }
                else R.layernorm(s2, zrows, hs_gamma, hs_beta, c.ln_eps_encoder, nullptr, Zt, st2);
            }
        }
        if (R.rc) return R.rc;

        float* bias_out = out_bias ? out_bias + r0 : nullptr;
        const int64_t* bias_rows = nullptr;
        int bias_dtype = -1;
        if (dest && dest->bias) {
            const size_t bes = dest->bias_dtype == ZETT_F32 ? 4 : 2;
            bias_rows = dest->rows ? dest->rows + r0 : nullptr;
            bias_out = (float*)((char*)dest->bias + (dest->rows ? 0 : (size_t)r0 * bes));
            bias_dtype = dest->bias_dtype;
        } else if (dest) {
            if (int rc = h->dest_sink.reserve((size_t)N * sizeof(float))) return rc;
            bias_out = h->dest_sink.as<float>() + r0;
        }
        LnReadout ro{c.predict_bias ? R.Wf("bias_projection.weight") : (const float*)nullptr,
                     c.predict_bias ? R.Wf("bias_projection.bias") : (const float*)nullptr, bias_out};
        ro.bias_rows = bias_rows;
        ro.range_flag = h->range_word;
        R.layernorm(hs_sum, rows, hs_gamma, hs_beta, c.ln_eps_encoder, Cf, Ct, nullptr, ro,
                    lo_stream ? (const T*)Zt : (const T*)nullptr, bias_dtype);
        R.check("readout");
        if (!R.rc) {
            if (ev_mode == 2) HIP_TRY(hipEventRecord(h->lane_ev[1], st));
            if (ev_mode == 3) HIP_TRY(hipStreamWaitEvent(st, h->lane_ev[1], 0));
            if (ev_mode == 1 || ev_mode == 3) HIP_TRY(hipEventRecord(h->out_ready[ZETT_OUT_BIAS], st));
        }

        const bool fold_heads = fold && h->ln_fold == 1 && h->fold_head_in.w != nullptr;
        {
            if (fold_heads) R.projector("output_projection.0.", Ct, Cf, rows, BIG, PRE, nullptr, CTX, PARTS, (int)ld_parts, STa);
            else R.projector("output_projection.0.", Ct, Cf, rows, BIG, PRE, nullptr, CTX);
            GemmEpilogue<T> e = R.epi();
            e.bias = fold_heads ? h->fold_head_in.b : R.Wf("output_projection.1.bias");
            e.scale = c.rescale ? h->head_scale : (fold_heads ? h->head_one : nullptr);
            e.shift = c.rescale ? h->head_shift : (fold_heads ? h->head_zero : nullptr);
            if (fold_heads) { e.fold_stats = STa; e.fold_c = h->fold_head_in.c; }
            e.ld_f32 = E; e.range_final = 1;
            const int width = c.single_head ? EIN : E;
            const bool split = c.single_head && c.separate_out;
            if (!dest) {
                e.out_f32 = out_in + (size_t)r0 * E;
                if (split) { e.split_col = E; e.out_f32_b = out_out + (size_t)r0 * E; }
            } else if (split) {
                e.split_col = E;
            }
            const T* w1 = fold_heads ? (const T*)h->fold_head_in.w : R.Wlo("output_projection.1.weight");
            if (dest) {
                const typename Runner<T>::DestOut din = dest_out(dest->in, dest->ld_in, r0), dout = dest_out(dest->out, dest->ld_out, r0);
                R.head_gemm(CTX, w1, rows, width, H, e, &din, split ? &dout : nullptr, E);
            } else {
                R.gemm(CTX, H, w1, H, rows, width, H, e);
            }
            if (!R.rc) {
                if (ev_mode == 2) HIP_TRY(hipEventRecord(h->lane_ev[2], st));
                if (ev_mode == 3) HIP_TRY(hipStreamWaitEvent(st, h->lane_ev[2], 0));
                if (ev_mode == 1 || ev_mode == 3) HIP_TRY(hipEventRecord(h->out_ready[ZETT_OUT_IN], st));
            }
        }
        if (c.separate_out && !c.single_head) {
            if (fold_heads) R.projector("output_projection_out.0.", Ct, Cf, rows, BIG, PRE, nullptr, CTX, PARTS, (int)ld_parts, STa);
            else R.projector("output_projection_out.0.", Ct, Cf, rows, BIG, PRE, nullptr, CTX);
            GemmEpilogue<T> e = R.epi();
            e.bias = fold_heads ? h->fold_head_out.b : R.Wf("output_projection_out.1.bias");
            e.scale = c.rescale ? R.Wf("out_scaler.w") : (fold_heads ? h->head_one : nullptr);
            e.shift = c.rescale ? R.Wf("out_scaler.b") : (fold_heads ? h->head_zero : nullptr);
            if (fold_heads) { e.fold_stats = STa; e.fold_c = h->fold_head_out.c; }
            e.ld_f32 = E; e.range_final = 1;
            const T* w2 = fold_heads ? (const T*)h->fold_head_out.w : R.Wlo("output_projection_out.1.weight");
            if (dest) {
                const typename Runner<T>::DestOut dout = dest_out(dest->out, dest->ld_out, r0);
                R.head_gemm(CTX, w2, rows, E, H, e, &dout, nullptr, E);
            } else {
                e.out_f32 = out_out + (size_t)r0 * E;
                R.gemm(CTX, H, w2, H, rows, E, H, e);
            }
        }
        return R.rc;
    };
    bool two_lanes = false;
    if (h->concurrent_lanes && Ttot <= MC && N >= 512) {
        const int Pn = pair_plan ? hoff[N + 3] : 0;
        const bool pairs_taken = pair_plan && Pn > 0 && (int64_t)Pn * 100 <= Ttot * 85;
        const double r = (double)((Ttot + 255) / 256) * (double)((H + 255) / 256) / 256.0;
        two_lanes = h->concurrent_lanes == 2 ||
                    (!pairs_taken && !h->time_gemm && H >= 1024 && r < 4.0 && (std::ceil(r) - r) / std::ceil(r) > 0.08);
    }
    if (two_lanes) {
        if (!h->lane_stream) HIP_TRY(hipStreamCreateWithFlags(&h->lane_stream, hipStreamNonBlocking));
        for (hipEvent_t& e : h->lane_ev)
            if (!e) HIP_TRY(hipEventCreateWithFlags(&e, hipEventDisableTiming));
        int64_t ra = ((N / 2 + 128) / 256) * 256;
        ra = std::min<int64_t>(std::max<int64_t>(ra, 256), N - 1);
        const size_t off1 = (size_t)(hoff[ra] - hoff[0]) + 384;
        HIP_TRY(hipEventRecord(h->lane_ev[0], st));
// ... 50 lines not shown
```

Measured before the change: 629,600.

## Reorder single-token rows first and skip their Q/K GEMM tiles

Adds a planning pass that flags rows holding a single non-pad token, permutes them to the front, and records a row map so outputs are scattered back to vocabulary order. For those rows attention reduces to the value vector, so the QKV GEMM launches skip the Q/K column tiles over the leading single-row block and attention avoids loading Q/K. This removes wasted matmul work and loads for single-token words, at the cost of extra plan kernels, a permutation copy, an indirect output scatter and a more complex tile mapping.

Result: no change. 629,800, median of 5 (+0.0%).

```diff
diff --git a/zett_amd/csrc/gemm.hip.h b/zett_amd/csrc/gemm.hip.h
--- a/zett_amd/csrc/gemm.hip.h
+++ b/zett_amd/csrc/gemm.hip.h
@@ -252,7 +252,36 @@
     int tile_order = 0;
     int group = 0;
     int row0 = 0;
+    int skip_rows = 0, skip_cols = 0;
 };
+
+struct G4dTile { int tm, tn; };
+__host__ __device__ inline G4dTile gemm4d_live_tile(int wg, int tiles_m, int tiles_n, int group, int stm, int sc) {
+    G4dTile t;
+    const int gfull = sc / group, rem = sc % group;
+    const int a = group * (tiles_m - stm);
+    if (wg < gfull * a) {
+        const int idx = wg % a;
+        t.tm = stm + idx / group; t.tn = (wg / a) * group + idx % group;
+        return t;
+    }
+    wg -= gfull * a;
+    int first_n = gfull * group;
+    int gn = tiles_n - first_n < group ? tiles_n - first_n : group;
+    if (gn > 0) {
+        const int head = stm * (gn - rem), live = gn * tiles_m - rem * stm;
+        if (wg < head) { t.tm = wg / (gn - rem); t.tn = first_n + rem + wg % (gn - rem); return t; }
+        if (wg < live) { wg -= head; t.tm = stm + wg / gn; t.tn = first_n + wg % gn; return t; }
+        wg -= live;
+        first_n += gn;
+    }
+    const int group_size = group * tiles_m;
+    first_n += (wg / group_size) * group;
+    gn = tiles_n - first_n < group ? tiles_n - first_n : group;
+    t.tn = first_n + (wg % group_size) % gn;
+    t.tm = (wg % group_size) / gn;
+    return t;
+}
 
 constexpr int GEMM_BM = 128;
 constexpr int GEMM_BN = 128;
diff --git a/zett_amd/csrc/gemm4d.hip.h b/zett_amd/csrc/gemm4d.hip.h
--- a/zett_amd/csrc/gemm4d.hip.h
+++ b/zett_amd/csrc/gemm4d.hip.h
@@ -65,7 +65,20 @@
     static constexpr int LDS_BYTES = STAGES * STAGE_BYTES;
 };
 
-template <typename T, int ACT = ACT_NONE, bool RES = false, int EPI = G4D_EPI_GENERIC, bool HALF = false, typename OT = void>
+struct G4dSkip { int stm, sc; };
+template <int BM, typename T>
+__host__ __device__ inline G4dSkip gemm4d_skip(const GemmArgs<T>& g, int tiles_m, int tiles_n) {
+    G4dSkip s{0, 0};
+    if (g.skip_rows <= g.row0 || g.skip_cols < G256_BN) return s;
+    s.stm = (g.skip_rows - g.row0) / BM;
+    if (s.stm > tiles_m) s.stm = tiles_m;
+    s.sc = g.skip_cols / G256_BN;
+    if (s.sc > tiles_n) s.sc = tiles_n;
+    if (s.stm == 0 || s.sc == 0) s.stm = s.sc = 0;
+    return s;
+}
+
+template <typename T, int ACT = ACT_NONE, bool RES = false, int EPI = G4D_EPI_GENERIC, bool HALF = false, typename OT = void, bool SKIP = false>
 __global__ __launch_bounds__(256) __attribute__((amdgpu_waves_per_eu(1, 1))) void gemm4d_tn_kernel(GemmArgs<T> g) {
     extern __shared__ __attribute__((aligned(16))) unsigned char smem[];
     constexpr int BK = GEMM_ROW_BYTES / (int)sizeof(T);
@@ -76,7 +89,9 @@
 
     const int tiles_m = (g.M - g.row0 + GEO::BM - 1) / GEO::BM;
     const int tiles_n = (g.N + G256_BN - 1) / G256_BN;
-    const int nwg = tiles_m * tiles_n;
+    G4dSkip skip{0, 0};
+    if constexpr (SKIP) skip = gemm4d_skip<GEO::BM>(g, tiles_m, tiles_n);
+    const int nwg = tiles_m * tiles_n - skip.stm * skip.sc;
     int wg = blockIdx.x;
     {
         const int q = nwg >> 3, r = nwg & 7, xcd = wg & 7;
@@ -84,7 +99,10 @@
     }
     const int GROUP_N = g.group > 0 ? g.group : 4;
     int tm, tn;
-    if (g.tile_order == 0) {
+    if (SKIP && skip.stm > 0) {
+        const G4dTile t = gemm4d_live_tile(wg, tiles_m, tiles_n, GROUP_N, skip.stm, skip.sc);
+        tm = t.tm; tn = t.tn;
+    } else if (g.tile_order == 0) {
         const int group_size = GROUP_N * tiles_m;
         const int first_n = (wg / group_size) * GROUP_N;
         const int gn = (tiles_n - first_n) < GROUP_N ? (tiles_n - first_n) : GROUP_N;
@@ -692,14 +710,15 @@
     return G4D_EPI_GENERIC;
 }
 
-template <typename T, int ACT, bool RES, int EPI, bool HALF = false>
+template <typename T, int ACT, bool RES, int EPI, bool HALF = false, bool SKIP = false>
 inline hipError_t launch_gemm4d_inst(const GemmArgs<T>& g, hipStream_t stream) {
+    static_assert(!SKIP || ((EPI == G4D_EPI_LO || EPI == G4D_EPI_LO_FOLD) && ACT == ACT_NONE && !RES), "skipped blocks: the QKV projections' epilogues only");
     constexpr int lds = EPI == G4D_EPI_GENERIC ? G256_LDS_BYTES : (G4dGeom<HALF>::LDS_BYTES > G4D_LDS_BYTES ? G4dGeom<HALF>::LDS_BYTES : G4D_LDS_BYTES);
     static_assert(lds <= 160 * 1024, "LDS budget");
     static DeviceFlags attr;
     bool* done = attr.current();
     if (!done || !*done) {
-        hipError_t e = hipFuncSetAttribute((const void*)gemm4d_tn_kernel<T, ACT, RES, EPI, HALF>, hipFuncAttributeMaxDynamicSharedMemorySize, lds);
+        hipError_t e = hipFuncSetAttribute((const void*)gemm4d_tn_kernel<T, ACT, RES, EPI, HALF, void, SKIP>, hipFuncAttributeMaxDynamicSharedMemorySize, lds);
         if (e != hipSuccess) return e;
         if (done) *done = true;
     }
@@ -707,7 +726,10 @@
     const int tiles_m = (g.M - g.row0 + BM - 1) / BM;
     const int tiles_n = (g.N + G256_BN - 1) / G256_BN;
     if (tiles_m <= 0 || tiles_n <= 0) return hipSuccess;
-    hipLaunchKernelGGL((gemm4d_tn_kernel<T, ACT, RES, EPI, HALF>), dim3(tiles_m * tiles_n), dim3(256), lds, stream, g);
+    G4dSkip skip{0, 0};
+    if constexpr (SKIP) skip = gemm4d_skip<BM>(g, tiles_m, tiles_n);
+    if (tiles_m * tiles_n - skip.stm * skip.sc <= 0) return hipSuccess;
+    hipLaunchKernelGGL((gemm4d_tn_kernel<T, ACT, RES, EPI, HALF, void, SKIP>), dim3(tiles_m * tiles_n - skip.stm * skip.sc), dim3(256), lds, stream, g);
     return hipGetLastError();
 }
 
@@ -715,8 +737,12 @@
 inline hipError_t launch_gemm4d_act(const GemmArgs<T>& g, hipStream_t stream, int mode) {
     const bool res = g.epi.residual != nullptr;
     switch (mode) {
-        case G4D_EPI_LO: return launch_gemm4d_inst<T, ACT, false, G4D_EPI_LO, HALF>(g, stream);
-        case G4D_EPI_LO_FOLD: return launch_gemm4d_inst<T, ACT, false, G4D_EPI_LO_FOLD, HALF>(g, stream);
+        case G4D_EPI_LO:
+            if constexpr (ACT == ACT_NONE) { if (g.skip_rows > 0) return launch_gemm4d_inst<T, ACT, false, G4D_EPI_LO, HALF, true>(g, stream); }
+            return launch_gemm4d_inst<T, ACT, false, G4D_EPI_LO, HALF>(g, stream);
+        case G4D_EPI_LO_FOLD:
+            if constexpr (ACT == ACT_NONE) { if (g.skip_rows > 0) return launch_gemm4d_inst<T, ACT, false, G4D_EPI_LO_FOLD, HALF, true>(g, stream); }
+            return launch_gemm4d_inst<T, ACT, false, G4D_EPI_LO_FOLD, HALF>(g, stream);
         case G4D_EPI_F32:
             if constexpr (ACT == ACT_NONE) return res ? launch_gemm4d_inst<T, ACT, true, G4D_EPI_F32, HALF>(g, stream) : launch_gemm4d_inst<T, ACT, false, G4D_EPI_F32, HALF>(g, stream);
             else if constexpr (ACT == ACT_GELU_TANH) { if (res) return launch_gemm4d_inst<T, ACT, true, G4D_EPI_F32, HALF>(g, stream); }
@@ -813,10 +839,29 @@
 hipError_t launch_gemm_4d_half_dst(const GemmArgs<bf16_t>& g, hipStream_t stream, int mode);
 
 template <typename T>
+inline bool gemm4d_skips(const GemmArgs<T>& g, int mode) {
+    return g.skip_rows >= G256_BM && g.skip_cols >= G256_BN && g.tile_order == 0 && !g.epi.dst && g.epi.act == ACT_NONE &&
+           (mode == G4D_EPI_LO || mode == G4D_EPI_LO_FOLD);
+}
+
+template <typename T>
+inline hipError_t launch_gemm4d_split(const GemmArgs<T>& g, hipStream_t stream, int mode, bool dst);
+
+template <typename T>
 inline hipError_t launch_gemm4d(const GemmArgs<T>& g, hipStream_t stream, bool force_generic = false) {
     const bool dst = g.epi.dst != nullptr;
     const int mode = dst ? gemm4d_dst_mode(g) : (force_generic && !g.epi.stats_part && !g.epi.fold_stats) ? G4D_EPI_GENERIC : gemm4d_epi_mode(g);
     if (mode < 0) return hipErrorInvalidValue;
+    if (!gemm4d_skips(g, mode)) {
+        GemmArgs<T> all = g;
+        all.skip_rows = all.skip_cols = 0;
+        return launch_gemm4d_split(all, stream, mode, dst);
+    }
+    return launch_gemm4d_split(g, stream, mode, dst);
+}
+
+template <typename T>
+inline hipError_t launch_gemm4d_split(const GemmArgs<T>& g, hipStream_t stream, int mode, bool dst) {
     int split = g.row0 == -1 ? gemm4d_row_split(g.M, g.N) : (g.row0 == -2 ? 0 : (g.row0 > 0 ? std::min(g.row0, g.M) : g.M));
     if (split < g.M && (!gemm4d_half_ok(g, mode) || split % G256_BM != 0)) split = g.M;
     GemmArgs<T> full = g;
diff --git a/zett_amd/csrc/gemm4d.inc b/zett_amd/csrc/gemm4d.inc
--- a/zett_amd/csrc/gemm4d.inc
+++ b/zett_amd/csrc/gemm4d.inc
@@ -13,4 +13,6 @@
 
 int gemm_4d_dst_mode(const GemmArgs<ZETT_GEMM_T>& g) { return gemm4d_dst_mode<ZETT_GEMM_T>(g); }
 
+bool gemm_4d_skips(const GemmArgs<ZETT_GEMM_T>& g) { return !g.epi.dst && gemm4d_skips<ZETT_GEMM_T>(g, gemm4d_epi_mode(g)); }
+
 }
diff --git a/zett_amd/csrc/gemm_launch.hip.h b/zett_amd/csrc/gemm_launch.hip.h
--- a/zett_amd/csrc/gemm_launch.hip.h
+++ b/zett_amd/csrc/gemm_launch.hip.h
@@ -18,5 +18,8 @@
 int gemm_4d_dst_mode(const GemmArgs<f16_t>& g);
 int gemm_4d_dst_mode(const GemmArgs<bf16_t>& g);
 inline int gemm_4d_dst_mode(const GemmArgs<float>&) { return -1; }
+bool gemm_4d_skips(const GemmArgs<f16_t>& g);
+bool gemm_4d_skips(const GemmArgs<bf16_t>& g);
+inline bool gemm_4d_skips(const GemmArgs<float>&) { return false; }
 
 }
diff --git a/zett_amd/csrc/rowops.hip.h b/zett_amd/csrc/rowops.hip.h
--- a/zett_amd/csrc/rowops.hip.h
+++ b/zett_amd/csrc/rowops.hip.h
@@ -30,6 +30,7 @@
     int32_t* err;
     int32_t* counters;
     int32_t n_pair_keys;
+    const int64_t* row_map;
 };
 
 __global__ void plan_rows_kernel(const int32_t* __restrict__ sfm, int64_t n_rows, int seq, int pad, int lam,
@@ -41,7 +42,8 @@
     for (int j = 0; j < seq; ++j) {
         const int id = row[j];
         if (id < 0 || id >= n_ids) {
-            atomicMax(p.err, (int)(n < 0x7ffffffe ? n + 1 : 0x7fffffff));
+            const int64_t rn = p.row_map ? p.row_map[n] : n;
+            atomicMax(p.err, (int)(rn < 0x7ffffffe ? rn + 1 : 0x7fffffff));
             p.row_count[n] = 0;
             p.row_uniform[n] = 2;
             return;
@@ -60,6 +62,36 @@
     }
     p.row_count[n] = count;
     p.row_uniform[n] = uniform ? 1 : 0;
+}
+
+__global__ void plan_single_flag_kernel(const int32_t* __restrict__ sfm, int64_t n_rows, int seq, int pad, int lam, int n_ids,
+                                        int32_t* __restrict__ flag) {
+    const int64_t n = (int64_t)blockIdx.x * blockDim.x + threadIdx.x;
+    if (n >= n_rows) return;
+    const int32_t* row = sfm + n * seq;
+    const int id0 = row[0];
+    bool single = lam == 0 && id0 != pad && id0 >= 0 && id0 < n_ids;
+    for (int j = 1; j < seq; ++j) single = single && row[j] == pad;
+    flag[n] = single ? 1 : 0;
+}
+
+__global__ void plan_permute_kernel(const int32_t* __restrict__ sfm, int64_t n_rows, int seq, const int32_t* __restrict__ flag,
+                                    const int32_t* __restrict__ rank, int min_single, int32_t* __restrict__ sfm_perm,
+                                    int64_t* __restrict__ row_map, int32_t* __restrict__ n_single_out) {
+    const int64_t n = (int64_t)blockIdx.x * blockDim.x + threadIdx.x;
+    if (n >= n_rows) return;
+    const int ns = rank[n_rows];
+    const bool on = ns >= min_single;
+    const int64_t d = !on ? n : (flag[n] ? (int64_t)rank[n] : (int64_t)ns + (n - rank[n]));
+    for (int j = 0; j < seq; ++j) sfm_perm[d * seq + j] = sfm[n * seq + j];
+    row_map[d] = n;
+    if (n == 0) *n_single_out = on ? ns : 0;
+}
+
+__global__ void compose_rows_kernel(const int64_t* __restrict__ perm, const int64_t* __restrict__ rows_caller, int64_t n,
+                                    int64_t* __restrict__ out) {
+    const int64_t i = (int64_t)blockIdx.x * blockDim.x + threadIdx.x;
+    if (i < n) out[i] = rows_caller[perm[i]];
 }
 
 __global__ __launch_bounds__(1024) void exclusive_scan_kernel(const int32_t* __restrict__ in,
@@ -191,6 +223,7 @@
         p.counters[0] = p.id_slot[n_ids];
         p.counters[1] = p.err[0];
         p.counters[2] = p.n_pair_keys ? p.pair_slot[p.n_pair_keys] : 0;
+        if (!p.row_map) p.counters[3] = 0;
     }
 }
 
@@ -684,6 +717,7 @@
         return t - t0 < lpr ? (size_t)__shfl(pslot, base + (t - t0), 64) : (size_t)tok_pair[tok0 + t];
     };
     const int nk = t1 - t0;
+    const bool one = nk == 1 && !uniform;
     if constexpr (sizeof(T) == 2) {
         if (nk <= ATT_FAST_KEYS && (flags & 2)) {
             const bool mine = li < nk && (uniform || tok_key[tok0 + t0 + li] != 0);
@@ -693,12 +727,13 @@
             for (int j = 0; j < ATT_FAST_KEYS; ++j) {
                 if (j < nk) {
                     const size_t kr = qrow(t0 + j);
+                    vv[j] = *(const uint4*)(vbase + kr * ldkv + ccol);
+                    if (one) { kk[j] = make_uint4(0, 0, 0, 0); qq[j] = make_uint4(0, 0, 0, 0); continue; }
                     kk[j] = *(const uint4*)(kbase + kr * ldkv + ccol);
-                    vv[j] = *(const uint4*)(vbase + kr * ldkv + ccol);
                     if (!cls_only) qq[j] = *(const uint4*)(qbase + kr * ldq + ccol);
                 }
             }
-            if (cls_only) qq[0] = *(const uint4*)(qbase + (size_t)rl * ldq + ccol);
+            if (cls_only && !one) qq[0] = *(const uint4*)(qbase + (size_t)rl * ldq + ccol);
             const float sc2 = scaling * 1.4426950408889634f;
 #pragma unroll
             for (int qi = 0; qi < ATT_FAST_KEYS; ++qi) {
@@ -743,7 +778,12 @@
     }
     for (int qi = 0; qi < nq; ++qi) {
         float q[8];
-        load8<T>(qbase + (cls_only ? (size_t)rl : qrow(t0 + qi)) * ldq + ccol, q);
+        if (one) {
+#pragma unroll
+            for (int c = 0; c < 8; ++c) q[c] = 0.f;
+        } else {
+            load8<T>(qbase + (cls_only ? (size_t)rl : qrow(t0 + qi)) * ldq + ccol, q);
+        }
         float mx = -INFINITY, l = 0.f, acc[8];
 #pragma unroll
         for (int c = 0; c < 8; ++c) acc[c] = 0.f;
@@ -751,7 +791,12 @@
             if (!uniform && !tok_key[tok0 + kj]) continue;
             float k[8], v[8];
             const size_t kr = qrow(kj);
-            load8<T>(kbase + kr * ldkv + ccol, k);
+            if (one) {
+#pragma unroll
+                for (int c = 0; c < 8; ++c) k[c] = 0.f;
+            } else {
+                load8<T>(kbase + kr * ldkv + ccol, k);
+            }
             load8<T>(vbase + kr * ldkv + ccol, v);
             float s = 0.f;
 #pragma unroll
diff --git a/zett_amd/csrc/zett_hip.hip b/zett_amd/csrc/zett_hip.hip
--- a/zett_amd/csrc/zett_hip.hip
+++ b/zett_amd/csrc/zett_hip.hip
@@ -69,6 +69,7 @@
     int table_lo = 1;
     int gemm_group = 0;
     int gemm4d_min_k = 512;
+    int single_rows = 1;
     int gemm_variant = 0;
     struct PlanSlot {
         DevBuf i32, u8;
@@ -80,6 +81,7 @@
         int64_t n_rows = 0;
         int seq = 0;
         bool pair_plan = false;
+        bool single_plan = false;
         const int32_t* ext_id_slot = nullptr;
         bool pending = false;
     } plan[2];
@@ -94,7 +96,7 @@
     int range_accumulate = 0;
     int32_t* range_word = nullptr;
     int32_t* range_host = nullptr;
-    DevBuf dest_word, dest_stage[2], dest_sink;
+    DevBuf dest_word, dest_stage[2], dest_sink, dest_map;
     int32_t* dest_host = nullptr;
     hipEvent_t dest_checked = nullptr;
     std::vector<hipEvent_t> ev;
@@ -195,7 +197,8 @@
     const int64_t max_tok = N * (int64_t)(seq + (c.embed_lang ? 1 : 0));
     const int64_t K = pair_keys(c, seq);
     const size_t scan_scratch = 2 * ((size_t)std::max<int64_t>(std::max<int64_t>(N, V), K) / SCAN_CHUNK + 2) + 1;
-    return ((size_t)N + (N + 1) + 3 + V + (V + 1) + V + 7 * (size_t)max_tok + 2 * (size_t)K + 2 + scan_scratch) * 4;
+    const size_t singles = (size_t)N + (N + 1) + (size_t)N * seq + 2 * (size_t)N + 2 + 1;
+    return ((size_t)N + (N + 1) + 3 + V + (V + 1) + V + 7 * (size_t)max_tok + 2 * (size_t)K + 2 + scan_scratch + singles) * 4;
 }
 
 static int64_t chunk_token_cap(const zett_config& c, size_t es) {
@@ -226,7 +229,16 @@
     bool pair_plan = false;
     int64_t PK = 0;
     size_t n_clear = 0;
+    int32_t* single_flag = nullptr;
+    int32_t* single_rank = nullptr;
+    int32_t* sfm_perm = nullptr;
+    int64_t* row_map = nullptr;
 };
+static bool single_rows_eligible(const zett_hypernet* h) {
+    return h->single_rows && h->precision != ZETT_PREC_F32 && h->gemm_variant == 0 && !h->cfg.single_head && !h->cfg.embed_lang &&
+           h->concurrent_lanes == 0;
+}
+constexpr int SINGLE_ROWS_MIN = 256;
 static PlanLayout plan_layout(const zett_hypernet* h, const zett_hypernet::PlanSlot& s, int64_t N, int seq) {
     const zett_config& c = h->cfg;
     const int lam = c.embed_lang ? 1 : 0;
@@ -243,7 +255,7 @@
     L.n_clear = (size_t)(base - s.i32.as<int32_t>());
     p.row_count = base; base += N;
     p.row_offset = base; base += N + 1;
-    p.counters = base; base += 3;
+    p.counters = base; base += 4;
     p.id_slot = base; base += V + 1;
     p.id_list = base; base += V;
     p.tok_slot = base; base += max_tok;
@@ -257,20 +269,26 @@
         p.pair_pos = base; base += max_tok;
         p.pair_slot = base; base += L.PK + 1;
     }
+    L.single_flag = base; base += N;
+    L.single_rank = base; base += N + 1;
+    L.sfm_perm = base; base += N * (int64_t)seq;
+    if ((base - s.i32.as<int32_t>()) & 1) base += 1;
+    L.row_map = (int64_t*)base; base += 2 * N;
     L.scan_tmp = base;
     p.row_uniform = s.u8.as<uint8_t>();
     p.tok_key = p.row_uniform + N;
     return L;
 }
 
-static int enqueue_plan(zett_hypernet* h, zett_hypernet::PlanSlot& s, const int32_t* sfm, int64_t N, int seq, hipStream_t st) {
+static int enqueue_plan(zett_hypernet* h, zett_hypernet::PlanSlot& s, const int32_t* sfm, int64_t N, int seq, hipStream_t st, bool singles = false) {
     const zett_config& c = h->cfg;
     const int lam = c.embed_lang ? 1 : 0;
     const int V = c.original_vocab_size + c.n_extra;
     const int64_t max_tok = N * (int64_t)(seq + lam);
+    const int32_t* const caller_sfm = sfm;
     if (int rc = s.i32.reserve(plan_i32_bytes(c, N, seq))) return rc;
     if (int rc = s.u8.reserve((size_t)N + (size_t)max_tok)) return rc;
-    const size_t need_ints = (size_t)N + 1 + 3;
+    const size_t need_ints = (size_t)N + 1 + 4;
     if (s.host_ints < need_ints) {
         if (s.host) (void)hipHostFree(s.host);
         s.host = nullptr;
@@ -279,10 +297,18 @@
     }
     if (!s.done) HIP_TRY(hipEventCreateWithFlags(&s.done, hipEventDisableTiming));
     if (!s.released) HIP_TRY(hipEventCreateWithFlags(&s.released, hipEventDisableTiming));
-    const PlanLayout L = plan_layout(h, s, N, seq);
-    const PlanArrays& p = L.p;
+    PlanLayout L = plan_layout(h, s, N, seq);
     HIP_TRY(hipMemsetAsync(s.i32.p, 0, L.n_clear * 4, st));
     const int rb = (int)((N + 255) / 256);
+    if (singles) {
+        hipLaunchKernelGGL(plan_single_flag_kernel, dim3(rb), dim3(256), 0, st, sfm, N, seq, c.pad_token_id, lam, V, L.single_flag);
+        launch_exclusive_scan(L.single_flag, L.single_rank, N, L.scan_tmp, st);
+        hipLaunchKernelGGL(plan_permute_kernel, dim3(rb), dim3(256), 0, st, sfm, N, seq, (const int32_t*)L.single_flag, (const int32_t*)L.single_rank,
+                           SINGLE_ROWS_MIN, L.sfm_perm, L.row_map, L.p.counters + 3);
+        L.p.row_map = L.row_map;
+        sfm = L.sfm_perm;
+    }
+    const PlanArrays& p = L.p;
     hipLaunchKernelGGL(plan_rows_kernel, dim3(rb), dim3(256), 0, st, sfm, N, seq, c.pad_token_id, lam, V, p);
     launch_exclusive_scan(p.row_count, p.row_offset, N, L.scan_tmp, st);
     launch_exclusive_scan(p.id_flag, p.id_slot, (int64_t)V, L.scan_tmp, st);
@@ -297,9 +323,9 @@
     }
     hipLaunchKernelGGL(plan_idlist_kernel, dim3((V + 255) / 256), dim3(256), 0, st, V, p);
     HIP_TRY(hipGetLastError());
-    HIP_TRY(hipMemcpyAsync(s.host, p.row_offset, ((size_t)N + 1 + 3) * 4, hipMemcpyDeviceToHost, st));
+    HIP_TRY(hipMemcpyAsync(s.host, p.row_offset, ((size_t)N + 1 + 4) * 4, hipMemcpyDeviceToHost, st));
     HIP_TRY(hipEventRecord(s.done, st));
-    s.sfm = sfm; s.n_rows = N; s.seq = seq; s.pair_plan = L.pair_plan; s.ext_id_slot = h->ext.id_slot;
+    s.sfm = caller_sfm; s.n_rows = N; s.single_plan = singles; s.seq = seq; s.pair_plan = L.pair_plan; s.ext_id_slot = h->ext.id_slot;
     return 0;
 }
 
@@ -347,7 +373,7 @@
         if (kv.second.lo && kv.second.lo != (void*)kv.second.f32) (void)hipFree(kv.second.lo);
     }
     for (void* p : h->owned) (void)hipFree(p);
-    for (DevBuf* b : {&h->table, &h->x0, &h->yf, &h->yt, &h->big, &h->pre, &h->ctx, &h->cf, &h->ct, &h->lnstats, &h->lnparts, &h->dest_word, &h->dest_stage[0], &h->dest_stage[1], &h->dest_sink})
+    for (DevBuf* b : {&h->table, &h->x0, &h->yf, &h->yt, &h->big, &h->pre, &h->ctx, &h->cf, &h->ct, &h->lnstats, &h->lnparts, &h->dest_word, &h->dest_stage[0], &h->dest_stage[1], &h->dest_sink, &h->dest_map})
         b->release();
     for (zett_hypernet::PlanSlot* psp : {&h->plan[0], &h->plan[1], &h->table_plan}) {
         zett_hypernet::PlanSlot& ps = *psp;
@@ -568,6 +594,9 @@
         h->gemm4d_min_k = (int)value;
     } else if (k == "range_accumulate") {
         h->range_accumulate = value != 0;
+    } else if (k == "single_rows") {
+        if (value < 0 || value > 1) return fail(ZETT_E_INVALID, "single_rows must be 0 (vocabulary row order) or 1 (single-position rows first, their Q/K tiles skipped)");
+        h->single_rows = (int)value;
     } else if (k == "gemm_variant") {
         if (value != 0 && value != 1 && value != 2 && value != 3 && value != 7 && value != 8)
             return fail(ZETT_E_INVALID, "gemm_variant must be 0 (auto), 1 (128x128), 2 (256x256 register-staged), 3 (384x256), 7 (256x256 four-wave direct-to-LDS) or 8 (7 with the generic epilogue drain)");
@@ -709,7 +738,7 @@
     HIP_TRY(hipEventRecord(h->plan_fork, (hipStream_t)input_stream));
     HIP_TRY(hipStreamWaitEvent(h->plan_stream, h->plan_fork, 0));
     if (ps.released) HIP_TRY(hipStreamWaitEvent(h->plan_stream, ps.released, 0));
-    if (int rc = enqueue_plan(h, ps, surface_forms, n_rows, seq, h->plan_stream)) return rc;
+    if (int rc = enqueue_plan(h, ps, surface_forms, n_rows, seq, h->plan_stream, single_rows_eligible(h))) return rc;
     ps.pending = true;
     return 0;
 }
@@ -922,13 +951,17 @@
     }
 
 
-    void gemm(const T* A, int lda, const T* Wp, int ldw, int M, int N, int K, const GemmEpilogue<T>& e) {
+    void gemm(const T* A, int lda, const T* Wp, int ldw, int M, int N, int K, const GemmEpilogue<T>& e, int skip_rows = 0, int skip_cols = 0) {
         if (rc || M <= 0) return;
         GemmArgs<T> g{A, lda, Wp, ldw, M, N, K, e};
         g.tile_order = h->gemm_tile_order;
         g.group = h->gemm_group;
         g.row0 = h->gemm_tail_split == 1 ? -1 : h->gemm_tail_split == 2 ? ((M / 2 + 255) / 256) * 256 : h->gemm_tail_split == 3 ? -2 : 0;
-        const double fl = 2.0 * (double)M * (double)N * (double)K;
+        const int variant = variant_for(M, N, K, e);
+        g.skip_rows = skip_rows; g.skip_cols = skip_cols;
+        if (variant != 7 || !gemm_4d_skips(g)) g.skip_rows = g.skip_cols = skip_rows = skip_cols = 0;
+        const double skipped = (double)skip_rows * (double)skip_cols;
+        const double fl = 2.0 * (double)K * ((double)M * (double)N - skipped);
         hipEvent_t e0 = nullptr, e1 = nullptr;
         if (h->time_gemm) {
             while (h->ev.size() < h->ev_used + 2) {
@@ -942,7 +975,6 @@
             h->ev_shape.push_back({M, N, K, 0});
             (void)hipEventRecord(e0, st);
         }
-        const int variant = variant_for(M, N, K, e);
         if (h->time_gemm && !h->ev_shape.empty()) h->ev_shape.back()[3] = variant;
         {
             zett_gemm_record r{};
@@ -951,7 +983,7 @@
                          (e.stats_part ? 16 : 0) | (e.fold_stats ? 32 : 0) | (e.residual_lo ? 64 : 0) | (e.act << 8) |
                          (e.dst ? 1024 : 0) | (staged_dst ? 2048 : 0);
             r.flops = fl;
-            const double mn = (double)M * (double)N;
+            const double mn = (double)M * (double)N - skipped;
             const double dst_es = e.dst_dtype == ZETT_F32 ? 4.0 : 2.0;
             r.bytes = ((double)M + (double)N) * (double)K * sizeof(T) + (e.out_lo ? mn * sizeof(T) : 0.0) + ((e.out_f32 || e.out_f32_b) ? mn * 4.0 : 0.0) +
                       (e.dst ? mn * dst_es : 0.0) +
@@ -1160,13 +1192,14 @@
     h->gemm_log.clear();
 
     zett_hypernet::PlanSlot& ps = h->plan[h->plan_cur ^ 1];
+    const bool single_plan = single_rows_eligible(h);
     if (ps.pending && ps.sfm == sfm && ps.n_rows == N && ps.seq == seq && ps.pair_plan == plan_layout(h, ps, N, seq).pair_plan &&
-        ps.ext_id_slot == h->ext.id_slot) {
+        ps.single_plan == single_plan && ps.ext_id_slot == h->ext.id_slot) {
         HIP_TRY(hipStreamWaitEvent(st, ps.done, 0));
     } else {
         if (ps.pending) HIP_TRY(hipEventSynchronize(ps.done));
         if (ps.released) HIP_TRY(hipStreamWaitEvent(st, ps.released, 0));
-        if (int rc = enqueue_plan(h, ps, sfm, N, seq, st)) return rc;
+        if (int rc = enqueue_plan(h, ps, sfm, N, seq, st, single_plan)) return rc;
     }
     ps.pending = false;
     h->plan_cur ^= 1;
@@ -1212,6 +1245,25 @@
     h->stats.packed_tokens = Ttot;
     h->stats.distinct_ids = D;
     h->stats.distinct_positions = Ttot;
+    const int64_t n_single = ps.single_plan ? hoff[N + 4] : 0;
+    zett_dest own_dest{};
+    if (n_single > 0) {
+        if (!dest) {
+            own_dest.in = out_in; own_dest.out = c.separate_out ? out_out : nullptr; own_dest.bias = out_bias;
+            own_dest.dtype = ZETT_F32; own_dest.bias_dtype = ZETT_F32; own_dest.ld_in = E; own_dest.ld_out = E;
+            own_dest.rows = PL.row_map; own_dest.n_dest_rows = N;
+        } else {
+            own_dest = *dest;
+            own_dest.rows = PL.row_map;
+            if (dest->rows) {
+                if (int rc = h->dest_map.reserve((size_t)N * sizeof(int64_t))) return rc;
+                hipLaunchKernelGGL(compose_rows_kernel, dim3((unsigned)((N + 255) / 256)), dim3(256), 0, st, (const int64_t*)PL.row_map, dest->rows, N, h->dest_map.as<int64_t>());
+                HIP_TRY(hipGetLastError());
+                own_dest.rows = h->dest_map.as<int64_t>();
+            }
+        }
+        dest = &own_dest;
+    }
 
     const WorkspaceSizes ws = workspace_sizes(c, sizeof(T), seq, Ttot, D, h->max_chunk_tokens);
     const int64_t MC = ws.chunk_tokens;
@@ -1270,6 +1322,8 @@
         const int rows = (int)(r1 - r0);
         const int tok0 = hoff[r0];
         const int m = hoff[r1] - tok0;
+        const int ns = (int)std::min<int64_t>(std::max<int64_t>(n_single - r0, 0), rows);
+        const int skip_r = ns / 256 * 256;
         h->stats.chunks += 1;
         hipStream_t st = lane.st;
         R.st = lane.st;
@@ -1348,7 +1402,7 @@
                 GemmEpilogue<T> eq = R.epi();
                 eq.bias = bqkv; eq.out_lo = BIG; eq.ld_lo = 3 * H;
                 if (raw) { eq.fold_stats = hs_stats; eq.fold_c = cqkv; }
-                R.gemm(Zt, H, wqkv, H, by_pair ? P : m, 3 * H, H, eq);
+                R.gemm(Zt, H, wqkv, H, by_pair ? P : m, 3 * H, H, eq, by_pair ? 0 : skip_r, by_pair ? 0 : 2 * H / 256 * 256);
                 hipLaunchKernelGGL((attention_rows_kernel<T>), dim3((unsigned)((waves + 3) / 4)), dim3(256), 0, st,
                                    (const T*)BIG, (size_t)3 * H, (const T*)BIG + H, (const T*)BIG + 2 * H, (size_t)3 * H,
                                    H, H / c.heads, p.row_offset, p.row_uniform, p.tok_key, r0, rows, tok0, scaling, 0 | att_flags,
@@ -1360,11 +1414,11 @@
                 GemmEpilogue<T> ekv = R.epi();
                 ekv.bias = bqkv + H; ekv.out_lo = KV; ekv.ld_lo = 2 * H;
                 if (raw) { ekv.fold_stats = hs_stats; ekv.fold_c = cqkv + H; }
-                R.gemm(Zt, H, wqkv + (size_t)H * H, H, m, 2 * H, H, ekv);
+                R.gemm(Zt, H, wqkv + (size_t)H * H, H, m, 2 * H, H, ekv, skip_r, H / 256 * 256);
                 GemmEpilogue<T> eq = R.epi();
-                eq.bias = bqkv; eq.out_lo = Q; eq.ld_lo = H;
-                if (raw) { eq.fold_stats = hs_stats; eq.fold_c = cqkv; }
-                R.gemm(Zt, H, wqkv, H, rows, H, H, eq);
+                eq.bias = bqkv; eq.out_lo = Q + (size_t)ns * H; eq.ld_lo = H;
+                if (raw) { eq.fold_stats = hs_stats + 2 * (size_t)ns; eq.fold_c = cqkv; }
+                R.gemm(Zt + (size_t)ns * H, H, wqkv, H, rows - ns, H, H, eq);
                 hipLaunchKernelGGL((attention_rows_kernel<T>), dim3((unsigned)((waves + 3) / 4)), dim3(256), 0, st,
                                    (const T*)Q, (size_t)H, (const T*)KV, (const T*)KV + H, (size_t)2 * H,
                                    H, H / c.heads, p.row_offset, p.row_uniform, p.tok_key, r0, rows, tok0, scaling, 1 | att_flags,
```
